# UZ-SLAMLab/DefSLAM

Hardware: AMD Instinct MI355X
Metric: SfT GN iters/sec (500-node mesh, 1k matches) (higher is better)
Workload: dtype f64

## Files before the change

### defslam_amd/_lib.py

```python
from __future__ import annotations

import ctypes as C
import os

_HERE = os.path.dirname(os.path.abspath(__file__))
LIB_PATH = os.path.join(_HERE, "lib", "libdefslam_hip.so")
LAB_LIB_PATH = os.path.join(_HERE, "lib", "libdefslam_hip_lab.so")

DSH_OK = 0
DSH_ERR_ARG = 1
DSH_ERR_STATE = 3
DSH_TRACE_STRIDE = 8
DSH_MAX_ITERS = 64

c_double_p = C.POINTER(C.c_double)
c_float_p = C.POINTER(C.c_float)
c_i32_p = C.POINTER(C.c_int32)
c_u8_p = C.POINTER(C.c_uint8)


class SftFrameC(C.Structure):
    _fields_ = [
        ("Tcw", c_float_p),
        ("K", C.c_double * 4),
# ... 37 lines not shown

class BbsC(C.Structure):
    _fields_ = [("umin", C.c_double), ("umax", C.c_double), ("nptsu", C.c_int32), ("vmin", C.c_double), ("vmax", C.c_double),
                ("nptsv", C.c_int32), ("valdim", C.c_int32)]


SchwarpProblemC._fields_ = [("bbs", BbsC), ("P", C.c_int32), ("kp1", C.c_void_p), ("kp2", C.c_void_p), ("invsig", C.c_void_p), ("fx_slot", C.c_double),
                            ("fy_slot", C.c_double), ("lam", C.c_double), ("fx", C.c_float), ("fy", C.c_float), ("max_iters", C.c_int32), ("x", C.c_void_p),
                            ("diff", C.c_void_p), ("drop", C.c_void_p), ("info", C.c_int32 * 2), ("costs", C.c_double * 2), ("init_lambda", C.c_double), ("init_ok", C.c_int32)]



class SchwarpStoreC(C.Structure):
    _fields_ = [("point_id", C.c_void_p), ("idx2", C.c_void_p), ("tag", C.c_int32)]


class TrackFrameC(C.Structure):
    _fields_ = [("Tcw", c_float_p), ("Ow", C.c_float * 3), ("K", C.c_float * 4), ("bounds", C.c_float * 4), ("grid_cols", C.c_int32),
                ("grid_rows", C.c_int32), ("levels", C.c_int32), ("scale_factors", c_float_p), ("log_scale_factor", C.c_float), ("N", C.c_int32),
                ("kp", c_float_p), ("octave", c_i32_p), ("desc", c_u8_p), ("state", c_u8_p)]


class TrackProblemC(C.Structure):
    _fields_ = [("frame", TrackFrameC), ("mode", C.c_int32), ("th", C.c_float), ("Q", C.c_int32), ("xyz", c_float_p), ("octave", c_i32_p),
                ("normal", c_float_p), ("max_distance", c_float_p), ("desc", c_u8_p), ("skip", c_u8_p), ("match", c_i32_p), ("in_view", c_u8_p),
                ("level", c_i32_p), ("uv", c_float_p), ("view_cos", c_float_p), ("nmatches", C.c_int32), ("rescans", C.c_int32)]


DSH_TRACK_FRAME = 0
DSH_TRACK_LOCAL = 1


class MpKeyFrameC(C.Structure):
    _fields_ = [("Ow", C.c_float * 3), ("N", C.c_int32), ("desc", c_u8_p), ("octave", c_i32_p), ("levels", C.c_int32),
                ("scale_factors", c_float_p), ("bad", C.c_int32)]


DSH_MP_DESCRIPTOR = 1
DSH_MP_NORMAL_DEPTH = 2
DSH_MP_NO_OBS = 1
DSH_MP_NO_GOOD_DESC = 2
DSH_MP_MAX_OBS = 65535


class MpdbDescC(C.Structure):
    _fields_ = [("ctx", C.c_void_p), ("point_capacity", C.c_int32), ("keyframe_capacity", C.c_int32), ("observation_capacity", C.c_int64)]


DSH_MPDB_POSITION = 1
DSH_MPDB_NORMAL_DEPTH = 2
DSH_MPDB_DESCRIPTOR = 4


class TrackCloseCountsC(C.Structure):
    _fields_ = [(n, C.c_int32) for n in ("matches_inliers", "matches_outliers", "to_match_local", "observed", "inliers", "outliers",
                                         "local_map_points", "n_moved")]


class TrackEndCountsC(C.Structure):
    _fields_ = [(n, C.c_int32) for n in ("cleaned", "dropped", "kept")]


class PoseOnlyProblemC(C.Structure):
    _fields_ = [("Tcw", c_float_p), ("K", C.c_float * 4), ("N", C.c_int32), ("kp", c_float_p), ("octave", c_i32_p), ("levels", C.c_int32),
                ("inv_level_sigma2", c_float_p), ("frame_points", c_i32_p), ("outlier", c_u8_p), ("Tcw_out", C.c_float * 16),
                ("pose", C.c_double * 7), ("n_initial", C.c_int32), ("n_bad", C.c_int32), ("n_good", C.c_int32), ("rounds", C.c_int32),
                ("iters", C.c_int32 * 4), ("trials", C.c_int32 * 4), ("bad", C.c_int32 * 4), ("chi2", C.c_double * 4)]


class KfKeypointsC(C.Structure):
    _fields_ = [("rows", C.c_int32), ("cols", C.c_int32), ("N", C.c_int32), ("kp", c_float_p)]


class SurfaceGridC(C.Structure):
    _fields_ = [("ctx", C.c_void_p), ("bbs", C.POINTER(BbsC)), ("depth_ctrl", c_double_p), ("Twc", c_float_p), ("xs", C.c_int32), ("ys", C.c_int32)]


class TemplateSwitchCountsC(C.Structure):
    _fields_ = [(n, C.c_int32) for n in ("n_new", "first_id", "n_moved", "n_masked", "n_embedded", "n_points")]


class TemplateSwitchInputC(C.Structure):
    _fields_ = [("kfdb", C.c_void_p), ("slot", C.c_int32), ("kf", C.POINTER(KfKeypointsC)), ("surface_pts", c_float_p), ("Twc", c_float_p)]


class AnchorListsC(C.Structure):
    _fields_ = ([(n, C.c_int32) for n in ("anchor_capacity", "pair_capacity", "query_capacity")] + [("max_matrix_bytes", C.c_int64)] +
                [(n, c_i32_p) for n in ("anchor_slot", "anchor_count", "anchor_pairs", "pair_ptr", "pair_idx1", "pair_idx2", "pair_point")] +
                [("pair_own", c_u8_p)] + [(n, c_i32_p) for n in ("query_ptr", "query_idx1", "query_point")] + [("has", c_u8_p)] +
                [(n, C.c_int32) for n in ("n_anchors", "n_pairs", "n_queries", "n_no_ref")])


DSH_MP_NO_REF = 4
DSH_MP_SKIPPED_BAD = 8
DSH_UPKEEP_IDS = 0
DSH_UPKEEP_EMBEDDED = 1


class KeyframeProcessInputC(C.Structure):
    _fields_ = [("kfdb", C.c_void_p), ("slot", C.c_int32)]


class KeyframeProcessCountsC(C.Structure):
    _fields_ = [(n, C.c_int32) for n in ("n_empty", "n_bad", "n_added", "n_recent", "n_no_good_desc", "n_no_ref")] + [("first_record", C.c_int64)]


class PointUpkeepInputC(C.Structure):
    _fields_ = [("kfdb", C.c_void_p), ("what", C.c_int32), ("select", C.c_int32), ("n", C.c_int32), ("ids", c_i32_p)]


class PointUpkeepCountsC(C.Structure):
    _fields_ = [(n, C.c_int32) for n in ("n_selected", "n_no_obs", "n_no_good_desc", "n_no_ref", "n_bad")]


class PointEraseCountsC(C.Structure):
    _fields_ = [(n, C.c_int32) for n in ("n_found", "n_ref_moved", "n_set_bad", "n_records", "n_entries")]


DIFFPROP_FIELDS = ["I1u", "I1v", "I2u", "I2v", "J12a", "J12b", "J12c", "J12d", "J21a", "J21b", "J21c", "J21d",
                   "H12uux", "H12uuy", "H12uvx", "H12uvy", "H12vvx", "H12vvy"]


EXPORTED_SYMBOLS = [
    "dsh_create", "dsh_destroy", "dsh_last_error", "dsh_stream", "dsh_synchronize",
    "dsh_template_build", "dsh_template_set", "dsh_template_dims", "dsh_template_get", "dsh_template_embed",
    "dsh_sft_solve", "dsh_sft_batch_upload", "dsh_sft_batch_run", "dsh_sft_batch_download",
    "dsh_sft_batch_counts", "dsh_sft_batch_problem_info",
    "dsh_bbs_eval", "dsh_bbs_coloc", "dsh_normals_estimate", "dsh_schwarp_eval", "dsh_schwarp_fit", "dsh_schwarp_fit_batch",
    "dsh_sfn_estimate", "dsh_bbs_bending", "dsh_warp_initialize", "dsh_search_by_schwarp",
    "dsh_template_embed_device", "dsh_scale_min_median", "dsh_optimize_horn", "dsh_surface_register",
    "dsh_comm_unique_id", "dsh_comm_create", "dsh_comm_destroy", "dsh_sft_shared_solve", "dsh_sft_shared_solve_group", "dsh_sft_connected_solve", "dsh_sft_connected_solve_group",
    "dsh_diffdb_create", "dsh_diffdb_destroy", "dsh_diffdb_clear", "dsh_diffdb_count", "dsh_diffdb_append", "dsh_schwarp_fit_batch_store",
    "dsh_normals_estimate_db", "dsh_sfn_estimate_db",
    "dsh_search_by_projection_batch", "dsh_search_by_projection_frame", "dsh_search_by_projection_local",
    "dsh_kfdb_create", "dsh_kfdb_destroy", "dsh_kfdb_clear", "dsh_kfdb_add", "dsh_kfdb_set_bad", "dsh_kfdb_count", "dsh_mappoint_update",
    "dsh_mpdb_create", "dsh_mpdb_destroy", "dsh_mpdb_clear", "dsh_mpdb_point_count", "dsh_mpdb_keyframe_count", "dsh_mpdb_add_points",
    "dsh_mpdb_update_points", "dsh_mpdb_set_points_bad", "dsh_mpdb_add_observations", "dsh_mpdb_erase_observations", "dsh_mpdb_add_keyframe",
    "dsh_mpdb_set_keyframe_point", "dsh_mpdb_set_keyframe_parent", "dsh_mpdb_set_keyframe_bad",
    "dsh_local_map_update", "dsh_local_map_points", "dsh_local_map_search",
    "dsh_trackstate_set_embedding", "dsh_trackstate_clear_embedding", "dsh_trackstate_set_counters", "dsh_trackstate_get",
    "dsh_trackstate_seed_local_points", "dsh_trackstate_repose", "dsh_trackstate_cull", "dsh_track_close_frame",
    "dsh_track_end_frame", "dsh_track_last_frame", "dsh_motion_model_search",
    "dsh_track_pose_only", "dsh_track_pose_only_batch",
    "dsh_surface_vertices", "dsh_need_new_template", "dsh_template_switch", "dsh_point_store_get_points", "dsh_point_store_get_embedding",
    "dsh_point_store_add_observations_indexed", "dsh_point_store_set_reference_keyframes", "dsh_point_store_get_reference_keyframes", "dsh_keyframe_anchors",
    "dsh_keyframe_process_new", "dsh_point_store_upkeep",
    "dsh_point_store_erase_observations", "dsh_point_store_set_bad", "dsh_point_store_cull", "dsh_point_store_get_observations",
    "dsh_point_store_get_keyframe_table",
]
DSH_COMM_ID_BYTES = 128

LAB_SYMBOLS = ["dsh_lab_set_option", "dsh_lab_sft_run_timed", "dsh_lab_sft_assemble_timed", "dsh_lab_sft_phase_ms", "dsh_lab_sft_step_trace",
               "dsh_lab_sft_system", "dsh_lab_sft_solver_info", "dsh_lab_sft_wave_check", "dsh_lab_sft_dump", "dsh_lab_sft_rounds_timed",
               "dsh_lab_sft_factor_check"]

_lib = None
_lab = None


def load() -> C.CDLL:
    global _lib
    if _lib is None:
        _lib = _bind(LIB_PATH, lab=False)
    return _lib


def load_lab() -> C.CDLL:
    global _lab
    if _lab is None:
        _lab = _bind(LAB_LIB_PATH, lab=True)
    return _lab


def _bind(path: str, lab: bool) -> C.CDLL:
    if not os.path.exists(path):
        raise OSError(f"{path} is missing: run `python -c 'import __graft_entry__ as g; g.build()'` "
                      f"(or `make -C defslam_amd/csrc`). There is no CPU fallback.")
    L = C.CDLL(path)
    vp = C.c_void_p
    L.dsh_create.argtypes = [C.POINTER(vp), C.c_int]
    L.dsh_destroy.argtypes = [vp]
    L.dsh_last_error.argtypes = [vp]
    L.dsh_last_error.restype = C.c_char_p
    L.dsh_stream.argtypes = [vp]
    L.dsh_stream.restype = vp
    L.dsh_synchronize.argtypes = [vp]
    L.dsh_template_build.argtypes = [vp, C.c_int, c_double_p, C.c_int, c_i32_p]
    L.dsh_template_set.argtypes = [vp, C.c_int, c_double_p, c_u8_p, c_i32_p, c_i32_p, c_double_p, c_double_p, C.c_int, c_i32_p,
                                   c_double_p, C.c_double]
    L.dsh_template_dims.argtypes = [vp, c_i32_p, c_i32_p, c_i32_p]
    L.dsh_template_get.argtypes = [vp, c_u8_p, c_i32_p, c_i32_p, c_double_p, c_double_p, c_i32_p, c_double_p, c_double_p]
    L.dsh_template_embed.argtypes = [vp, C.c_int, c_float_p, c_i32_p, c_i32_p, c_float_p]
    L.dsh_sft_solve.argtypes = [vp, C.POINTER(SftFrameC), C.POINTER(SftResultC)]
    L.dsh_sft_batch_upload.argtypes = [vp, C.c_int, C.POINTER(SftFrameC)]
    L.dsh_sft_batch_run.argtypes = [vp]
    L.dsh_sft_batch_download.argtypes = [vp, C.c_int, C.POINTER(SftResultC)]
    L.dsh_sft_batch_counts.argtypes = [vp, C.POINTER(C.c_int64), C.POINTER(C.c_int64)]
    L.dsh_sft_batch_problem_info.argtypes = [vp, C.c_int, C.POINTER(C.c_int64), c_i32_p]
    L.dsh_bbs_eval.argtypes = [vp, C.POINTER(BbsC), c_double_p, c_double_p, c_double_p, C.c_int, C.c_int, C.c_int, c_double_p, c_u8_p]
    L.dsh_bbs_coloc.argtypes = [vp, C.POINTER(BbsC), c_double_p, c_double_p, C.c_int, C.c_int, C.c_int, c_i32_p, c_double_p, c_i32_p]
    L.dsh_normals_estimate.argtypes = [vp, C.c_int, c_i32_p, c_float_p, c_u8_p, c_float_p, c_u8_p, c_float_p, c_u8_p, c_float_p,
                                       c_double_p, c_double_p, c_i32_p, c_float_p, c_float_p, c_u8_p, c_i32_p]
    L.dsh_schwarp_eval.argtypes = [vp, C.POINTER(BbsC), C.c_int, c_float_p, c_float_p, c_float_p, C.c_double, C.c_double, C.c_double, c_double_p,
                                   c_double_p, c_double_p]
    L.dsh_schwarp_fit.argtypes = [vp, C.POINTER(BbsC), C.c_int, c_float_p, c_float_p, c_float_p, C.c_double, C.c_double, C.c_double, C.c_float,
                                  C.c_float, C.c_int, c_double_p, c_float_p, c_u8_p, c_i32_p, c_double_p]
    L.dsh_schwarp_fit_batch.argtypes = [vp, C.c_int, C.POINTER(SchwarpProblemC)]
    L.dsh_diffdb_create.argtypes = [vp, C.c_int64, C.POINTER(vp)]
    L.dsh_diffdb_destroy.argtypes = [vp]
    L.dsh_diffdb_clear.argtypes = [vp]
    L.dsh_diffdb_count.argtypes = [vp]
    L.dsh_diffdb_count.restype = C.c_int64
    L.dsh_diffdb_append.argtypes = [vp, C.c_int, c_float_p, c_i32_p, c_i32_p, c_i32_p]
    L.dsh_schwarp_fit_batch_store.argtypes = [vp, C.c_int, C.POINTER(SchwarpProblemC), C.POINTER(SchwarpStoreC), vp]
    L.dsh_normals_estimate_db.argtypes = [vp, vp, C.c_int, c_i32_p, c_float_p, c_u8_p, c_float_p, c_double_p, c_double_p, c_i32_p, c_float_p, c_i32_p,
                                          C.c_int32, c_i32_p, c_i32_p, c_i32_p, c_i32_p, c_float_p, c_u8_p]
    L.dsh_sfn_estimate.argtypes = [vp, C.POINTER(BbsC), C.c_int, c_double_p, c_double_p, c_float_p, C.c_double, C.c_double, C.c_int, c_double_p, c_double_p,
                                   c_double_p, c_double_p, c_float_p, c_i32_p]
    L.dsh_sfn_estimate_db.argtypes = [vp, C.POINTER(BbsC), vp, C.c_int, c_i32_p, c_double_p, c_double_p, C.c_double, C.c_double, C.c_int, c_double_p, c_double_p,
                                      c_double_p, c_double_p, c_float_p, c_i32_p]
    L.dsh_bbs_bending.argtypes = [C.POINTER(BbsC), C.c_double, c_double_p]
    L.dsh_search_by_schwarp.argtypes = [vp, C.POINTER(BbsC), c_double_p, C.c_int, c_float_p, c_u8_p, c_float_p, c_float_p, C.c_int, C.c_int, C.c_int, c_float_p,
                                        c_u8_p, c_u8_p, C.c_float, C.c_int, c_i32_p, c_i32_p]
    L.dsh_warp_initialize.argtypes = [vp, C.POINTER(BbsC), C.c_int, c_float_p, c_float_p, C.c_double, c_double_p, c_i32_p]
    c_i64_p = C.POINTER(C.c_int64)
    L.dsh_template_embed_device.argtypes = [vp, C.c_int, c_float_p, c_i32_p, c_i32_p, c_float_p]
    L.dsh_scale_min_median.argtypes = [vp, C.c_int, c_float_p, c_float_p, c_double_p, C.c_int64, c_float_p, c_i64_p, c_i32_p]
    L.dsh_optimize_horn.argtypes = [vp, C.c_int, c_float_p, c_float_p, c_double_p, C.c_double, C.c_double, c_i32_p, c_double_p]
    L.dsh_surface_register.argtypes = [vp, C.c_int, c_float_p, c_float_p, c_double_p, C.c_int64, c_float_p, C.c_double, C.c_int, c_i32_p, c_double_p,
                                       c_double_p, c_float_p, c_double_p]
    L.dsh_comm_unique_id.argtypes = [vp]
    L.dsh_comm_create.argtypes = [vp, C.c_int, C.c_int, vp, C.POINTER(vp)]
    L.dsh_comm_destroy.argtypes = [vp]
    L.dsh_sft_shared_solve.argtypes = [vp, vp, C.POINTER(SftFrameC), C.POINTER(SftResultC)]
    L.dsh_sft_shared_solve_group.argtypes = [C.c_int, C.POINTER(vp), C.POINTER(SftFrameC), C.POINTER(SftResultC)]
    L.dsh_sft_connected_solve.argtypes = [vp, vp, C.POINTER(SftFrameC), C.POINTER(SftResultC)]
    L.dsh_sft_connected_solve_group.argtypes = [vp, vp, C.POINTER(SftFrameC), C.POINTER(SftResultC)]
    L.dsh_search_by_projection_batch.argtypes = [vp, C.c_int, C.POINTER(TrackProblemC)]
    L.dsh_search_by_projection_frame.argtypes = [vp, C.POINTER(TrackFrameC), C.c_int, c_float_p, c_i32_p, c_u8_p, C.c_float, c_i32_p, c_i32_p]
    L.dsh_search_by_projection_local.argtypes = [vp, C.POINTER(TrackFrameC), C.c_int, c_float_p, c_float_p, c_float_p, c_u8_p, c_u8_p, C.c_float,
                                                 c_i32_p, c_u8_p, c_i32_p, c_i32_p]
    L.dsh_kfdb_create.argtypes = [vp, C.c_int32, C.POINTER(vp)]
    L.dsh_kfdb_destroy.argtypes = [vp]
    L.dsh_kfdb_clear.argtypes = [vp]
    L.dsh_kfdb_add.argtypes = [vp, C.POINTER(MpKeyFrameC), c_i32_p]
    L.dsh_kfdb_set_bad.argtypes = [vp, C.c_int32, C.c_int32]
    L.dsh_kfdb_count.argtypes = [vp]
    L.dsh_mappoint_update.argtypes = [vp, vp, C.c_int, c_float_p, c_i32_p, c_i32_p, c_i32_p, c_i32_p, C.c_int32, c_u8_p, c_i32_p, c_float_p,
                                      c_float_p, c_float_p, c_i32_p]
    i32 = C.c_int32
    L.dsh_mpdb_create.argtypes = [C.POINTER(MpdbDescC), C.POINTER(vp)]
    L.dsh_mpdb_destroy.argtypes = [vp]
    L.dsh_mpdb_clear.argtypes = [vp]
    L.dsh_mpdb_point_count.argtypes = [vp]
    L.dsh_mpdb_keyframe_count.argtypes = [vp]
    L.dsh_mpdb_add_points.argtypes = [vp, C.c_int, c_float_p, c_float_p, c_float_p, c_u8_p, c_u8_p, c_i32_p]
    L.dsh_mpdb_update_points.argtypes = [vp, C.c_int, c_i32_p, i32, c_float_p, c_float_p, c_float_p, c_u8_p]
    L.dsh_mpdb_set_points_bad.argtypes = [vp, C.c_int, c_i32_p, c_u8_p]
    L.dsh_mpdb_add_observations.argtypes = [vp, C.c_int, c_i32_p, c_i32_p]
    L.dsh_mpdb_erase_observations.argtypes = [vp, C.c_int, c_i32_p, c_i32_p]
    L.dsh_mpdb_add_keyframe.argtypes = [vp, i32, c_i32_p, i32, i32, c_i32_p]
    L.dsh_mpdb_set_keyframe_point.argtypes = [vp, i32, i32, i32]
    L.dsh_mpdb_set_keyframe_parent.argtypes = [vp, i32, i32]
    L.dsh_mpdb_set_keyframe_bad.argtypes = [vp, i32, i32]
    L.dsh_local_map_update.argtypes = [vp, C.c_int, c_i32_p, c_u8_p, i32, c_i32_p, c_i32_p, c_i32_p, c_i32_p, c_i32_p, c_i32_p]
    L.dsh_local_map_points.argtypes = [vp, i32, c_i32_p, c_i32_p]
    L.dsh_local_map_search.argtypes = [vp, C.POINTER(TrackFrameC), C.c_float, i32, c_i32_p, c_i32_p, c_u8_p, c_i32_p, c_float_p, c_float_p, c_i32_p]
    L.dsh_trackstate_set_embedding.argtypes = [vp, C.c_int, c_i32_p, c_i32_p, c_double_p]
    L.dsh_trackstate_clear_embedding.argtypes = [vp]
    L.dsh_trackstate_set_counters.argtypes = [vp, C.c_int, c_i32_p, c_i32_p, c_i32_p]
    L.dsh_trackstate_get.argtypes = [vp, C.c_int, c_i32_p, c_i32_p, c_i32_p, c_i32_p, c_float_p]
    L.dsh_trackstate_seed_local_points.argtypes = [vp, C.c_int, c_i32_p]
    L.dsh_trackstate_repose.argtypes = [vp, C.c_int, c_double_p, c_i32_p]
    L.dsh_trackstate_cull.argtypes = [vp, C.c_int, c_i32_p, c_i32_p, i32, c_u8_p]
    L.dsh_track_close_frame.argtypes = [vp, C.POINTER(TrackFrameC), C.c_int, c_i32_p, c_u8_p, C.c_int, c_double_p, i32, C.POINTER(TrackCloseCountsC)]
    L.dsh_track_end_frame.argtypes = [vp, C.c_int, c_i32_p, c_u8_p, c_i32_p, c_i32_p, c_u8_p, C.POINTER(TrackEndCountsC)]
    L.dsh_track_last_frame.argtypes = [vp, i32, c_i32_p, c_i32_p, c_i32_p]
    L.dsh_motion_model_search.argtypes = [vp, C.POINTER(TrackFrameC), C.c_float, C.c_float, i32, c_i32_p, c_i32_p, c_i32_p, c_float_p]
    L.dsh_track_pose_only.argtypes = [vp, C.POINTER(PoseOnlyProblemC)]
    L.dsh_track_pose_only_batch.argtypes = [vp, C.c_int, C.POINTER(PoseOnlyProblemC)]
    L.dsh_surface_vertices.argtypes = [C.POINTER(SurfaceGridC), c_double_p]
    L.dsh_need_new_template.argtypes = [vp, i32, C.POINTER(KfKeypointsC), c_i32_p, c_u8_p]
    L.dsh_template_switch.argtypes = [vp, C.POINTER(TemplateSwitchInputC), c_i32_p, C.POINTER(TemplateSwitchCountsC)]
    L.dsh_point_store_get_points.argtypes = [vp, C.c_int, c_i32_p, c_float_p, c_float_p, c_float_p, c_u8_p, c_u8_p]
    L.dsh_point_store_get_embedding.argtypes = [vp, C.c_int, c_i32_p, c_i32_p, c_double_p]
    L.dsh_point_store_add_observations_indexed.argtypes = [vp, C.c_int, c_i32_p, c_i32_p, c_i32_p]
    L.dsh_point_store_set_reference_keyframes.argtypes = [vp, C.c_int, c_i32_p, c_i32_p]
    L.dsh_point_store_get_reference_keyframes.argtypes = [vp, C.c_int, c_i32_p, c_i32_p]
    L.dsh_keyframe_anchors.argtypes = [vp, i32, i32, C.POINTER(AnchorListsC)]
    L.dsh_keyframe_process_new.argtypes = [vp, C.POINTER(KeyframeProcessInputC), c_u8_p, c_i32_p, C.POINTER(KeyframeProcessCountsC)]
    L.dsh_point_store_upkeep.argtypes = [vp, C.POINTER(PointUpkeepInputC), c_i32_p, C.POINTER(PointUpkeepCountsC)]
    L.dsh_point_store_erase_observations.argtypes = [vp, C.c_int, c_i32_p, c_i32_p, i32, c_u8_p, C.POINTER(PointEraseCountsC)]
    L.dsh_point_store_set_bad.argtypes = [vp, C.c_int, c_i32_p, C.POINTER(PointEraseCountsC)]
    L.dsh_point_store_cull.argtypes = [vp, C.c_int, c_i32_p, c_i32_p, i32, c_u8_p, C.POINTER(PointEraseCountsC)]
    L.dsh_point_store_get_observations.argtypes = [vp, C.c_int, c_i32_p, c_i32_p, i32, c_i32_p, c_i32_p, c_i32_p]
    L.dsh_point_store_get_keyframe_table.argtypes = [vp, i32, i32, c_i32_p]
    for name in EXPORTED_SYMBOLS:
        fn = getattr(L, name)
        if name not in ("dsh_last_error", "dsh_stream"):
            fn.restype = C.c_int
    if lab:
        L.dsh_lab_set_option.argtypes = [vp, C.c_char_p, C.c_int]
        L.dsh_lab_sft_run_timed.argtypes = [vp, C.c_int, c_double_p]
        L.dsh_lab_sft_assemble_timed.argtypes = [vp, C.c_int, c_double_p]
        L.dsh_lab_sft_phase_ms.argtypes = [vp, C.c_int, c_double_p]
        L.dsh_lab_sft_step_trace.argtypes = [vp, C.c_int, c_double_p]
        L.dsh_lab_sft_system.argtypes = [vp, C.c_int, C.c_int32, c_double_p, c_double_p, c_double_p]
        L.dsh_lab_sft_solver_info.argtypes = [vp, C.c_int, c_i32_p]
        L.dsh_lab_sft_wave_check.argtypes = [vp, C.c_double, C.c_int, C.c_int, c_double_p, c_double_p, c_i32_p, c_double_p]
        L.dsh_lab_sft_dump.argtypes = [vp, C.c_int, C.c_int, C.c_int64, c_double_p]
        L.dsh_lab_sft_rounds_timed.argtypes = [vp, c_double_p, c_i32_p]
        L.dsh_lab_sft_factor_check.argtypes = [vp, c_double_p, c_u8_p, C.c_int, c_double_p, c_i32_p]
        for name in LAB_SYMBOLS:
            getattr(L, name).restype = C.c_int
    return L


class HipEvents:

    def __init__(self):
        self._hip = C.CDLL("libamdhip64.so")
        self._hip.hipEventCreate.argtypes = [C.POINTER(C.c_void_p)]
        self._hip.hipEventRecord.argtypes = [C.c_void_p, C.c_void_p]
        self._hip.hipEventSynchronize.argtypes = [C.c_void_p]
        self._hip.hipEventElapsedTime.argtypes = [C.POINTER(C.c_float), C.c_void_p, C.c_void_p]
        self._hip.hipEventDestroy.argtypes = [C.c_void_p]
        self.e0, self.e1 = C.c_void_p(), C.c_void_p()
        for e in (self.e0, self.e1):
            if self._hip.hipEventCreate(C.byref(e)) != 0:
                raise OSError("hipEventCreate failed")

    def start(self, stream: int):
        if self._hip.hipEventRecord(self.e0, C.c_void_p(stream)) != 0:
            raise OSError("hipEventRecord failed")

    def stop_ms(self, stream: int) -> float:
        ms = C.c_float()
        if (self._hip.hipEventRecord(self.e1, C.c_void_p(stream)) != 0 or self._hip.hipEventSynchronize(self.e1) != 0
                or self._hip.hipEventElapsedTime(C.byref(ms), self.e0, self.e1) != 0):
            raise OSError("HIP event timing failed")
        return float(ms.value)

    def close(self):
        for e in (self.e0, self.e1):
            if e:
                self._hip.hipEventDestroy(e)
        self.e0 = self.e1 = None


HIP_DEVICE_ATTRIBUTE_MULTIPROCESSOR_COUNT = 63


def device_cus(device: int = 0) -> int:
    hip = C.CDLL("libamdhip64.so")
    hip.hipDeviceGetAttribute.argtypes = [C.POINTER(C.c_int), C.c_int, C.c_int]
    n = C.c_int(0)
    if hip.hipDeviceGetAttribute(C.byref(n), HIP_DEVICE_ATTRIBUTE_MULTIPROCESSOR_COUNT, int(device)) != 0 or n.value <= 0:
        raise OSError("hipDeviceGetAttribute(hipDeviceAttributeMultiprocessorCount) failed")
    return int(n.value)
```

### defslam_amd/csrc/dsh_api.cpp

```cpp
#include <hip/hip_runtime.h>

#include <algorithm>
#include <cmath>
#include <cstdio>
#include <cstdlib>
#include <cstring>

#include <memory>
#include <mutex>
#include <string>
#include <vector>

#include "dsh_sft_ctx.h"

#include "mapping_launch.h"

#ifdef DSH_LAB
#include "../../include/defslam_hip_debug.h"
#endif

LdsMarks g_lds_marks[64];
std::mutex g_lds_mu;

using dsh::Tcw_from_pose7;

dsh_ctx_base* dsh_base(dsh_ctx* ctx) { return static_cast<dsh_ctx_base*>(ctx); }
const dsh::TemplateHost* dsh_facet_template(dsh_ctx_base* c) {
  const dsh_ctx* x = static_cast<const dsh_ctx*>(c);
  return x && x->tmpl.valid && x->tmpl.F > 0 ? &x->tmpl : nullptr;
}

namespace {

void drop_graphs(dsh_ctx* c) {
  if (!c->host_only && c->stream) (void)hipStreamSynchronize(c->stream);
  for (auto& g : c->graphs)
    if (g->d_base) (void)hipFree(g->d_base);
  c->graphs.clear();
  c->packed.clear();
}

int upload_template(dsh_ctx* c) {
  c->B = 0;
  c->ran = false;
  drop_graphs(c);
  if (c->host_only) return DSH_OK;
  const dsh::TemplateHost& t = c->tmpl;
  Arena a;
  const size_t o_xyz0 = a.take(sizeof(double) * 3 * t.n);
  const size_t o_ptr = a.take(sizeof(int32_t) * (t.n + 1));
  const size_t o_idx = a.take(sizeof(int32_t) * t.nbr_idx.size());
  const size_t o_w = a.take(sizeof(double) * t.nbr_w.size());
  const size_t o_sw = a.take(sizeof(double) * t.n);
  const size_t o_k0 = a.take(sizeof(double) * t.n);
  if (c->d_tmpl) { (void)hipFree(c->d_tmpl); c->d_tmpl = nullptr; }
  HIPCHK(c, hipMalloc((void**)&c->d_tmpl, a.size));
  c->d_tmpl_bytes = a.size;
  std::vector<char> st(a.size, 0);
  std::memcpy(&st[o_xyz0], t.xyz0.data(), sizeof(double) * 3 * t.n);
  std::memcpy(&st[o_ptr], t.nbr_ptr.data(), sizeof(int32_t) * (t.n + 1));
  std::memcpy(&st[o_idx], t.nbr_idx.data(), sizeof(int32_t) * t.nbr_idx.size());
  std::memcpy(&st[o_w], t.nbr_w.data(), sizeof(double) * t.nbr_w.size());
  std::memcpy(&st[o_sw], t.nbr_sumw.data(), sizeof(double) * t.n);
  std::memcpy(&st[o_k0], t.k0.data(), sizeof(double) * t.n);
  HIPCHK(c, hipMemcpy(c->d_tmpl, st.data(), a.size, hipMemcpyHostToDevice));
  c->dt.xyz0 = (const double*)(c->d_tmpl + o_xyz0);
  c->dt.nbr_ptr = (const int32_t*)(c->d_tmpl + o_ptr);
  c->dt.nbr_idx = (const int32_t*)(c->d_tmpl + o_idx);
  c->dt.nbr_w = (const double*)(c->d_tmpl + o_w);
  c->dt.nbr_sumw = (const double*)(c->d_tmpl + o_sw);
  c->dt.k0 = (const double*)(c->d_tmpl + o_k0);
  return DSH_OK;
}

template <class T>
size_t reserve(Arena& a, const std::vector<T>& v) { return a.take(sizeof(T) * v.size()); }
template <class T>
void put(char* st, size_t off, const std::vector<T>& v) {
  if (!v.empty()) std::memcpy(st + off, v.data(), sizeof(T) * v.size());
}

int graph_for(dsh_ctx* c, const std::vector<uint8_t>& opt, dsh::SftGraph** out, std::string& err) {
  uint64_t h = 1469598103934665603ull;
  for (uint8_t b : opt) { h ^= b; h *= 1099511628211ull; }
  for (auto& g : c->graphs)
    if (g->opt_hash == h && g->opt == opt) { g->last_use = c->upload_serial; *out = g.get(); return DSH_OK; }
  if (c->graphs.size() >= 64) {
    if (!c->host_only && c->stream) (void)hipStreamSynchronize(c->stream);
    auto& gs = c->graphs;
    for (size_t i = 0; i < gs.size();) {
      if (gs[i]->last_use != c->upload_serial) {
        if (gs[i]->d_base) (void)hipFree(gs[i]->d_base);
        gs.erase(gs.begin() + i);
      } else {
        i++;
      }
    }
  }
  std::unique_ptr<dsh::SftGraph> g(new dsh::SftGraph());
  const int rc = dsh::build_graph(c->tmpl, opt, *g, err);
  if (rc != DSH_OK) return rc;
  g->last_use = c->upload_serial;
  if (!c->host_only) {
    Arena a;
    auto& o = g->o;
    o.act = reserve(a, g->act); o.actnode = reserve(a, g->actnode); o.star_node = reserve(a, g->star_node); o.star_sL = reserve(a, g->star_sL);
    o.str_nodes = reserve(a, g->str_nodes); o.str_L0 = reserve(a, g->str_L0); o.off_ptr = reserve(a, g->off_ptr); o.off_rc = reserve(a, g->off_rc);
    o.sh_ptr = reserve(a, g->sh_ptr); o.sh_rec = reserve(a, g->sh_rec); o.sh_cf = reserve(a, g->sh_cf); o.tmask = reserve(a, g->tmask);
    o.hgather = reserve(a, g->hgather);
    o.hgatherT = reserve(a, g->hgatherT);
    std::vector<char> st(a.size, 0);
    put(st.data(), o.act, g->act); put(st.data(), o.actnode, g->actnode); put(st.data(), o.star_node, g->star_node); put(st.data(), o.star_sL, g->star_sL);
    put(st.data(), o.str_nodes, g->str_nodes); put(st.data(), o.str_L0, g->str_L0); put(st.data(), o.off_ptr, g->off_ptr); put(st.data(), o.off_rc, g->off_rc);
    put(st.data(), o.sh_ptr, g->sh_ptr); put(st.data(), o.sh_rec, g->sh_rec); put(st.data(), o.sh_cf, g->sh_cf); put(st.data(), o.tmask, g->tmask);
    put(st.data(), o.hgather, g->hgather);
    put(st.data(), o.hgatherT, g->hgatherT);
    if (hipMalloc((void**)&g->d_base, a.size) != hipSuccess) { err = "out of device memory (graph)"; return DSH_ERR_HIP; }
    g->d_bytes = a.size;
    if (hipMemcpy(g->d_base, st.data(), a.size, hipMemcpyHostToDevice) != hipSuccess) { (void)hipFree(g->d_base); err = "graph upload failed"; return DSH_ERR_HIP; }
  }
  *out = g.get();
  c->graphs.push_back(std::move(g));
  return DSH_OK;
}

int pack_problem(dsh_ctx* c, const dsh_sft_frame& f, Packed& P, std::string& err) {
  const dsh::TemplateHost& t = c->tmpl;
  std::vector<uint8_t> viewed, opt;
  int rc = dsh::frame_active_set(t, f, viewed, opt, err);
  if (rc != DSH_OK) return rc;
  rc = graph_for(c, opt, &P.g, err);
  if (rc != DSH_OK) return rc;
  const dsh::SftGraph& g = *P.g;
  rc = dsh::pack_frame(t, g, f, viewed, P.f, err);
  if (rc != DSH_OK) return rc;
  SftDev& h = P.h;
  h = SftDev{};
  h.n = t.n; h.nA = g.nA; h.Dn = 3 * g.nA; h.kd = g.kd; h.ldh = h.kd + 1;
  h.M = f.M; h.V = P.f.V; h.S = g.S; h.Es = g.Es; h.noff = g.noff; h.max_iters = f.max_iters; h.mode = 0;
  h.fx = f.K[0]; h.fy = f.K[1]; h.cx = f.K[2]; h.cy = f.K[3];
  h.w_ref = f.reg_temp / std::pow(t.median_L, 2);
  h.w_curv = f.reg_lap / (double)g.nA;
  h.w_str = g.Es > 0 ? f.reg_inex / (double)g.Es : 0.0;
  const float deltaMono = (float)std::sqrt(5.991);
  h.hub_delta = (double)deltaMono;
  h.hub_dsqr = h.hub_delta * h.hub_delta;
  return DSH_OK;
}

int run_rounds_enqueue(dsh_ctx* c);
int run_rounds(dsh_ctx* c) {
  const int rc = run_rounds_enqueue(c);
  if (rc != DSH_OK)
    for (int s = 0; s < c->plan.n_sub; s++) if (c->sub_stream[s]) (void)hipStreamSynchronize(c->sub_stream[s]);
  return rc;
}
int run_rounds_enqueue(dsh_ctx* c) {
  const int B = c->B, S = c->plan.n_sub;
  int b0[kSftMaxSub + 1];
  for (int s = 0; s <= S; s++) b0[s] = (int)((long long)B * s / S);
  int tail_below = -1;
  if (S == 1 && c->opt.tail != 0) {
    if (c->opt.tail > 0) tail_below = c->opt.tail * c->num_cus;
    else tail_below = std::min(4 * c->num_cus, std::max(2 * c->num_cus, (int)((long long)3 * B / 4)));
  }
  auto launch = [&](int s, int phase) {
    const bool ev = c->phase_events && S == 1;
    if (ev) { hipEvent_t e; if (hipEventCreate(&e) == hipSuccess) { (void)hipEventRecord(e, c->stream); c->phase_events->push_back(e); c->phase_ids.push_back(phase); } }
    hipError_t r;
    {
      LDS_LOCK();
      if (phase == SFTB_PH_TAIL) r = sftb_tail_launch(c->d_probs + b0[s], c->d_runs + b0[s], c->d_counters + 16 * s, b0[s + 1] - b0[s], c->plan.max_kd, c->plan.jl_doubles, &LDS_MARKS(c).tail, c->num_cus, tail_below, c->sub_stream[s]);
      else r = sftb_launch(c->d_probs + b0[s], c->d_runs + b0[s], c->d_counters + 16 * s, c->d_linlist + b0[s], b0[s + 1] - b0[s], phase, c->plan.jl_doubles, c->plan.xyz_doubles, LDS_MARKS(c).b,
                           c->num_cus, tail_below, c->sub_stream[s]);
    }
    if (ev) { hipEvent_t e; if (hipEventCreate(&e) == hipSuccess) { (void)hipEventRecord(e, c->stream); c->phase_events->push_back(e); } }
    return r;
  };
  if (S > 1) {
    HIPCHK(c, hipEventRecord(c->sub_event[0], c->stream));
    for (int s = 1; s < S; s++) HIPCHK(c, hipStreamWaitEvent(c->sub_stream[s], c->sub_event[0], 0));
  }
  for (int s = 0; s < S; s++) HIPCHK(c, launch(s, SFTB_PH_INIT));
  const int worst = std::max(1, c->plan.max_iters_batch) * 10 + 1;
  int rounds = 0, group = std::max(1, std::min(worst, c->rounds_hint));
  if (tail_below >= B) group = 0;
  HIPCHK(c, c->spec_done.ensure(64 * kSftMaxSub, true));
  int rc = DSH_OK;
  while (true) {
    for (int i = 0; i < group && rounds < worst; i++, rounds++)
      for (int s = 0; s < S; s++) {
        HIPCHK(c, launch(s, SFTB_PH_LIN));
        HIPCHK(c, launch(s, SFTB_PH_FACTOR));
        HIPCHK(c, launch(s, SFTB_PH_TRIAL));
      }
    if (tail_below >= 0) HIPCHK(c, launch(0, SFTB_PH_TAIL));
    for (int s = 0; s < S; s++) HIPCHK(c, hipMemcpyAsync(c->spec_done.p + 64 * s, c->d_counters + 16 * s, 8 * sizeof(int), hipMemcpyDeviceToHost, c->sub_stream[s]));
    for (int s = 0; s < S; s++) HIPCHK(c, hipStreamSynchronize(c->sub_stream[s]));
    int done = 0;
    for (int s = 0; s < S; s++) done += *reinterpret_cast<const int*>(c->spec_done.p + 64 * s);
    const int* c0 = reinterpret_cast<const int*>(c->spec_done.p);
    if (done >= B) { c->rounds_hint = (tail_below >= 0 && c0[6]) ? std::max(1, c0[7]) : rounds; break; }
    if (rounds >= worst) { rc = dsh_fail(c, DSH_ERR_STATE, "batched rounds: a problem did not terminate within its trial budget"); break; }
    group = 2;
  }
  return rc;
}

int run_once(dsh_ctx* c) {
  if (c->plan.rounds_mode) return run_rounds(c);
  if (c->plan.K <= 1) {
    LDS_LOCK();
    HIPCHK(c, sft_lm_launch(c->d_probs, c->B, c->plan.max_kd, c->plan.jl_doubles, c->plan.nw, LDS_MARKS(c).lm, c->stream));
    return DSH_OK;
  }
  const int K = c->plan.K, B = c->B;
  HIPCHK(c, hipMemsetAsync(c->d_spec, 0, sizeof(SftSpec) * (size_t)B * K, c->stream));
  const int rounds_per_iter = (10 + K - 1) / K;
  const int worst = c->plan.max_iters_batch * rounds_per_iter;
  auto launch = [&](int phase) { LDS_LOCK(); return sft_spec_launch(c->d_probs, c->d_spec, B, K, phase, c->plan.nh, c->opt.owner_waves, c->plan.max_kd, c->plan.jl_doubles, LDS_MARKS(c).spec, c->stream); };
  if (c->plan.nh > 0) HIPCHK(c, hipMemsetAsync(c->d_sync, 0, c->layout.sync_total, c->stream));
  HIPCHK(c, launch(SFT_SPEC_INIT));
  int rounds = 0, group = std::max(2, std::min(worst, c->spec_hint));
  HIPCHK(c, c->spec_done.ensure(sizeof(SftSpec) * (size_t)B, true));
  while (true) {
    for (int i = 0; i < group && rounds < worst; i++, rounds++) {
      HIPCHK(c, launch(SFT_SPEC_LIN));
      if (c->plan.any_split) {
        HIPCHK(c, launch(SFT_SPEC_FACTOR));
        HIPCHK(c, launch(SFT_SPEC_SOLVE));
      }
      HIPCHK(c, launch(SFT_SPEC_TRIAL));
    }
    HIPCHK(c, launch(SFT_SPEC_LIN));
    HIPCHK(c, hipMemcpyAsync(c->spec_done.p, c->d_spec, sizeof(SftSpec) * (size_t)B, hipMemcpyDeviceToHost, c->stream));
    HIPCHK(c, hipStreamSynchronize(c->stream));
    const SftSpec* sp = reinterpret_cast<const SftSpec*>(c->spec_done.p);
    bool all_done = true;
    int needed = 0;
    for (int b = 0; b < B; b++) { all_done = all_done && sp[b].done; needed = std::max(needed, sp[b].launches); }
    if (all_done) { c->spec_hint = needed; break; }
    if (rounds >= worst) return dsh_fail(c, DSH_ERR_STATE, "speculative trials: a problem did not terminate within its launch budget");
    group = 2;
  }
  return DSH_OK;
}


SftBatchLayout layout_batch(const SftBatchPlan& plan, const std::vector<Packed>& packed, int B) {
  const int K = plan.K, nh = plan.nh;
  SftBatchLayout L;
  Arena a;
  L.o_tab = a.take(sizeof(SftDev) * B * K);
  L.ro.resize(B);
  for (int b = 0; b < B; b++) {
    const dsh::SftFramePack& F = packed[b].f;
    SftBatchLayout::ReadOnly& o = L.ro[b];
    o.obs_nodes = reserve(a, F.obs_nodes); o.obs_bary = reserve(a, F.obs_bary); o.obs_uv = reserve(a, F.obs_uv); o.obs_w = reserve(a, F.obs_w);
    o.ob_ptr = reserve(a, F.ob_ptr); o.ob_m = reserve(a, F.ob_m); o.ob_c = reserve(a, F.ob_c); o.viewed = reserve(a, F.viewed);
    o.xyz_init = reserve(a, F.xyz_init);
    o.pose_init = a.take(8 * 8);
  }
  L.ro_bytes = a.size;
  L.res_off = a.size;
  (void)a.take(sizeof(SftResHdr) * (size_t)B);
  L.res_offs.resize(B);
  for (int b = 0; b < B; b++) {
    const SftDev& h = packed[b].h;
    SftBatchLayout::Result& r = L.res_offs[b];
    r.xyz = a.take(8 * 3 * (size_t)h.n) - L.res_off; r.chi2 = a.take(8 * (size_t)h.M) - L.res_off;
    r.trace = a.take(8 * DSH_TRACE_STRIDE * DSH_MAX_ITERS) - L.res_off;
    r.mp = a.take(4 * 3 * (size_t)h.M) - L.res_off; r.outl = a.take((size_t)h.M) - L.res_off;
  }
  L.res_bytes = a.size - L.res_off;
  L.ws.resize((size_t)B * K);
  L.ws_off = a.size;
  L.o_spec = a.take(sizeof(SftSpec) * (size_t)B * K);
  L.o_runs = a.take(plan.rounds_mode ? sizeof(SftRun) * (size_t)B + 64 * kSftMaxSub + sizeof(int) * (size_t)B : 0);
  if (nh > 0)
    for (int e = 0; e < B * K; e++) {
      const SftProblemPlan& p = plan.prob[e % B];
      if (p.split) for (int g = 0; g < 2; g++) L.sync_total += Arena::round((size_t)4 * (16 + p.part[g].nT));
    }
  L.o_sync = a.take(L.sync_total);
  size_t sync_used = 0;
  for (int e = 0; e < B * K; e++) {
    const int b = e % B, lane = e / B;
    const SftDev& h = packed[b].h;
    const SftProblemPlan& p = plan.prob[b];
    const size_t Dnp = (size_t)((h.Dn + kNB - 1) / kNB) * kNB;
    SftBatchLayout::Work& w = L.ws[e];
    w.sx0 = a.take(K > 1 ? 8 * 3 * (size_t)h.n : 0); w.sx1 = a.take(K > 1 ? 8 * 3 * (size_t)h.n : 0);
    w.shadow_xyz = a.take(lane ? 8 * 3 * (size_t)h.n : 0); w.shadow_chi2 = a.take(lane ? 8 * (size_t)h.M : 0); w.shadow_hdr = a.take(lane ? sizeof(SftResHdr) : 0);
    w.bak = a.take(8 * 3 * (size_t)h.n);
    w.camrec = a.take(8 * (size_t)h.M * SFT_CAM_STRIDE);
    w.wtv = a.take(p.lds_class >= 1 ? 0 : 8 * ((size_t)h.M + 1)); w.Jstar = a.take(p.lds_class >= 1 ? 0 : 8 * 4 * (size_t)h.S);
    w.Anode = a.take(p.lds_class >= 2 ? 0 : 8 * 6 * (size_t)h.nA); w.Jstr = a.take(p.lds_class >= 2 ? 0 : 8 * 4 * (size_t)h.Es);
    const size_t band_elems = p.tile_mode ? (Dnp / kTS + SFT_H_PAD_TILE_ROWS) * (size_t)p.tpr * kTS * kTS : Dnp * (size_t)h.ldh;
    const size_t bord_elems = (SFT_BORDER + 1) * Dnp + SFT_H_PAD_BORDER;
    w.Hc = a.take(p.tile_mode == 1 ? 8 * packed[b].g->hc_elems() : 0);
    w.Hb = a.take(p.tile_mode == 1 ? 0 : 8 * band_elems); w.Hbord = a.take(8 * bord_elems); w.Hcn = a.take(8 * 56);
    w.Lb = a.take(8 * band_elems); w.Lbord = a.take(8 * bord_elems); w.Lc = a.take(8 * 56);
    w.Linv = a.take(8 * (Dnp / kTS) * (size_t)kTS * kTS);
    w.Lt = a.take(p.tile_mode == 2 ? 8 * band_elems : 0); w.LbT = a.take(p.tile_mode == 2 ? 8 * (Dnp / kTS) * (size_t)kTS * kTS : 0);
    w.x = a.take(8 * (Dnp + 8)); w.dbg = a.take(1024);
    if (p.split)
      for (int g = 0; g < 4; g++) {
        const SftPart& q = p.part[g];
        const size_t tiles = 8 * (size_t)q.nT * q.tpr * kTS * kTS, col = 8 * (size_t)q.nT * kTS * kTS;
        SftBatchLayout::Part& po = w.part[g];
        po.Hb = a.take(g < 2 && lane == 0 ? tiles : 0);
        po.Lb = a.take(tiles); po.Lt = a.take(tiles); po.LbT = a.take(col); po.Linv = a.take(col);
        po.Lbord = a.take(8 * 8 * (size_t)kTS * q.nT); po.x = a.take(8 * ((size_t)kTS * q.nT + 8)); po.xchg = a.take(8 * (size_t)p.sp_xl);
        const bool helped = nh > 0 && g < 2;
        po.Pf = a.take(helped ? tiles : 0); po.PfB = a.take(helped ? col : 0);
        po.sync = L.o_sync + sync_used;
        if (helped) sync_used += Arena::round((size_t)4 * (16 + q.nT));
      }
  }
  L.size = a.size;
  return L;
}

void stage_read_only(char* st, const SftBatchLayout& L, const std::vector<Packed>& packed, int B) {
  for (int b = 0; b < B; b++) {
    const dsh::SftFramePack& F = packed[b].f;
    const SftBatchLayout::ReadOnly& o = L.ro[b];
    put(st, o.obs_nodes, F.obs_nodes); put(st, o.obs_bary, F.obs_bary); put(st, o.obs_uv, F.obs_uv); put(st, o.obs_w, F.obs_w);
    put(st, o.ob_ptr, F.ob_ptr); put(st, o.ob_m, F.ob_m); put(st, o.ob_c, F.ob_c); put(st, o.viewed, F.viewed); put(st, o.xyz_init, F.xyz_init);
    std::memcpy(st + o.pose_init, F.pose_init, 7 * sizeof(double));
  }
}

SftDev bind_entry(const std::vector<Packed>& packed, const dsh_ctx::TemplateDev& dt, char* base, const SftBatchLayout& L, const SftBatchPlan& plan, int B, int e) {
  const int b = e % B, lane = e / B;
  const dsh::SftGraph& g = *packed[b].g;
  const SftBatchLayout::ReadOnly& o = L.ro[b];
  const SftBatchLayout::Result& r = L.res_offs[b];
  const SftBatchLayout::Work& w = L.ws[e];
  SftDev h = packed[b].h;
  plan.prob[b].apply(h);
  char* rbase = base + L.res_off;
  SftResHdr* d_hdr = (SftResHdr*)rbase;
  const char* gb = g.d_base;
  h.xyz0 = dt.xyz0; h.nbr_ptr = dt.nbr_ptr; h.nbr_idx = dt.nbr_idx; h.nbr_w = dt.nbr_w; h.nbr_sumw = dt.nbr_sumw; h.k0 = dt.k0;
  h.act = (const int32_t*)(gb + g.o.act); h.actnode = (const int32_t*)(gb + g.o.actnode); h.star_node = (const int32_t*)(gb + g.o.star_node);
  h.star_sL = (const double*)(gb + g.o.star_sL); h.str_nodes = (const int32_t*)(gb + g.o.str_nodes); h.str_L0 = (const double*)(gb + g.o.str_L0);
  h.off_ptr = (const int32_t*)(gb + g.o.off_ptr); h.off_rc = (const int32_t*)(gb + g.o.off_rc); h.sh_ptr = (const int32_t*)(gb + g.o.sh_ptr);
  h.sh_rec = (const uint32_t*)(gb + g.o.sh_rec); h.sh_cf = (const double*)(gb + g.o.sh_cf); h.tmask = (const int32_t*)(gb + g.o.tmask);
  h.hgather = (const uint32_t*)(gb + g.o.hgather);
  h.hgatherT = (const uint32_t*)(gb + g.o.hgatherT);
  h.obs_nodes = (const int32_t*)(base + o.obs_nodes); h.obs_bary = (const double*)(base + o.obs_bary);
  h.obs_uv = (const double*)(base + o.obs_uv); h.obs_w = (const double*)(base + o.obs_w);
  h.ob_ptr = (const int32_t*)(base + o.ob_ptr); h.ob_m = (const int32_t*)(base + o.ob_m); h.ob_c = (const double*)(base + o.ob_c);
  h.viewed = (const uint8_t*)(base + o.viewed);
  h.xyz_init = (const double*)(base + o.xyz_init); h.pose_init = (const double*)(base + o.pose_init);
  h.res = d_hdr + b; h.pose = d_hdr[b].pose;
  h.xyz = (double*)(rbase + r.xyz); h.chi2_obs = (double*)(rbase + r.chi2); h.trace = (double*)(rbase + r.trace);
  h.mappoint = (float*)(rbase + r.mp); h.outlier = (uint8_t*)(rbase + r.outl);
  h.xyz_bak = (double*)(base + w.bak);
  h.camrec = (double*)(base + w.camrec); h.wtv = (double*)(base + w.wtv); h.Anode = (double*)(base + w.Anode);
  h.Jstar = (double*)(base + w.Jstar); h.Jstr = (double*)(base + w.Jstr);
  h.Hc = (double*)(base + w.Hc); h.Hb = (double*)(base + w.Hb); h.Hbord = (double*)(base + w.Hbord); h.Hcorner = (double*)(base + w.Hcn);
  h.Lb = (double*)(base + w.Lb); h.Lbord = (double*)(base + w.Lbord); h.Lcorner = (double*)(base + w.Lc); h.Linv = (double*)(base + w.Linv);
  h.Lt = (double*)(base + w.Lt); h.LbT = (double*)(base + w.LbT);
  h.x = (double*)(base + w.x); h.dbg = (double*)(base + w.dbg);
  h.spec_xyz[0] = (double*)(base + w.sx0); h.spec_xyz[1] = (double*)(base + w.sx1);
  if (h.split)
    for (int g = 0; g < 4; g++) {
      const SftBatchLayout::Part& po = w.part[g];
      SftPart& q = h.part[g];
      q.Hb = g < 2 ? (double*)(base + L.ws[b].part[g].Hb) : (double*)(base + po.xchg);
      q.Lb = (double*)(base + po.Lb); q.Lt = (double*)(base + po.Lt); q.LbT = (double*)(base + po.LbT); q.Linv = (double*)(base + po.Linv);
      q.Lbord = (double*)(base + po.Lbord); q.x = (double*)(base + po.x); q.xchg = (double*)(base + po.xchg);
      const bool helped = plan.nh > 0 && g < 2;
      q.Pf = helped ? (double*)(base + po.Pf) : nullptr; q.PfB = helped ? (double*)(base + po.PfB) : nullptr;
      q.sync = helped ? (int32_t*)(base + po.sync) : nullptr;
    }
  if (lane) {
    h.xyz = (double*)(base + w.shadow_xyz); h.chi2_obs = (double*)(base + w.shadow_chi2);
    h.res = (SftResHdr*)(base + w.shadow_hdr); h.pose = ((SftResHdr*)(base + w.shadow_hdr))->pose;
    h.trace = nullptr; h.mappoint = nullptr; h.outlier = nullptr;
    if (h.tile_mode == 1 || h.split) {
      const SftBatchLayout::Work& w0 = L.ws[b];
      h.Hc = (double*)(base + w0.Hc); h.Hbord = (double*)(base + w0.Hbord); h.Hcorner = (double*)(base + w0.Hcn);
    }
  }
  return h;
}

int sub_streams(dsh_ctx* c, int want) {
  for (int i = 1; i < want; i++)
    if (!c->sub_stream[i] && hipStreamCreateWithFlags(&c->sub_stream[i], hipStreamNonBlocking) != hipSuccess) c->sub_stream[i] = nullptr;
  for (int i = 0; i < want; i++) if (!c->sub_stream[i] || !c->sub_event[0]) return 1;
  return want;
}

}

int dsh_sft_upload(dsh_ctx* c, int B, const dsh_sft_frame* frames, SftUploadMode mode) {
  if (!c || B <= 0 || !frames) return dsh_fail(c, DSH_ERR_ARG, "dsh_sft_batch_upload: bad argument");
  if (!c->tmpl.valid) return dsh_fail(c, DSH_ERR_STATE, "dsh_sft_batch_upload: no template");
  if (!c->host_only) (void)hipSetDevice(c->device);
  c->B = 0;
  c->ran = false;
  c->upload_serial++;
  if ((int)c->packed.size() != B) c->packed.resize(B);
  std::vector<SftSizes> sizes(B);
  for (int b = 0; b < B; b++) {
    std::string e;
    const int rc = pack_problem(c, frames[b], c->packed[b], e);
    if (rc != DSH_OK) return dsh_fail(c, rc, "problem " + std::to_string(b) + ": " + e);
    const SftDev& h = c->packed[b].h;
    sizes[b] = SftSizes{h.n, h.nA, h.Dn, h.kd, h.M, h.S, h.Es, h.max_iters};
  }
  SftBatchPlan plan = sft_plan_batch(sizes.data(), B, c->num_cus, c->opt, c->host_only, mode);
  if (c->host_only) {
    c->h_probs.resize(B);
    for (int b = 0; b < B; b++) { c->h_probs[b] = c->packed[b].h; plan.prob[b].apply(c->h_probs[b]); }
    c->plan = std::move(plan);
    c->B = B;
    return DSH_OK;
  }
  if (sft_lm_kernel_lds_bytes(plan.max_kd, plan.jl_doubles) > 160 * 1024 || plan.max_kd + kNB + SFT_BORDER > SFT_NT)
    return dsh_fail(c, DSH_ERR_ARG, "half-bandwidth too large for the LDS panel / workgroup");
  if (plan.n_sub > 1) plan.n_sub = sub_streams(c, plan.n_sub);
  SftBatchLayout L = layout_batch(plan, c->packed, B);
  bool fresh_arena = false;
  if (L.size > c->d_batch_cap) {
    HIPCHK(c, hipStreamSynchronize(c->stream));
    if (c->d_batch) { (void)hipFree(c->d_batch); c->d_batch = nullptr; c->d_batch_cap = 0; }
    HIPCHK(c, hipMalloc((void**)&c->d_batch, L.size));
    c->d_batch_cap = L.size;
    fresh_arena = true;
  }
  if (c->stage_busy) { HIPCHK(c, hipEventSynchronize(c->stage_free)); c->stage_busy = false; }
  HIPCHK(c, c->stage.ensure(L.ro_bytes, true));
  char* st = c->stage.p;
  char* base = c->d_batch;
  const size_t entries = (size_t)B * plan.K;
  c->h_probs.resize(entries);
  for (size_t e = 0; e < entries; e++) c->h_probs[e] = bind_entry(c->packed, c->dt, base, L, plan, B, (int)e);
  std::memcpy(st + L.o_tab, c->h_probs.data(), sizeof(SftDev) * entries);
  stage_read_only(st, L, c->packed, B);
  HIPCHK(c, hipMemcpyAsync(base, st, L.ro_bytes, hipMemcpyHostToDevice, c->stream));
  HIPCHK(c, hipEventRecord(c->stage_free, c->stream));
  c->stage_busy = true;
  if (fresh_arena) HIPCHK(c, hipMemsetAsync(base + L.ws_off, 0, L.size - L.ws_off, c->stream));
  HIPCHK(c, hipMemsetAsync(base + L.res_off, 0, L.res_bytes, c->stream));
  c->d_probs = (SftDev*)(base + L.o_tab);
  c->d_spec = (SftSpec*)(base + L.o_spec);
  c->d_runs = (SftRun*)(base + L.o_runs);
  c->d_counters = (int*)(base + L.o_runs + sizeof(SftRun) * (size_t)B);
  c->d_linlist = c->d_counters + 16 * kSftMaxSub;
  c->d_sync = base + L.o_sync;
  c->plan = std::move(plan);
  c->layout = std::move(L);
  c->B = B;
  return DSH_OK;
}

extern "C" {

int dsh_create(dsh_ctx** out, int device) {
  if (!out) return DSH_ERR_ARG;
  *out = nullptr;
  if (device == -1) {
    dsh_ctx* hc = new dsh_ctx();
    hc->device = -1;
    hc->host_only = true;
    *out = hc;
    return DSH_OK;
  }
  int count = 0;
  if (hipGetDeviceCount(&count) != hipSuccess || count <= 0) return DSH_ERR_NO_DEVICE;
  if (device < 0 || device >= count) return DSH_ERR_ARG;
  dsh_ctx* c = new dsh_ctx();
  c->device = device;
  if (hipSetDevice(device) != hipSuccess || hipStreamCreateWithFlags(&c->stream, hipStreamNonBlocking) != hipSuccess) {
    delete c;
    return DSH_ERR_HIP;
  }
  if (hipEventCreateWithFlags(&c->stage_free, hipEventDisableTiming) != hipSuccess) {
    (void)hipStreamDestroy(c->stream);
    delete c;
    return DSH_ERR_HIP;
  }
  int cus = 0;
  if (hipDeviceGetAttribute(&cus, hipDeviceAttributeMultiprocessorCount, device) == hipSuccess && cus > 0) c->num_cus = cus;
  c->sub_stream[0] = c->stream;
  if (hipEventCreateWithFlags(&c->sub_event[0], hipEventDisableTiming) != hipSuccess) c->sub_event[0] = nullptr;
  *out = c;
  return DSH_OK;
}

int dsh_destroy(dsh_ctx* c) {
  if (!c) return DSH_ERR_ARG;
  dsh_detach_stores(c);
  if (c->host_only) { c->stage.release(); c->results.release(); delete c; return DSH_OK; }
  (void)hipSetDevice(c->device);
  drop_graphs(c);
  for (int i = 1; i < kSftMaxSub; i++) if (c->sub_stream[i]) { (void)hipStreamSynchronize(c->sub_stream[i]); (void)hipStreamDestroy(c->sub_stream[i]); }
  for (int i = 0; i < kSftMaxSub; i++) if (c->sub_event[i]) (void)hipEventDestroy(c->sub_event[i]);
  if (c->stream) { (void)hipStreamSynchronize(c->stream); (void)hipStreamDestroy(c->stream); }
  if (c->stage_free) (void)hipEventDestroy(c->stage_free);
  c->stage.release();
  c->results.release();
  c->spec_done.release();
  if (c->d_tmpl) (void)hipFree(c->d_tmpl);
  c->scratch.release();
  c->pin_in.release();
  c->pin_out.release();
  if (c->d_batch) (void)hipFree(c->d_batch);
  if (c->d_sc) (void)hipFree(c->d_sc);
  delete c;
  return DSH_OK;
}

const char* dsh_last_error(const dsh_ctx* c) { return c ? c->err.c_str() : "null context"; }
void* dsh_stream(dsh_ctx* c) { return c ? (void*)c->stream : nullptr; }
int dsh_synchronize(dsh_ctx* c) {
  if (const int rc = dsh_enter(c, "dsh_synchronize")) return rc;
  HIPCHK(c, hipStreamSynchronize(c->stream));
  return DSH_OK;
}

int dsh_template_build(dsh_ctx* c, int n, const double* xyz0, int F, const int32_t* facets) {
  if (!c || n <= 0 || F <= 0 || !xyz0 || !facets) return dsh_fail(c, DSH_ERR_ARG, "dsh_template_build: bad argument");
  for (int i = 0; i < 3 * F; i++)
    if (facets[i] < 0 || facets[i] >= n) return dsh_fail(c, DSH_ERR_ARG, "dsh_template_build: facet index out of range");
  if (!c->host_only) (void)hipSetDevice(c->device);
  c->tmpl.build(n, xyz0, F, facets);
  return upload_template(c);
}

int dsh_template_set(dsh_ctx* c, int n, const double* xyz0, const uint8_t* boundary, const int32_t* rp, const int32_t* col, const double* w,
                     const double* k0, int E, const int32_t* en, const double* eL, double median_L) {
  if (!c || n <= 0 || E < 0 || !xyz0 || !boundary || !rp || !col || !w || !k0 || !en || !eL) return dsh_fail(c, DSH_ERR_ARG, "dsh_template_set: bad argument");
  if (rp[0] != 0) return dsh_fail(c, DSH_ERR_ARG, "dsh_template_set: nbr_rowptr[0] != 0");
  for (int i = 0; i < n; i++)
    if (rp[i + 1] < rp[i]) return dsh_fail(c, DSH_ERR_ARG, "dsh_template_set: nbr_rowptr is not non-decreasing");
  for (int p = 0; p < rp[n]; p++)
    if (col[p] < 0 || col[p] >= n) return dsh_fail(c, DSH_ERR_ARG, "dsh_template_set: neighbour index out of range");
  for (int e = 0; e < E; e++) {
    if (en[2 * e] < 0 || en[2 * e] >= n || en[2 * e + 1] < 0 || en[2 * e + 1] >= n) return dsh_fail(c, DSH_ERR_ARG, "dsh_template_set: edge node out of range");
    if (!(eL[e] > 0.0)) return dsh_fail(c, DSH_ERR_ARG, "dsh_template_set: edge rest length must be positive");
  }
  if (!(median_L > 0.0)) return dsh_fail(c, DSH_ERR_ARG, "dsh_template_set: median edge length must be positive");
  if (!c->host_only) (void)hipSetDevice(c->device);
  c->tmpl.set(n, xyz0, boundary, rp, col, w, k0, E, en, eL, median_L);
  return upload_template(c);
}

int dsh_template_dims(const dsh_ctx* c, int32_t* n, int32_t* E, int32_t* nnz) {
  if (!c || !c->tmpl.valid) return DSH_ERR_STATE;
  if (n) *n = c->tmpl.n;
  if (E) *E = c->tmpl.E;
  if (nnz) *nnz = (int32_t)c->tmpl.nbr_idx.size();
  return DSH_OK;
}

int dsh_template_get(const dsh_ctx* c, uint8_t* boundary, int32_t* rp, int32_t* col, double* w, double* k0, int32_t* en, double* eL, double* med) {
  if (!c || !c->tmpl.valid) return DSH_ERR_STATE;
  const dsh::TemplateHost& t = c->tmpl;
  if (boundary) std::memcpy(boundary, t.boundary.data(), t.n);
  if (rp) std::memcpy(rp, t.nbr_ptr.data(), sizeof(int32_t) * (t.n + 1));
  if (col) std::memcpy(col, t.nbr_idx.data(), sizeof(int32_t) * t.nbr_idx.size());
  if (w) std::memcpy(w, t.nbr_w.data(), sizeof(double) * t.nbr_w.size());
  if (k0) std::memcpy(k0, t.k0.data(), sizeof(double) * t.n);
  if (en) std::memcpy(en, t.edge_nodes.data(), sizeof(int32_t) * 2 * t.E);
  if (eL) std::memcpy(eL, t.edge_L0.data(), sizeof(double) * t.E);
  if (med) *med = t.median_L;
  return DSH_OK;
}

int dsh_template_embed(const dsh_ctx* c, int P, const float* pts, int32_t* facet_id, int32_t* nodes, float* bary) {
  if (!c || !c->tmpl.valid || c->tmpl.F <= 0) return DSH_ERR_STATE;
  if (P < 0 || !pts || !facet_id || !nodes || !bary) return DSH_ERR_ARG;
  c->tmpl.embed(P, pts, facet_id, nodes, bary);
  return DSH_OK;
}

int dsh_template_embed_device(dsh_ctx* c, int P, const float* pts, int32_t* facet_id, int32_t* nodes, float* bary) {
  if (!c) return DSH_ERR_ARG;
  if (!c->tmpl.valid || c->tmpl.F <= 0) return dsh_fail(c, DSH_ERR_STATE, "dsh_template_embed_device: needs a template built from facets");
  if (P < 0 || (P > 0 && (!pts || !facet_id || !nodes || !bary))) return dsh_fail(c, DSH_ERR_ARG, "dsh_template_embed_device: bad argument");
  if (c->host_only) return dsh_fail(c, DSH_ERR_NO_DEVICE, "dsh_template_embed_device: host-only context, no GPU (dsh_template_embed is the host routine)");
  if (P == 0) return DSH_OK;
  if (const int rc = dsh_enter(c, "dsh_template_embed_device")) return rc;
  const dsh::TemplateHost& t = c->tmpl;
  const size_t Pz = (size_t)P;
  UpBlock up;
  const size_t o_pts = up.copy_of(pts, 12 * Pz), o_xyz = up.copy_of(t.xyz0.data(), 24 * (size_t)t.n), o_fac = up.copy_of(t.facets.data(), 12 * (size_t)t.F),
               o_ptr = up.copy_of(t.nf_ptr.data(), 4 * (size_t)(t.n + 1)), o_idx = up.copy_of(t.nf_idx.data(), 4 * t.nf_idx.size());
  DownBlock down;
  const size_t d_fid = down.copy_to(facet_id, 4 * Pz), d_nodes = down.copy_to(nodes, 12 * Pz), d_bary = down.copy_to(bary, 12 * Pz);
  if (const int rc = up.copy(c)) return rc;
  if (const int rc = down.alloc(c)) return rc;
  HIPCHK(c, reg_embed(P, up.dev<float>(o_pts), t.n, up.dev<double>(o_xyz), up.dev<int32_t>(o_fac), up.dev<int32_t>(o_ptr), up.dev<int32_t>(o_idx),
                      down.dev<int32_t>(d_fid), down.dev<int32_t>(d_nodes), down.dev<float>(d_bary), c->stream));
  return down.receive(c);
}

int dsh_sft_batch_upload(dsh_ctx* c, int B, const dsh_sft_frame* frames) { return dsh_sft_upload(c, B, frames, SftUploadMode::batch); }

int dsh_sft_batch_run(dsh_ctx* c) {
  if (!c) return DSH_ERR_ARG;
  if (const int rc = dsh_enter(c, "dsh_sft_batch_run")) return rc;
  if (c->B <= 0) return dsh_fail(c, DSH_ERR_STATE, "dsh_sft_batch_run: nothing uploaded");
  const int rc = run_once(c);
  if (rc != DSH_OK) return rc;
  c->ran = true;
  return DSH_OK;
}

int dsh_sft_batch_counts(dsh_ctx* c, int64_t* iters, int64_t* trials) {
  if (!c || c->B <= 0 || !c->ran) return DSH_ERR_STATE;
  if (const int rc = dsh_enter(c, "dsh_sft_batch_counts")) return rc;
  const size_t bytes = sizeof(SftResHdr) * (size_t)c->B;
  HIPCHK(c, c->results.ensure(std::max(bytes, c->results.cap), true));
  HIPCHK(c, hipMemcpyAsync(c->results.p, c->d_batch + c->layout.res_off, bytes, hipMemcpyDeviceToHost, c->stream));
  HIPCHK(c, hipStreamSynchronize(c->stream));
  const SftResHdr* hd = reinterpret_cast<const SftResHdr*>(c->results.p);
  int64_t it = 0, tr = 0;
  for (int b = 0; b < c->B; b++) { it += hd[b].iters; tr += hd[b].trials; }
  if (iters) *iters = it;
  if (trials) *trials = tr;
  return DSH_OK;
}

int dsh_sft_batch_problem_info(dsh_ctx* c, int b, int64_t* bytes, int32_t* counts) {
  if (!c || b < 0 || b >= c->B) return DSH_ERR_ARG;
  const Packed& P = c->packed[b];
  const SftDev& h = P.h;
  const int64_t M = h.M, n = h.n, C = P.g->n_curv_ref, E = h.Es, V = h.V;
  const int64_t reads = 60 * M + 24 * n + 88 + 92 * C + 16 * E + 28 * V;
  const int64_t writes = 8 * (30 * M + 21 * C + 6 * E + 9 * V) + 8 * (2 * M + C + E + 3 * V) + 8 * M;
  if (bytes) *bytes = reads + writes;
  if (counts) { counts[0] = h.M; counts[1] = h.nA; counts[2] = P.g->n_curv_ref; counts[3] = h.Es; counts[4] = h.V; counts[5] = 6 + h.Dn; counts[6] = h.kd; counts[7] = c->plan.rounds_mode ? 1 : c->plan.nw; counts[8] = P.g->noff; }
  return DSH_OK;
}

int dsh_sft_batch_download(dsh_ctx* c, int B, dsh_sft_result* res) {
  if (!c || !res || B != c->B) return dsh_fail(c, DSH_ERR_ARG, "dsh_sft_batch_download: bad argument");
  if (const int rc = dsh_enter(c, "dsh_sft_batch_download")) return rc;
  if (!c->ran) return dsh_fail(c, DSH_ERR_STATE, "dsh_sft_batch_download: no run");
  HIPCHK(c, c->results.ensure(c->layout.res_bytes, true));
  HIPCHK(c, hipMemcpyAsync(c->results.p, c->d_batch + c->layout.res_off, c->layout.res_bytes, hipMemcpyDeviceToHost, c->stream));
  HIPCHK(c, hipStreamSynchronize(c->stream));
  const char* rb = c->results.p;
  const SftResHdr* hd = reinterpret_cast<const SftResHdr*>(rb);
  for (int b = 0; b < B; b++) {
    const SftDev& h = c->h_probs[b];
    const Packed& P = c->packed[b];
    const SftBatchLayout::Result& o = c->layout.res_offs[b];
    dsh_sft_result& r = res[b];
    r.rep_error = hd[b].rep_error;
    r.inliers = hd[b].inliers;
    r.iters = hd[b].iters;
    r.trials = hd[b].trials;
    r.status = hd[b].status;
    r.dim = 6 + h.Dn;
    r.half_bandwidth = h.kd;
    if (r.chi2_obs) std::memcpy(r.chi2_obs, rb + o.chi2, 8 * (size_t)h.M);
    if (r.outlier) std::memcpy(r.outlier, rb + o.outl, (size_t)h.M);
    if (r.xyz) std::memcpy(r.xyz, rb + o.xyz, 8 * 3 * (size_t)h.n);
    if (r.pose7) std::memcpy(r.pose7, hd[b].pose, 8 * 7);
    if (r.Tcw) Tcw_from_pose7(hd[b].pose, r.Tcw);
    if (r.mappoint_xyz) std::memcpy(r.mappoint_xyz, rb + o.mp, 4 * 3 * (size_t)h.M);
    if (r.trace) {
      const size_t rows = (size_t)std::max(P.f.max_iters, 0), done = std::min(rows, (size_t)std::max(hd[b].iters, 0));
      std::memcpy(r.trace, rb + o.trace, 8 * DSH_TRACE_STRIDE * done);
      std::memset(r.trace + DSH_TRACE_STRIDE * done, 0, 8 * DSH_TRACE_STRIDE * (rows - done));
    }
  }
  return DSH_OK;
}

int dsh_sft_solve(dsh_ctx* c, const dsh_sft_frame* frame, dsh_sft_result* result) {
  if (!c || !frame || !result) return dsh_fail(c, DSH_ERR_ARG, "dsh_sft_solve: bad argument");
  int rc = dsh_sft_batch_upload(c, 1, frame);
  if (rc != DSH_OK) return rc;
  rc = dsh_sft_batch_run(c);
  if (rc != DSH_OK) return rc;
  return dsh_sft_batch_download(c, 1, result);
}

#ifdef DSH_LAB
namespace {
struct EventPair {
  hipEvent_t e0 = nullptr, e1 = nullptr;
  hipError_t create() { hipError_t e = hipEventCreate(&e0); return e != hipSuccess ? e : hipEventCreate(&e1); }
  ~EventPair() { if (e0) (void)hipEventDestroy(e0); if (e1) (void)hipEventDestroy(e1); }
};
}

int dsh_lab_set_option(dsh_ctx* c, const char* name, int value) {
  if (!c || !name) return DSH_ERR_ARG;
  const std::string k(name);
  if (k == "waves") { if (value != 0 && value != 4 && value != 8) return dsh_fail(c, DSH_ERR_ARG, "dsh_lab_set_option: waves is 0 (automatic), 4 or 8"); c->opt.waves = value; }
  else if (k == "dataflow") c->opt.dataflow = value != 0;
  else if (k == "wide_off") c->opt.wide_off = value != 0;
  else if (k == "rounds") c->opt.rounds = value != 0;
  else if (k == "streams") { if (value < 0 || value > kSftMaxSub) return dsh_fail(c, DSH_ERR_ARG, "dsh_lab_set_option: streams is 0 (automatic) or 1..4 sub-batches"); c->opt.streams = value; }
  else if (k == "split") { if (value < 0 || value > 2) return dsh_fail(c, DSH_ERR_ARG, "dsh_lab_set_option: split is 0 (off), 1 (wide bands only) or 2 (every band long enough)"); c->opt.split = value; }
  else if (k == "helpers_wbt") { if (value < 1 || value > 16) return dsh_fail(c, DSH_ERR_ARG, "dsh_lab_set_option: helpers_wbt is 1..16 (tiles of half-bandwidth from which parts get helper workgroups)"); c->opt.helpers_wbt = value; }
  else if (k == "owner_waves") { if (value != 8 && value != 16) return dsh_fail(c, DSH_ERR_ARG, "dsh_lab_set_option: owner_waves is 8 or 16 (wavefronts of a FACTOR workgroup with helpers)"); c->opt.owner_waves = value; }
  else if (k == "helpers") { if (value < -1 || value > 3) return dsh_fail(c, DSH_ERR_ARG, "dsh_lab_set_option: helpers is -1 (automatic) or 0..3 workgroups per part"); c->opt.helpers = value; }
  else if (k == "tail") { if (value < -1 || value > 8) return dsh_fail(c, DSH_ERR_ARG, "dsh_lab_set_option: tail is -1 (automatic), 0 (rounds to the end) or the number of problems per CU from which downwards the last problems go to the tail kernel"); c->opt.tail = value; }
  else if (k == "speculate") { if (value < 0 || value > SFT_SPEC_MAXK) return dsh_fail(c, DSH_ERR_ARG, "dsh_lab_set_option: speculate is 0 (automatic) or 1..4 lanes"); c->opt.speculate = value; }
  else return dsh_fail(c, DSH_ERR_ARG, "dsh_lab_set_option: unknown option " + k);
  return DSH_OK;
}

int dsh_lab_sft_solver_info(dsh_ctx* c, int b, int32_t* out8) {
  if (!c || !out8 || b < 0 || b >= c->B) return dsh_fail(c, DSH_ERR_ARG, "dsh_lab_sft_solver_info: bad argument");
  const SftDev& h = c->h_probs[b];
  out8[0] = h.split; out8[1] = h.sp_c0; out8[2] = h.sp_s; out8[3] = h.sp_n1p; out8[4] = h.sp_pad; out8[5] = c->plan.K; out8[6] = h.tile_mode; out8[7] = c->plan.nw;
  return DSH_OK;
}

int dsh_lab_sft_run_timed(dsh_ctx* c, int launches, double* total_ms) {
  if (!c || launches <= 0 || !total_ms) return dsh_fail(c, DSH_ERR_ARG, "dsh_lab_sft_run_timed: bad argument");
  if (const int rc = dsh_enter(c, "dsh_lab_sft_run_timed")) return rc;
  if (c->B <= 0) return dsh_fail(c, DSH_ERR_STATE, "dsh_lab_sft_run_timed: nothing uploaded");
  EventPair ev;
  HIPCHK(c, ev.create());
  HIPCHK(c, hipEventRecord(ev.e0, c->stream));
  for (int i = 0; i < launches; i++) { const int rc = run_once(c); if (rc != DSH_OK) return rc; }
  HIPCHK(c, hipEventRecord(ev.e1, c->stream));
  HIPCHK(c, hipEventSynchronize(ev.e1));
  float ms = 0.f;
  HIPCHK(c, hipEventElapsedTime(&ms, ev.e0, ev.e1));
  *total_ms = (double)ms;
  c->ran = true;
  return DSH_OK;
}

int dsh_lab_sft_assemble_timed(dsh_ctx* c, int launches, double* total_ms) {
  if (!c || launches <= 0 || !total_ms) return dsh_fail(c, DSH_ERR_ARG, "dsh_lab_sft_assemble_timed: bad argument");
  if (const int rc = dsh_enter(c, "dsh_lab_sft_assemble_timed")) return rc;
  if (c->B <= 0 || !c->ran) return dsh_fail(c, DSH_ERR_STATE, "dsh_lab_sft_assemble_timed: needs an uploaded batch that has run once");
  EventPair ev;
  HIPCHK(c, ev.create());
  HIPCHK(c, hipEventRecord(ev.e0, c->stream));
  for (int i = 0; i < launches; i++) HIPCHK(c, sft_assembly_launch(c->d_probs, c->B, c->plan.max_kd, c->plan.jl_doubles, c->plan.rounds_mode ? 8 : c->plan.nw, c->stream));
  HIPCHK(c, hipEventRecord(ev.e1, c->stream));
  HIPCHK(c, hipEventSynchronize(ev.e1));
  float ms = 0.f;
  HIPCHK(c, hipEventElapsedTime(&ms, ev.e0, ev.e1));
  *total_ms = ms;
  c->ran = false;
  return DSH_OK;
}

int dsh_lab_sft_wave_check(dsh_ctx* c, double rel, int launches, int only, double* x_ref, double* x_new, int32_t* ok2, double* ms2) {
  if (!c || launches <= 0 || !ms2) return dsh_fail(c, DSH_ERR_ARG, "dsh_lab_sft_wave_check: bad argument");
  if (const int rc = dsh_enter(c, "dsh_lab_sft_wave_check")) return rc;
  if (c->B <= 0 || !c->ran) return dsh_fail(c, DSH_ERR_STATE, "dsh_lab_sft_wave_check: needs an uploaded batch that has run once");
  for (int b = 0; b < c->B; b++)
    if (c->h_probs[b].tile_mode != 1) return dsh_fail(c, DSH_ERR_STATE, "dsh_lab_sft_wave_check: register-window problems (half-bandwidth <= 128) only");
  HIPCHK(c, sft_assembly_launch(c->d_probs, c->B, c->plan.max_kd, c->plan.jl_doubles, c->plan.rounds_mode ? 8 : c->plan.nw, c->stream));
  EventPair ev;
  HIPCHK(c, ev.create());
  for (int which = 0; which < 2; which++) {
    if (only == 2 - which) continue;
    HIPCHK(c, sft_wave_lab_launch(c->d_probs, c->B, which, rel, c->plan.max_kd, c->plan.jl_doubles, c->stream));
    HIPCHK(c, hipEventRecord(ev.e0, c->stream));
    for (int i = 0; i < launches; i++) HIPCHK(c, sft_wave_lab_launch(c->d_probs, c->B, which, rel, c->plan.max_kd, c->plan.jl_doubles, c->stream));
    HIPCHK(c, hipEventRecord(ev.e1, c->stream));
    HIPCHK(c, hipEventSynchronize(ev.e1));
    float ms = 0.f;
    HIPCHK(c, hipEventElapsedTime(&ms, ev.e0, ev.e1));
    ms2[which] = (double)ms / launches;
    double* dst = which == 0 ? x_ref : x_new;
    size_t off = 0;
    for (int b = 0; b < c->B; b++) {
      const SftDev& h = c->h_probs[b];
      const size_t Dnp = (size_t)((h.Dn + kNB - 1) / kNB) * kNB;
      if (dst) HIPCHK(c, hipMemcpy(dst + off, h.x, 8 * (Dnp + 6), hipMemcpyDeviceToHost));
      off += Dnp + 6;
      double flag = 0.0;
      if (ok2) { HIPCHK(c, hipMemcpy(&flag, h.dbg + 2, 8, hipMemcpyDeviceToHost)); ok2[2 * b + which] = (int32_t)flag; }
    }
  }
  return DSH_OK;
}

int dsh_lab_sft_factor_check(dsh_ctx* c, const double* lambda, const uint8_t* factor, int grid, double* x, int32_t* ok) {
  if (!c || !lambda || grid < 0) return dsh_fail(c, DSH_ERR_ARG, "dsh_lab_sft_factor_check: bad argument");
  if (const int rc = dsh_enter(c, "dsh_lab_sft_factor_check")) return rc;
  if (c->B <= 0 || !c->ran) return dsh_fail(c, DSH_ERR_STATE, "dsh_lab_sft_factor_check: needs an uploaded batch that has run once");
  for (int b = 0; b < c->B; b++)
    if (c->h_probs[b].tile_mode != 1) return dsh_fail(c, DSH_ERR_STATE, "dsh_lab_sft_factor_check: register-window problems (half-bandwidth <= 128) only");
  const int B = c->B;
  struct OwnedDevBuf { void* p = nullptr; ~OwnedDevBuf() { if (p) (void)hipFree(p); } } runs, counters;
  HIPCHK(c, hipMalloc(&runs.p, sizeof(SftRun) * (size_t)B));
  HIPCHK(c, hipMalloc(&counters.p, 16 * sizeof(int)));
  std::vector<SftRun> h_runs(B);
  for (int b = 0; b < B; b++) {
    SftRun& R = h_runs[b];
    std::memset(&R, 0, sizeof(R));
    R.lambda = lambda[b];
    R.state = (!factor || factor[b]) ? SFTB_TRIAL : SFTB_DONE;
    R.fact_ok = -1;
  }
  HIPCHK(c, sft_assembly_launch(c->d_probs, B, c->plan.max_kd, c->plan.jl_doubles, c->plan.rounds_mode ? 8 : c->plan.nw, c->stream));
  for (int b = 0; b < B; b++) HIPCHK(c, hipMemcpyAsync(c->h_probs[b].dbg + 1, &lambda[b], sizeof(double), hipMemcpyHostToDevice, c->stream));
  HIPCHK(c, hipMemcpyAsync(runs.p, h_runs.data(), sizeof(SftRun) * (size_t)B, hipMemcpyHostToDevice, c->stream));
  HIPCHK(c, hipMemsetAsync(counters.p, 0, 16 * sizeof(int), c->stream));
  HIPCHK(c, sftb_factor_lab_launch(c->d_probs, (SftRun*)runs.p, (int*)counters.p, B, grid ? grid : std::min(B, 4 * c->num_cus), c->stream));
  HIPCHK(c, hipStreamSynchronize(c->stream));
  HIPCHK(c, hipMemcpy(h_runs.data(), runs.p, sizeof(SftRun) * (size_t)B, hipMemcpyDeviceToHost));
  size_t off = 0;
  for (int b = 0; b < B; b++) {
    const SftDev& h = c->h_probs[b];
    const size_t Dnp = (size_t)((h.Dn + kNB - 1) / kNB) * kNB;
    if (x) HIPCHK(c, hipMemcpy(x + off, h.x, 8 * (Dnp + 6), hipMemcpyDeviceToHost));
    off += Dnp + 6;
    if (ok) ok[b] = h_runs[b].fact_ok;
  }
  return DSH_OK;
}

int dsh_lab_sft_rounds_timed(dsh_ctx* c, double* ms4, int32_t* rounds) {
  if (!c || !ms4) return dsh_fail(c, DSH_ERR_ARG, "dsh_lab_sft_rounds_timed: bad argument");
  if (const int rc = dsh_enter(c, "dsh_lab_sft_rounds_timed")) return rc;
  if (c->B <= 0 || !c->plan.rounds_mode) return dsh_fail(c, DSH_ERR_STATE, "dsh_lab_sft_rounds_timed: needs an uploaded batch that runs as rounds of phase kernels");
  std::vector<hipEvent_t> ev;
  c->phase_events = &ev;
  c->phase_ids.clear();
  const int rc = run_rounds(c);
  c->phase_events = nullptr;
  (void)hipStreamSynchronize(c->stream);
  for (int i = 0; i < 7; i++) ms4[i] = 0.0;
  { int32_t cnt[16] = {0}; if (hipMemcpy(cnt, c->d_counters, sizeof(cnt), hipMemcpyDeviceToHost) == hipSuccess) { ms4[5] = (double)cnt[8]; ms4[6] = (double)cnt[9]; } }
  int n_trial = 0;
  for (size_t i = 0; i + 1 < ev.size(); i += 2) {
    float ms = 0.f;
    (void)hipEventElapsedTime(&ms, ev[i], ev[i + 1]);
    const int ph = c->phase_ids[i / 2];
    ms4[ph == SFTB_PH_INIT ? 0 : ph == SFTB_PH_LIN ? 1 : ph == SFTB_PH_FACTOR ? 2 : ph == SFTB_PH_TRIAL ? 3 : 4] += ms;
    n_trial += ph == SFTB_PH_TRIAL;
  }
  if (rounds) *rounds = n_trial;
  for (hipEvent_t e : ev) (void)hipEventDestroy(e);
  if (rc == DSH_OK) c->ran = true;
  return rc;
}

int dsh_lab_sft_dump(dsh_ctx* c, int b, int what, int64_t n, double* out) {
  if (!c || !out || b < 0 || b >= c->B || n <= 0) return dsh_fail(c, DSH_ERR_ARG, "dsh_lab_sft_dump: bad argument");
  if (const int rc = dsh_enter(c, "dsh_lab_sft_dump")) return rc;
  const SftDev& h = c->h_probs[b];
  const double* src = what == 0 ? h.Lb : what == 1 ? h.Linv : what == 2 ? h.Lbord : what == 3 ? h.Hc : what == 4 ? h.Hbord : what == 5 ? h.x : what == 6 ? h.Hcorner :
                      (what == 8 || what == 9) ? (const double*)h.part[what - 8].sync : h.dbg;
  if (!src) return dsh_fail(c, DSH_ERR_STATE, "dsh_lab_sft_dump: the problem has no such buffer");
  HIPCHK(c, hipStreamSynchronize(c->stream));
  HIPCHK(c, hipMemcpy(out, src, 8 * (size_t)n, hipMemcpyDeviceToHost));
  return DSH_OK;
}

int dsh_lab_sft_phase_ms(dsh_ctx* c, int b, double* out8) {
  if (!c || !out8 || b < 0 || b >= c->B) return dsh_fail(c, DSH_ERR_ARG, "dsh_lab_sft_phase_ms: bad argument");
  if (const int rc = dsh_enter(c, "dsh_lab_sft_phase_ms")) return rc;
  if (!c->ran) return dsh_fail(c, DSH_ERR_STATE, "dsh_lab_sft_phase_ms: no run");
#ifndef SFT_PHASE_TIMERS
  return dsh_fail(c, DSH_ERR_STATE, "dsh_lab_sft_phase_ms: this build has no phase timers (make lab EXTRA=-DSFT_PHASE_TIMERS)");
#else
  HIPCHK(c, hipStreamSynchronize(c->stream));
  HIPCHK(c, hipMemcpy(out8, c->h_probs[b].dbg, 8 * sizeof(double), hipMemcpyDeviceToHost));
  for (int i = 0; i < 8; i++) out8[i] *= 1e-5;
  {
    double as[6];
    HIPCHK(c, hipMemcpy(as, c->h_probs[b].dbg + 32, sizeof(as), hipMemcpyDeviceToHost));
    std::fprintf(stderr, "[lab] assembly sections of problem %d, kcycles of wave 0: corner %.0f, diagonal gather %.0f, butterfly+finish %.0f, off-diagonal %.0f, round overhead %.0f; rounds %.0f\n",
                 b, as[0] * 1e-3, as[1] * 1e-3, as[2] * 1e-3, as[3] * 1e-3, as[4] * 1e-3, as[5]);
  }
  return DSH_OK;
#endif
}

int dsh_lab_sft_step_trace(dsh_ctx* c, int b, double* out64) {
  if (!c || !out64 || b < 0 || b >= c->B) return dsh_fail(c, DSH_ERR_ARG, "dsh_lab_sft_step_trace: bad argument");
  if (const int rc = dsh_enter(c, "dsh_lab_sft_step_trace")) return rc;
  if (!c->ran) return dsh_fail(c, DSH_ERR_STATE, "dsh_lab_sft_step_trace: no run");
#ifndef SFT_STEP_TRACE
  return dsh_fail(c, DSH_ERR_STATE, "dsh_lab_sft_step_trace: this build has no step trace (make lab EXTRA=-DSFT_STEP_TRACE)");
#else
  HIPCHK(c, hipStreamSynchronize(c->stream));
  HIPCHK(c, hipMemcpy(out64, c->h_probs[b].dbg + 16, 64 * sizeof(double), hipMemcpyDeviceToHost));
  return DSH_OK;
#endif
}

int dsh_lab_sft_system(dsh_ctx* c, int b, int32_t D, double* H, double* bvec, double* chi2) {
  if (!c || b < 0 || b >= c->B) return dsh_fail(c, DSH_ERR_ARG, "dsh_lab_sft_system: bad argument");
  if (const int rc = dsh_enter(c, "dsh_lab_sft_system")) return rc;
  HIPCHK(c, hipStreamSynchronize(c->stream));
  SftDev h = c->h_probs[b];
  if (D != 6 + h.Dn) return dsh_fail(c, DSH_ERR_ARG, "dsh_lab_sft_system: D mismatch");
  const int32_t mode_saved = h.mode, split_saved = h.split;
  h.mode = 1;
  h.split = 0;
  HIPCHK(c, hipMemcpy(c->d_probs + b, &h, sizeof(SftDev), hipMemcpyHostToDevice));
  { LDS_LOCK(); HIPCHK(c, sft_lm_launch(c->d_probs + b, 1, c->plan.max_kd, c->plan.jl_doubles, c->plan.nw, LDS_MARKS(c).lm, c->stream)); }
  HIPCHK(c, hipStreamSynchronize(c->stream));
  c->ran = false;
  h.mode = mode_saved;
  h.split = split_saved;
  HIPCHK(c, hipMemcpy(c->d_probs + b, &h, sizeof(SftDev), hipMemcpyHostToDevice));
  const size_t Dnp = (size_t)((h.Dn + kNB - 1) / kNB) * kNB;
  const size_t band_elems = h.tile_mode ? (Dnp / kTS) * (size_t)h.tpr * kTS * kTS : Dnp * (size_t)h.ldh;
  std::vector<double> Hb(h.tile_mode == 1 ? 0 : band_elems), Hbord(SFT_BORDER * Dnp), Hc(56);
  auto hidx = [&](int r, int cc) -> size_t {
    const size_t tb = ((size_t)(r >> 4) * h.tpr + ((r >> 4) - (cc >> 4))) * (kTS * kTS);
    if (h.tile_mode == 1) return tb + ((((r & 15) & 3) << 4) + (cc & 15)) * 4 + ((r & 15) >> 2);
    if (h.tile_mode == 2) return tb + ((((cc & 15) & 3) << 4) + (r & 15)) * 4 + ((cc & 15) >> 2);
    return (size_t)r * h.ldh + (cc - r + h.kd);
  };
  const dsh::SftGraph& g = *c->packed[b].g;
  std::vector<double> Hcomp;
  if (h.tile_mode == 1) {
    Hcomp.resize(g.hc_elems());
    HIPCHK(c, hipMemcpy(Hcomp.data(), h.Hc, 8 * Hcomp.size(), hipMemcpyDeviceToHost));
  } else {
    HIPCHK(c, hipMemcpy(Hb.data(), h.Hb, 8 * Hb.size(), hipMemcpyDeviceToHost));
  }
  auto hval = [&](int r, int cc) -> double {
    if (h.tile_mode != 1) return Hb[hidx(r, cc)];
    const int I = r >> 4, d = I - (cc >> 4);
    if (d > kBT) return 0.0;
    const int lane = (((r & 15) & 3) << 4) + (cc & 15), q = (r & 15) >> 2;
    return Hcomp[g.hgather[(((size_t)I * (kBT + 1) + d) * 64 + lane) * 4 + q] / 8];
  };
  HIPCHK(c, hipMemcpy(Hbord.data(), h.Hbord, 8 * Hbord.size(), hipMemcpyDeviceToHost));
  HIPCHK(c, hipMemcpy(Hc.data(), h.Hcorner, 8 * 49, hipMemcpyDeviceToHost));
  if (chi2) HIPCHK(c, hipMemcpy(chi2, h.dbg, 8, hipMemcpyDeviceToHost));
  if (H) {
    std::fill(H, H + (size_t)D * D, 0.0);
    for (int r = 0; r < h.Dn; r++)
      for (int k = 0; k <= h.kd; k++) {
        const int cidx = r - h.kd + k;
        if (cidx < 0) continue;
        const double v = hval(r, cidx);
        H[(size_t)(6 + r) + (size_t)(6 + cidx) * D] = v;
        H[(size_t)(6 + cidx) + (size_t)(6 + r) * D] = v;
      }
    for (int k = 0; k < 6; k++)
      for (int r = 0; r < h.Dn; r++) {
        const double v = Hbord[(size_t)k * Dnp + r];
        H[(size_t)k + (size_t)(6 + r) * D] = v;
        H[(size_t)(6 + r) + (size_t)k * D] = v;
      }
    for (int r = 0; r < 6; r++)
      for (int k = 0; k <= r; k++) {
        H[(size_t)r + (size_t)k * D] = Hc[r * 7 + k];
        H[(size_t)k + (size_t)r * D] = Hc[r * 7 + k];
      }
  }
  if (bvec) {
    for (int r = 0; r < 6; r++) bvec[r] = Hc[42 + r];
    for (int r = 0; r < h.Dn; r++) bvec[6 + r] = Hbord[(size_t)6 * Dnp + r];
  }
  return DSH_OK;
}
#endif

}
```

### defslam_amd/csrc/dsh_sft_ctx.h

```cpp
#pragma once
#include <hip/hip_runtime.h>

#include <memory>
#include <mutex>
#include <string>
#include <vector>

#include "../../include/defslam_hip.h"
#include "dsh_ctx.h"
#include "dsh_template.h"
#include "sft_pack.h"
#include "sft_plan.h"
#include "sft_problem.h"

struct LdsMarks { size_t lm[2] = {0, 0}, sc = 0, spec[2] = {0, 0}, cn = 0, b[2] = {0, 0}, tail = 0; };
extern LdsMarks g_lds_marks[64];
extern std::mutex g_lds_mu;
#define LDS_MARKS(c) (g_lds_marks[(c)->device & 63])
#define LDS_LOCK() std::lock_guard<std::mutex> lds_lock__(g_lds_mu)

struct Packed {
  SftDev h{};
  dsh::SftGraph* g = nullptr;
  dsh::SftFramePack f;
};

struct dsh_ctx : dsh_ctx_base {
  dsh::TemplateHost tmpl;
  char* d_tmpl = nullptr;
  size_t d_tmpl_bytes = 0;
  struct TemplateDev {
    const double *xyz0, *nbr_w, *nbr_sumw, *k0;
    const int32_t *nbr_ptr, *nbr_idx;
  } dt{};
  std::vector<std::unique_ptr<dsh::SftGraph>> graphs;
  uint64_t upload_serial = 0;
  int B = 0;
  std::vector<Packed> packed;
  SftBatchPlan plan;
  SftBatchLayout layout;
  char* d_batch = nullptr;
  size_t d_batch_cap = 0;
  SftDev* d_probs = nullptr;
  std::vector<SftDev> h_probs;
  HostBuf stage;
  hipEvent_t stage_free = nullptr;
  bool stage_busy = false;
  HostBuf results;
  char* d_sync = nullptr;
  int spec_hint = 12;
  SftSpec* d_spec = nullptr;
  HostBuf spec_done;
  SftSc* d_sc = nullptr;
  SftRun* d_runs = nullptr;
  int* d_counters = nullptr;
  int* d_linlist = nullptr;
  int rounds_hint = 24;
  hipStream_t sub_stream[kSftMaxSub] = {nullptr, nullptr, nullptr, nullptr};
  hipEvent_t sub_event[kSftMaxSub] = {nullptr, nullptr, nullptr, nullptr};
  std::vector<hipEvent_t>* phase_events = nullptr;
  std::vector<int> phase_ids;
  int num_cus = 256;
  bool ran = false;
  SftOptions opt;
};

int dsh_sft_upload(dsh_ctx* c, int B, const dsh_sft_frame* frames, SftUploadMode mode);
```

### defslam_amd/csrc/sft_batch.h

```cpp
#pragma once

#define SFTB_NW 8
#ifndef SFTB_LIN_NW
#define SFTB_LIN_NW 8
#endif
#ifndef SFTB_LIN_WAVES
#define SFTB_LIN_WAVES 2
#endif
#ifndef SFTB_TRIAL_WAVES
#define SFTB_TRIAL_WAVES 2
#endif

__device__ __forceinline__ void sftb_ctl_lds(char* smem, Ctl*& ctl, double*& red, double*& out, double*& panel) {
  ctl = reinterpret_cast<Ctl*>(smem);
  red = reinterpret_cast<double*>(smem + 512);
  out = red + 16 * 27 + 5;
  panel = out + 32;
}

__global__ __launch_bounds__(64 * SFTB_NW, 2) void sftb_init_kernel(const SftDev* __restrict__ probs, SftRun* __restrict__ runs, int* __restrict__ counters, int* __restrict__ lin_list, int tail_below) {
  const SftDev& P = probs[blockIdx.x];
  if (blockIdx.x == 0 && threadIdx.x == 0 && (int)gridDim.x <= tail_below) counters[6] = 1;
  init_state<64 * SFTB_NW>(P);
  if (threadIdx.x == 0) {
    SftRun& R = runs[blockIdx.x];
    R.lambda = -1.0; R.ni = 2.0; R.chi_cur = 0.0; R.chi_ini = 0.0; R.rho = 0.0; R.lambda_start = 0.0;
    R.it = 0; R.qmax = 0; R.nbad = 0; R.accepted = 0; R.all_ok = 1; R.iters = 0; R.trials = 0; R.fact_ok = 1;
    R.state = P.max_iters > 0 ? SFTB_LIN : SFTB_FINISH;
    if (P.max_iters > 0) lin_list[atomicAdd(&counters[2], 1)] = blockIdx.x;
  }
}

template <int NW>
__device__ __forceinline__ void sftb_lin_problem(const SftDev& P, SftRun& R, Ctl* ctl, double* red, double* out, double* panel) {
  constexpr int NT = 64 * NW;
  const int tid = threadIdx.x;
  auto nothing = [] {};
  const double chi0 = linearise<NW, decltype(nothing), true>(P, ctl, red, out, panel, nothing);
  double lambda = R.lambda;
  if (R.it == 0) {
    double mx = 0.0;
    for (int r = tid; r < P.Dn; r += NT) mx = fmax(mx, fabs(h_diag(P, r)));
    if (tid < 6) mx = fmax(mx, fabs(P.Hcorner[tid * 8]));
    mx = block_max(mx, red);
    lambda = 1e-5 * mx;
  }
  if (tid == 0) {
    if (R.it == 0) { R.lambda = lambda; R.ni = 2.0; R.nbad = 0; }
    R.chi_cur = chi0; R.chi_ini = chi0; R.qmax = 0; R.rho = 0.0; R.accepted = 0; R.all_ok = 1; R.lambda_start = lambda;
    R.state = SFTB_TRIAL;
  }
}

__global__ __launch_bounds__(64 * SFTB_LIN_NW, SFTB_LIN_WAVES) void sftb_lin_kernel(const SftDev* __restrict__ probs, SftRun* __restrict__ runs, int* __restrict__ counters,
                                                                                  const int* __restrict__ lin_list, int B, int tail_below) {
  constexpr int NW = SFTB_LIN_NW, NT = 64 * NW;
  extern __shared__ __attribute__((aligned(16))) char smem[];
  __shared__ int next_b;
  Ctl* ctl; double *red, *out, *panel;
  sftb_ctl_lds(smem, ctl, red, out, panel);
  const int tid = threadIdx.x;
  if (counters[6] || B - counters[0] <= tail_below) {
    if (blockIdx.x == 0 && tid == 0) counters[6] = 1;
    return;
  }
  if (blockIdx.x == 0 && tid == 0) counters[7]++;
  auto fetch = [&]() { const int i = atomicAdd(&counters[3], 1); return i < counters[2] ? lin_list[i] : -1; };
  int nxt = -1;
  if (tid == 0) nxt = fetch();
  while (true) {
    if (tid == 0) next_b = nxt;
    __syncthreads();
    const int b = __builtin_amdgcn_readfirstlane(next_b);
    if (b < 0) break;
    if (tid == 0) { nxt = fetch(); atomicAdd(&counters[9], 1); }
    sftb_lin_problem<NW>(probs[b], runs[b], ctl, red, out, panel);
  }
}

__global__ __launch_bounds__(64, 1) void sftb_factor_kernel(const SftDev* __restrict__ probs, SftRun* __restrict__ runs, int* __restrict__ counters, int B) {
  extern __shared__ __attribute__((aligned(16))) char smem[];
  lds_double* lds = to_lds(reinterpret_cast<double*>(smem));
  const int lane = threadIdx.x;
  if (counters[6]) return;
  for (int i = lane; i < WV_LDS_DOUBLES; i += 64) lds[i] = 0.0;
  if (blockIdx.x == 0 && lane == 0) { counters[2] = 0; counters[3] = 0; }
  WvPrev Q;
  Q.Lg = nullptr; Q.Linv = nullptr; Q.x = nullptr; Q.nT = 0; Q.active = 0; Q.xb = 0.0;
  int n_done = 0;
  while (true) {
    int b = 0;
    if (lane == 0) b = atomicAdd(&counters[1], 1);
    b = __builtin_amdgcn_readfirstlane(b);
    if (b >= B) break;
    if (runs[b].state != SFTB_TRIAL) continue;
    const SftDev& P = probs[b];
    const double lambda = runs[b].lambda;
    double xcam;
    const int ok = wv_factor(P, lambda, lambda, lds, Q, xcam);
    if (lane == 0) runs[b].fact_ok = ok;
    Q = wv_prev_of(P, ok, xcam, lane);
    n_done++;
  }
  int lane_now;
  asm volatile("v_mbcnt_lo_u32_b32 %0, -1, 0\n\tv_mbcnt_hi_u32_b32 %0, -1, %0" : "=v"(lane_now));
  if (Q.active) wv_backsub_now(Q, lane_now);
  if (lane_now == 0 && n_done) atomicAdd(&counters[8], n_done);
}

template <int NW>
__device__ __forceinline__ int sftb_trial_problem(const SftDev& P, SftRun& R, Ctl* ctl, double* red, double* out, double* panel, int* counters, int* lin_list, int b) {
  constexpr int NT = 64 * NW;
  const int tid = threadIdx.x;
  const int Dn = P.Dn;
  const int Dnp = ((Dn + NB - 1) / NB) * NB;
  const int ok = R.fact_ok;
  const double lam = R.lambda;
  const bool in_lds = P.lds_class >= 1;
  if (!in_lds)
    for (int i = tid; i < 3 * P.n; i += NT) {
      const double v = P.xyz[i];
      P.xyz_bak[i] = v;
      const int a = P.act[i / 3];
      if (a >= 0) P.xyz[i] = v + P.x[3 * a + (i % 3)];
    }
  if (tid < 7) R.pose_bak[tid] = P.pose[tid];
  __syncthreads();
  if (tid == 0) pose_oplus(P.pose, P.x + Dnp);
  double sc = 0.0;
  for (int r = tid; r < Dn; r += NT) { const double xv = P.x[r]; sc += xv * (lam * xv + P.Hbord[(size_t)6 * Dnp + r]); }
  if (tid < 6) { const double xv = P.x[Dnp + tid]; sc += xv * (lam * xv + P.Hcorner[42 + tid]); }
  __syncthreads();
  block_sum<1>(&sc, red, out);
  const double scale = out[0];
  __syncthreads();
  const auto staged = asm_records<NW, 1>(P, panel);
  const double chi_new = in_lds ? eval_edges<false, 1>(P, ctl, red, out, staged, P.x)
                                : eval_edges<false, 0>(P, ctl, red, out, asm_records<NW, 0>(P, panel));
  if (tid == 0) {
    const double tempChi = ok ? chi_new : DBL_MAX;
    double rho = (R.chi_cur - tempChi);
    rho /= (scale + 1e-3);
    R.rho = rho;
    if (rho > 0 && isfinite(tempChi)) {
      double alpha = 1. - pow((2 * rho - 1), 3);
      alpha = fmin(alpha, 2. / 3.);
      const double sf = fmax(1. / 3., alpha);
      R.lambda = lam * sf; R.ni = 2.0; R.chi_cur = tempChi; R.accepted = 1;
      ctl->stop = 0;
    } else {
      R.lambda = lam * R.ni; R.ni *= 2.0;
      ctl->stop = 1;
    }
    R.qmax++;
    R.all_ok &= ok;
    ctl->qmax = R.qmax;
    ctl->rho = rho;
  }
  __syncthreads();
  if (ctl->stop) {
    if (!in_lds)
      for (int i = tid; i < 3 * P.n; i += NT) P.xyz[i] = P.xyz_bak[i];
    if (tid < 7) P.pose[tid] = R.pose_bak[tid];
  } else if (in_lds) {
    for (int i = tid; i < 3 * P.n; i += NT) P.xyz[i] = staged.xyz_l[i];
  }
  const bool again = (ctl->rho < 0) && (ctl->qmax < 10);
  if (again) return 0;
  __syncthreads();
  if (tid == 0) {
    const int qmax = R.qmax;
    R.trials += qmax;
    R.iters++;
    if (P.trace) {
      double* t = P.trace + R.it * 8;
      t[0] = R.chi_ini; t[1] = R.lambda_start; t[2] = qmax; t[3] = R.chi_cur; t[4] = R.lambda; t[5] = R.rho; t[6] = R.accepted; t[7] = R.all_ok;
    }
    if (!R.all_ok) P.res->status |= 1;
    bool term = (qmax == 10) || (R.rho == 0);
    if (!term) {
      if ((R.chi_ini - R.chi_cur) * 1e3 < R.chi_ini) R.nbad++; else R.nbad = 0;
      term = R.nbad >= 3;
    }
    R.it++;
    if (R.it >= P.max_iters) term = true;
    ctl->nbad = term ? 1 : 0;
    ctl->it = R.iters;
    ctl->accepted = R.trials;
    R.state = term ? SFTB_DONE : SFTB_LIN;
    if (!term && lin_list) lin_list[atomicAdd(&counters[2], 1)] = b;
  }
  __syncthreads();
  if (ctl->nbad) {
    const int iters = ctl->it, trials = ctl->accepted;
    __syncthreads();
    classify<NT>(P, ctl, panel, iters, trials);
    if (tid == 0) atomicAdd(&counters[0], 1);
    return 2;
  }
  return 1;
}

__global__ __launch_bounds__(64 * SFTB_NW, SFTB_TRIAL_WAVES) void sftb_trial_kernel(const SftDev* __restrict__ probs, SftRun* __restrict__ runs, int* __restrict__ counters, int* __restrict__ lin_list) {
  constexpr int NW = SFTB_NW, NT = 64 * NW;
  SftRun& R = runs[blockIdx.x];
  const int st = R.state;
  if (counters[6]) return;
  if (blockIdx.x == 0 && threadIdx.x == 0) counters[1] = 0;
  if (st != SFTB_TRIAL && st != SFTB_FINISH) return;
  extern __shared__ __attribute__((aligned(16))) char smem[];
  const SftDev& P = probs[blockIdx.x];
  Ctl* ctl; double *red, *out, *panel;
  sftb_ctl_lds(smem, ctl, red, out, panel);
  const int tid = threadIdx.x;
  if (st == SFTB_FINISH) {
    classify<NT>(P, ctl, panel, 0, 0);
    if (tid == 0) { R.state = SFTB_DONE; atomicAdd(&counters[0], 1); }
    return;
  }
  (void)sftb_trial_problem<NW>(P, R, ctl, red, out, panel, counters, lin_list, blockIdx.x);
}

__device__ __noinline__ void sftb_solve8(const SftDev& P, unsigned ctl_off, unsigned ws_off, double lambda) {
  typedef __attribute__((address_space(3))) char lds_char;
  Ctl* ctl = reinterpret_cast<Ctl*>((char*)(lds_char*)(size_t)__builtin_amdgcn_readfirstlane(ctl_off));
  double* ws = reinterpret_cast<double*>((char*)(lds_char*)(size_t)__builtin_amdgcn_readfirstlane(ws_off));
  factor_tiles_df8<1>(P, ctl, ws, lambda, true);
  backsub_tiles<8>(P, ctl, ws);
}

__global__ __launch_bounds__(64 * SFTB_NW, SFT_WAVES_PER_EU) void sftb_tail_kernel(const SftDev* __restrict__ probs, SftRun* __restrict__ runs, int* __restrict__ counters, int B, int tail_below) {
  constexpr int NW = SFTB_NW, NT = 64 * NW;
  extern __shared__ __attribute__((aligned(16))) char smem[];
  Ctl* ctl; double *red, *out, *panel;
  sftb_ctl_lds(smem, ctl, red, out, panel);
  const int tid = threadIdx.x;
  if (!counters[6]) {
    if (B - counters[0] > tail_below) return;
    if (blockIdx.x == 0 && tid == 0) counters[6] = 1;
  }
  while (true) {
    __syncthreads();
    if (tid == 0) ctl->it = atomicAdd(&counters[5], 1);
    __syncthreads();
    const int b = __builtin_amdgcn_readfirstlane(ctl->it);
    __syncthreads();
    if (b >= B) break;
    SftRun& R = runs[b];
    const SftDev& P = probs[b];
    int st = R.state;
    if (st == SFTB_FINISH) {
      classify<NT>(P, ctl, panel, 0, 0);
      if (tid == 0) { R.state = SFTB_DONE; atomicAdd(&counters[0], 1); }
      continue;
    }
    while (st == SFTB_LIN || st == SFTB_TRIAL) {
      if (st == SFTB_LIN) {
        sftb_lin_problem<NW>(P, R, ctl, red, out, panel);
        __syncthreads();
      }
      if (tid == 0) ctl->lambda = R.lambda;
      __syncthreads();
      sftb_solve8(P, (unsigned)(size_t)(__attribute__((address_space(3))) char*)(char*)ctl, (unsigned)(size_t)(__attribute__((address_space(3))) char*)(char*)panel, R.lambda);
      if (tid == 0) R.fact_ok = ctl->fact_ok;
      __syncthreads();
      const int r = sftb_trial_problem<NW>(P, R, ctl, red, out, panel, counters, nullptr, b);
      __syncthreads();
      st = r == 0 ? SFTB_TRIAL : (r == 1 ? SFTB_LIN : SFTB_DONE);
    }
  }
}
```

### defslam_amd/csrc/sft_kernels.hip

```cpp
#include <hip/hip_runtime.h>
#include <type_traits>
#include <utility>
#include <algorithm>
#include <cstdio>
#include <cstdlib>
#include <math.h>
#include <float.h>
#define SFT_KERNEL_SOURCE
#include "sft_problem.h"
#include "tile_chol.h"

#define NB 32

#if defined(SFT_PHASE_TIMERS) && defined(DSH_LAB)
#define PH_T0() long long ph_t0__ = wall_clock64()
#define PH_ADD(slot)                                                          \
  do {                                                                        \
    const long long t1__ = wall_clock64();                                    \
    if (threadIdx.x == 0) P.dbg[slot] += (double)(t1__ - ph_t0__);            \
    ph_t0__ = t1__;                                                           \
  } while (0)
#define PH_RESET() ph_t0__ = wall_clock64()
#define AS_T0() long long as_t0__ = clock64()
#define AS_ADD(slot) do { const long long t1__ = clock64(); if (threadIdx.x == 0) P.dbg[slot] += (double)(t1__ - as_t0__); as_t0__ = t1__; } while (0)
#else
#define AS_T0() do {} while (0)
#define AS_ADD(slot) do {} while (0)
#define PH_T0() do {} while (0)
#define PH_ADD(slot) do {} while (0)
#define PH_RESET() do {} while (0)
#endif

#if defined(SFT_STEP_TRACE) && defined(DSH_LAB)
#define ST_MARK(ev) do { if (st_on && k == 40 && (threadIdx.x & 63) == 0) st_buf[(threadIdx.x >> 6) * 8 + (ev)] = (double)clock64(); } while (0)
#define ST_DONE() do {} while (0)
#define ST_BEGIN() lds_double* st_buf = to_lds(ws) + 5376; const bool st_on = P.dbg[8] < 0.5
#define ST_END() do { __syncthreads(); if (st_on && threadIdx.x < 64) P.dbg[16 + threadIdx.x] = st_buf[threadIdx.x]; if (threadIdx.x == 0) P.dbg[8] = 1.0; } while (0)
#else
#define ST_MARK(ev) do {} while (0)
#define ST_DONE() do {} while (0)
#define ST_BEGIN() do {} while (0)
#define ST_END() do {} while (0)
#endif

#define TS 16
#define TP 17
#define BT 8
#define TILE_LDS (TS * TP)


namespace {

__device__ __forceinline__ size_t tile_off(int I, int d) { return ((size_t)I * (BT + 1) + d) * (TS * TS); }

__device__ __forceinline__ int tile_elem(int row, int col) { return (((row & 3) << 4) + col) * 4 + (row >> 2); }

template <class PT>
__device__ __forceinline__ size_t h_index(const PT& P, int r, int c) {
  if (P.tile_mode == 1) return tile_off(r >> 4, (r >> 4) - (c >> 4)) + tile_elem(r & 15, c & 15);
  if (P.tile_mode == 2) return ((size_t)(r >> 4) * P.tpr + ((r >> 4) - (c >> 4))) * (TS * TS) + tile_elem(c & 15, r & 15);
  return (size_t)r * P.ldh + (c - r + P.kd);
}
struct SplitMap {
  int on, c0, s, n1p, pad, Dn, tpr0, tpr1;
  SFT_G double *H0, *H1;
};
template <class PT>
__device__ __forceinline__ SplitMap split_map(const PT& P) {
  return SplitMap{P.split, P.sp_c0, P.sp_s, P.sp_n1p, P.sp_pad, P.Dn, P.part[0].tpr, P.part[1].tpr, P.part[0].Hb, P.part[1].Hb};
}
__device__ __forceinline__ void split_target(const SplitMap& S, int r, int c, SFT_G double*& H, int& tpr, int& rr, int& cc) {
  if (r < S.c0 + S.s) { H = S.H0; tpr = S.tpr0; rr = r; cc = c; return; }
  const int rp = S.pad + (S.Dn - 1 - r);
  H = S.H1; tpr = S.tpr1; cc = rp;
  rr = (c >= S.c0 + S.s) ? S.pad + (S.Dn - 1 - c) : S.n1p + (S.s - 1 - (c - S.c0));
}
__device__ __forceinline__ size_t wide_elem(int tpr, int rr, int cc) {
  return ((size_t)(rr >> 4) * tpr + ((rr >> 4) - (cc >> 4))) * (TS * TS) + tile_elem(cc & 15, rr & 15);
}

template <class PT>
__device__ __forceinline__ double h_diag(const PT& P, int r) {
  if (P.tile_mode == 1) { const int a = r / 3, e = r - 3 * a; return P.Hc[9 * (size_t)(a + P.off_ptr[a]) + 4 * e]; }
  if (P.tile_mode == 2 && P.split) {
    SFT_G double* H; int tpr, rr, cc;
    split_target(split_map(P), r, r, H, tpr, rr, cc);
    return H[wide_elem(tpr, rr, cc)];
  }
  return P.Hb[h_index(P, r, r)];
}

struct Ctl {
  double R[9], t[3];
  double lambda, ni, chi_cur, chi_tmp, chi_ini, rho, scale;
  int fact_ok, qmax, nbad, stop, accepted, it;
};

__device__ __forceinline__ void quat_to_R(const double* q, double* R) {
  const double tx = 2 * q[0], ty = 2 * q[1], tz = 2 * q[2];
  const double twx = tx * q[3], twy = ty * q[3], twz = tz * q[3];
  const double txx = tx * q[0], txy = ty * q[0], txz = tz * q[0];
  const double tyy = ty * q[1], tyz = tz * q[1], tzz = tz * q[2];
  R[0] = 1 - (tyy + tzz); R[1] = txy - twz;       R[2] = txz + twy;
  R[3] = txy + twz;       R[4] = 1 - (txx + tzz); R[5] = tyz - twx;
  R[6] = txz - twy;       R[7] = tyz + twx;       R[8] = 1 - (txx + tyy);
}

__device__ void quat_from_R(const double* R, double* q) {
  double t = R[0] + R[4] + R[8];
  if (t > 0.0) {
    t = sqrt(t + 1.0);
    q[3] = 0.5 * t;
    t = 0.5 / t;
    q[0] = (R[7] - R[5]) * t;
    q[1] = (R[2] - R[6]) * t;
    q[2] = (R[3] - R[1]) * t;
  } else {
    int i = 0;
    if (R[4] > R[0]) i = 1;
    if (R[8] > R[i * 4]) i = 2;
    const int j = (i + 1) % 3, k = (j + 1) % 3;
    t = sqrt(R[i * 4] - R[j * 4] - R[k * 4] + 1.0);
    q[i] = 0.5 * t;
    t = 0.5 / t;
    q[3] = (R[k * 3 + j] - R[j * 3 + k]) * t;
    q[j] = (R[j * 3 + i] + R[i * 3 + j]) * t;
    q[k] = (R[k * 3 + i] + R[i * 3 + k]) * t;
  }
}

__device__ __forceinline__ void quat_unit_pos(double* q) {
  if (q[3] < 0) { q[0] = -q[0]; q[1] = -q[1]; q[2] = -q[2]; q[3] = -q[3]; }
  const double nrm = sqrt(q[0] * q[0] + q[1] * q[1] + q[2] * q[2] + q[3] * q[3]);
  q[0] /= nrm; q[1] /= nrm; q[2] /= nrm; q[3] /= nrm;
}

__device__ void pose_oplus(double* pose, const double* d) {
  const double om0 = d[0], om1 = d[1], om2 = d[2];
  const double theta = sqrt(om0 * om0 + om1 * om1 + om2 * om2);
  const double Om[9] = {0, -om2, om1, om2, 0, -om0, -om1, om0, 0};
  double Om2[9];
  for (int i = 0; i < 3; i++)
    for (int j = 0; j < 3; j++) {
      double s = 0;
      for (int k = 0; k < 3; k++) s += Om[i * 3 + k] * Om[k * 3 + j];
      Om2[i * 3 + j] = s;
    }
  double Rd[9], V[9];
  if (theta < 0.00001) {
    for (int i = 0; i < 9; i++) { Rd[i] = ((i % 4 == 0 ? 1.0 : 0.0) + Om[i]) + Om2[i]; V[i] = Rd[i]; }
  } else {
    const double a = sin(theta) / theta;
    const double b = (1 - cos(theta)) / (theta * theta);
    const double c = (theta - sin(theta)) / (theta * theta * theta);
    for (int i = 0; i < 9; i++) {
      const double id = (i % 4 == 0) ? 1.0 : 0.0;
      Rd[i] = (id + a * Om[i]) + b * Om2[i];
      V[i] = (id + b * Om[i]) + c * Om2[i];
    }
  }
  double qd[4], td[3];
  quat_from_R(Rd, qd);
// ... 2785 lines not shown
  if (e != hipSuccess) return e;
  if (nw == 4) hipLaunchKernelGGL(sft_assembly_kernel<4>, dim3(B), dim3(256), lds, stream, d_probs);
  else hipLaunchKernelGGL(sft_assembly_kernel<8>, dim3(B), dim3(512), lds, stream, d_probs);
  return hipGetLastError();
}
#endif

extern "C" hipError_t sft_sc_launch(const SftDev* d_probs, SftSc* d_sc, int B, int phase, int max_kd, size_t jl_doubles, size_t* configured, hipStream_t stream) {
  const size_t lds = sft_lm_kernel_lds_bytes(max_kd, jl_doubles);
  if (lds > *configured) {
    hipError_t e = hipFuncSetAttribute(reinterpret_cast<const void*>(sft_sc_kernel<8>), hipFuncAttributeMaxDynamicSharedMemorySize, (int)lds);
    if (e != hipSuccess) return e;
    *configured = lds;
  }
  hipLaunchKernelGGL(sft_sc_kernel<8>, dim3(B), dim3(512), lds, stream, d_probs, d_sc, phase);
  return hipGetLastError();
}

extern "C" hipError_t sft_cn_launch(const SftDev* d_probs, SftSc* d_sc, int phase, int max_kd, size_t jl_doubles, size_t* configured, hipStream_t stream) {
  const size_t lds = sft_lm_kernel_lds_bytes(max_kd, jl_doubles);
  if (lds > *configured) {
    hipError_t e = hipFuncSetAttribute(reinterpret_cast<const void*>(sft_cn_kernel<8>), hipFuncAttributeMaxDynamicSharedMemorySize, (int)lds);
    if (e != hipSuccess) return e;
    *configured = lds;
  }
  hipLaunchKernelGGL(sft_cn_kernel<8>, dim3(1), dim3(512), lds, stream, d_probs, d_sc, phase);
  return hipGetLastError();
}

extern "C" hipError_t sftb_tail_launch(const SftDev* d_probs, SftRun* d_runs, int* d_counters, int B, int max_kd, size_t jl_doubles, size_t* configured, int num_cus, int tail_below, hipStream_t stream) {
  const size_t lds = sft_lm_kernel_lds_bytes(max_kd, jl_doubles);
  if (lds > *configured) {
    hipError_t e = hipFuncSetAttribute(reinterpret_cast<const void*>(sftb_tail_kernel), hipFuncAttributeMaxDynamicSharedMemorySize, (int)lds);
    if (e != hipSuccess) return e;
    *configured = lds;
  }
  hipLaunchKernelGGL(sftb_tail_kernel, dim3(std::min(B, num_cus)), dim3(64 * SFTB_NW), lds, stream, d_probs, d_runs, d_counters, B, tail_below);
  return hipGetLastError();
}

#ifdef DSH_LAB
__global__ __launch_bounds__(1024) void sft_part_factor_kernel(const SftDev* __restrict__ probs, SftSpec* __restrict__ specs, int K, int nh) {
  constexpr int NT = 1024;
  extern __shared__ __attribute__((aligned(16))) char smem[];
  const int roles = 1 + nh, per_role = gridDim.x / roles;
  const int role = blockIdx.x / per_role, bid = blockIdx.x % per_role;
  const int fpart = bid % 2, bx = bid / 2;
  const int B = per_role / (K * 2), b = bx / K, j = bx % K;
  const SftDev& P = probs[(size_t)j * B + b];
  const SftSpec& S = specs[(size_t)j * B + b];
  Ctl* ctl = reinterpret_cast<Ctl*>(smem);
  double* red = reinterpret_cast<double*>(smem + 512);
  double* panel = red + 16 * 27 + 5 + 32;
  const int tid = threadIdx.x;
  if (S.done) return;
  if (!(P.tile_mode == 2 && P.split) || S.need_lin == 1) return;
  if (S.qbase + j >= 10) return;
  const int epoch = S.launches + 1;
  if (role > 0) {
    factor_wide_helper<16>(P, fpart, role - 1, nh, epoch, ctl, panel);
    return;
  }
  double lam = S.lambda, ni = S.ni;
  if (S.need_lin == 2 && S.it == 0) {
    double mx = 0.0;
    for (int r = tid; r < P.Dn; r += NT) mx = fmax(mx, fabs(h_diag(P, r)));
    if (tid < 6) mx = fmax(mx, fabs(P.Hcorner[tid * 8]));
    mx = block_max(mx, red);
    lam = 1e-5 * mx; ni = 2.0;
  }
  for (int t = 0; t < j; t++) { lam *= ni; ni *= 2.0; }
  if (tid == 0) ctl->lambda = lam;
  __syncthreads();
  factor_part<SFT_WIDE_NEAR, 16>(P, fpart, ctl, panel, epoch, nh);
}
#endif

__global__ void sft_vec_sum2_kernel(const double* a, const double* b, double* out_a, double* out_b, int n) {
  for (int i = blockIdx.x * blockDim.x + threadIdx.x; i < n; i += gridDim.x * blockDim.x) {
    const double v = a[i] + b[i];
    out_a[i] = v;
    out_b[i] = v;
  }
}
extern "C" hipError_t sft_vec_sum2(const double* a, const double* b, double* out_a, double* out_b, int n, hipStream_t stream) {
  hipLaunchKernelGGL(sft_vec_sum2_kernel, dim3(64), dim3(256), 0, stream, a, b, out_a, out_b, n);
  return hipGetLastError();
}

extern "C" hipError_t sft_spec_launch(const SftDev* d_probs, SftSpec* d_spec, int B, int K, int phase, int nh, int owner_waves, int max_kd, size_t jl_doubles, size_t* configured, hipStream_t stream) {
  const size_t lds = sft_lm_kernel_lds_bytes(max_kd, jl_doubles);
#ifdef DSH_LAB
  if (phase == SFT_SPEC_FACTOR && nh > 0 && owner_waves == 16) {
    if (lds > configured[1]) {
      hipError_t e = hipFuncSetAttribute(reinterpret_cast<const void*>(sft_part_factor_kernel), hipFuncAttributeMaxDynamicSharedMemorySize, (int)lds);
      if (e != hipSuccess) return e;
      configured[1] = lds;
    }
    hipLaunchKernelGGL(sft_part_factor_kernel, dim3(B * K * 2 * (1 + nh)), dim3(1024), lds, stream, d_probs, d_spec, K, nh);
    return hipGetLastError();
  }
#endif
  if (lds > *configured) {
    hipError_t e = hipFuncSetAttribute(reinterpret_cast<const void*>(sft_spec_kernel<8>), hipFuncAttributeMaxDynamicSharedMemorySize, (int)lds);
    if (e != hipSuccess) return e;
    *configured = lds;
  }
  const int wgs = (phase == SFT_SPEC_FACTOR || phase == SFT_SPEC_SOLVE) ? 2 : 1, roles = phase == SFT_SPEC_FACTOR ? 1 + nh : 1;
  hipLaunchKernelGGL(sft_spec_kernel<8>, dim3(B * K * wgs * roles), dim3(512), lds, stream, d_probs, d_spec, K, phase, nh);
  return hipGetLastError();
}

__global__ void sft_sc_local_reduce_kernel(SftSc* const* scs, int G) {
  const int i = threadIdx.x;
  if (i >= SFT_SC_XCHG) return;
  double s = 0.0;
  for (int g = 0; g < G; g++) s += scs[g]->send[i];
  for (int g = 0; g < G; g++) scs[g]->recv[i] = s;
}
extern "C" hipError_t sft_sc_local_reduce(SftSc* const* d_ptrs, int G, hipStream_t stream) {
  hipLaunchKernelGGL(sft_sc_local_reduce_kernel, dim3(1), dim3(64), 0, stream, d_ptrs, G);
  return hipGetLastError();
}

extern "C" hipError_t sft_lm_launch(const SftDev* d_probs, int B, int max_kd, size_t jl_doubles, int nw, size_t* configured, hipStream_t stream) {
  const size_t lds = sft_lm_kernel_lds_bytes(max_kd, jl_doubles);
  const int slot = nw == 4 ? 0 : 1;
  if (lds > configured[slot]) {
    const void* fn = nw == 4 ? reinterpret_cast<const void*>(sft_lm_kernel<4>) : reinterpret_cast<const void*>(sft_lm_kernel<8>);
    hipError_t e = hipFuncSetAttribute(fn, hipFuncAttributeMaxDynamicSharedMemorySize, (int)lds);
    if (e != hipSuccess) return e;
    configured[slot] = lds;
  }
  if (nw == 4) hipLaunchKernelGGL(sft_lm_kernel<4>, dim3(B), dim3(256), lds, stream, d_probs);
  else hipLaunchKernelGGL(sft_lm_kernel<8>, dim3(B), dim3(512), lds, stream, d_probs);
  return hipGetLastError();
}

#ifdef DSH_LAB
extern "C" hipError_t sft_wave_lab_launch(const SftDev* d_probs, int B, int which, double rel, int max_kd, size_t jl_doubles, hipStream_t stream) {
  if (which == 0) {
    (void)jl_doubles;
    const size_t lds = sft_lm_kernel_lds_bytes(max_kd, 0);
    hipError_t e = hipFuncSetAttribute(reinterpret_cast<const void*>(sft_ref_solve_kernel<4>), hipFuncAttributeMaxDynamicSharedMemorySize, (int)lds);
    if (e != hipSuccess) return e;
    hipLaunchKernelGGL(sft_ref_solve_kernel<4>, dim3(B), dim3(256), lds, stream, d_probs, rel);
  } else {
    hipLaunchKernelGGL(sft_wave_solve_kernel, dim3(B), dim3(64), WV_LDS_DOUBLES * sizeof(double), stream, d_probs);
  }
  return hipGetLastError();
}
#endif

extern "C" hipError_t sftb_launch(const SftDev* d_probs, SftRun* d_runs, int* d_counters, int* d_list, int B, int phase, size_t jl_doubles, size_t xyz_doubles, size_t* configured, int num_cus, int tail_below, hipStream_t stream) {
  const size_t head = 512 + (16 * 27 + 5 + 32) * sizeof(double) + 64;
  if (phase == SFTB_PH_INIT) {
    hipError_t e = hipMemsetAsync(d_counters, 0, 16 * sizeof(int), stream);
    if (e != hipSuccess) return e;
    hipLaunchKernelGGL(sftb_init_kernel, dim3(B), dim3(64 * SFTB_NW), 0, stream, d_probs, d_runs, d_counters, d_list, tail_below);
  } else if (phase == SFTB_PH_LIN) {
    const size_t lds = head + jl_doubles * sizeof(double);
    if (lds > configured[0]) {
      hipError_t e = hipFuncSetAttribute(reinterpret_cast<const void*>(sftb_lin_kernel), hipFuncAttributeMaxDynamicSharedMemorySize, (int)lds);
      if (e != hipSuccess) return e;
      configured[0] = lds;
    }
    const int per_cu = lds > 80 * 1024 ? 1 : 2;
    hipLaunchKernelGGL(sftb_lin_kernel, dim3(std::min(B, per_cu * num_cus)), dim3(64 * SFTB_LIN_NW), lds, stream, d_probs, d_runs, d_counters, d_list, B, tail_below);
  } else if (phase == SFTB_PH_FACTOR) {
    hipLaunchKernelGGL(sftb_factor_kernel, dim3(std::min(B, 4 * num_cus)), dim3(64), WV_LDS_DOUBLES * sizeof(double), stream, d_probs, d_runs, d_counters, B);
  } else {
    const size_t lds = head + std::max<size_t>(2048, xyz_doubles) * sizeof(double);
    if (lds > configured[1]) {
      hipError_t e = hipFuncSetAttribute(reinterpret_cast<const void*>(sftb_trial_kernel), hipFuncAttributeMaxDynamicSharedMemorySize, (int)lds);
      if (e != hipSuccess) return e;
      configured[1] = lds;
    }
    hipLaunchKernelGGL(sftb_trial_kernel, dim3(B), dim3(64 * SFTB_NW), lds, stream, d_probs, d_runs, d_counters, d_list);
  }
  return hipGetLastError();
}

#ifdef DSH_LAB
extern "C" hipError_t sftb_factor_lab_launch(const SftDev* d_probs, SftRun* d_runs, int* d_counters, int B, int grid, hipStream_t stream) {
  hipLaunchKernelGGL(sftb_factor_kernel, dim3(grid), dim3(64), WV_LDS_DOUBLES * sizeof(double), stream, d_probs, d_runs, d_counters, B);
  return hipGetLastError();
}
#endif
```

### defslam_amd/csrc/sft_plan.cpp

```cpp
#include "sft_plan.h"

#include <algorithm>

namespace {

void set_tile_mode(SftProblemPlan& p, int kd, int tile_mode) {
  p.tile_mode = tile_mode;
  p.wbt = tile_mode == 1 ? kBT : (tile_mode == 2 ? (kd + kTS - 1) / kTS : 0);
  p.tpr = tile_mode ? p.wbt + 1 : 0;
}

void set_cut(SftProblemPlan& p, const SftSizes& z, const SftCut& cut) {
  const int sT = cut.sT, n1p = ((cut.n1 + kTS - 1) / kTS) * kTS;
  p.split = 1; p.sp_c0 = cut.c0; p.sp_s = cut.sp; p.sp_n1p = n1p; p.sp_pad = n1p - cut.n1;
  SftPart& p0 = p.part[0]; SftPart& p1 = p.part[1]; SftPart& p2 = p.part[2];
  p0 = SftPart{}; p1 = SftPart{}; p2 = SftPart{};
  p0.nS = cut.c0 / kTS; p0.nT = p0.nS + sT; p0.tpr = p.tpr; p0.wbt = p.wbt; p0.b_base = 0; p0.b_sign = 1; p0.b_lo = 0; p0.b_hi = cut.c0 + cut.sp;
  p1.nS = n1p / kTS; p1.nT = p1.nS + sT; p1.tpr = p.tpr; p1.wbt = p.wbt; p1.b_base = z.Dn - 1 + p.sp_pad; p1.b_sign = -1; p1.b_lo = p.sp_pad; p1.b_hi = n1p;
  p2.nS = sT; p2.nT = sT; p2.wbt = sT - 1; p2.tpr = sT;
  p.sp_xl = sT * p2.tpr * kTS * kTS + 8 * kTS * sT + 64;
  p.part[3] = p2;
}

}

SftBatchPlan sft_plan_batch(const SftSizes* sizes, int B, int num_cus, const SftOptions& opt, bool host_only, SftUploadMode mode) {
  const bool one_lane = mode != SftUploadMode::batch;
  const bool force_split = mode == SftUploadMode::connected;
  SftBatchPlan plan;
  plan.prob.resize(B);
  bool all_tiles = true;
  for (int b = 0; b < B; b++) {
    const int kd = sizes[b].kd;
    set_tile_mode(plan.prob[b], kd, (kd <= kTS * kBT) ? 1 : ((kd <= kTS * kWB && !opt.wide_off) ? 2 : 0));
    all_tiles = all_tiles && plan.prob[b].tile_mode == 1;
    plan.max_iters_batch = std::max(plan.max_iters_batch, (int)sizes[b].max_iters);
  }
  if (all_tiles && 2 * B > num_cus) plan.nw = 4;
  if ((opt.waves == 4 && all_tiles) || opt.waves == 8) plan.nw = opt.waves;
  if (one_lane) plan.nw = 8;
  plan.rounds_mode = all_tiles && plan.nw == 4 && opt.waves == 0 && opt.rounds != 0 && !host_only;
  if (plan.rounds_mode) {
    const int want = opt.streams > 0 ? opt.streams : 1;
    while (plan.n_sub < want && plan.n_sub < kSftMaxSub && B / (plan.n_sub + 1) >= 16 * num_cus) plan.n_sub++;
    if (opt.streams > 0) plan.n_sub = std::min(std::min(opt.streams, kSftMaxSub), std::max(1, B / 64));
  }
  int K = 1;
  if (plan.nw == 8 && !one_lane && !host_only) {
    K = (4 * B <= num_cus) ? 4 : ((3 * B <= num_cus) ? 3 : ((2 * B <= num_cus) ? 2 : 1));
    bool wide = opt.split != 0 && opt.helpers != 0;
    for (int b = 0; b < B; b++) {
      const SftCut cut = sft_cut(sizes[b].Dn, sizes[b].kd);
      const int packed_tile_mode = plan.prob[b].tile_mode;
      wide = wide && packed_tile_mode == 2 && cut.sT >= opt.helpers_wbt && cut.room;
    }
    if (wide && K == 4 && (long long)B * 4 * 2 * 3 > num_cus && (long long)B * 2 * 2 * 3 <= num_cus) K = 2;
    if (opt.speculate >= 1 && opt.speculate <= SFT_SPEC_MAXK) K = opt.speculate;
    for (int b = 0; b < B; b++) if (sizes[b].max_iters < 1) K = 1;
  }
  plan.K = K;
  const size_t lds_budget = ((((plan.nw == 4 && !plan.rounds_mode) || SFT_WAVES_PER_EU >= 4) ? 75 : 155) * 1024) / 8;
  for (int b = 0; b < B; b++) {
    const SftSizes& z = sizes[b];
    SftProblemPlan& p = plan.prob[b];
    if ((force_split && p.tile_mode == 1) ||
        (K > 1 && p.tile_mode == 1 && opt.split >= 2 && 20 * B <= num_cus && z.kd > kTS && z.Dn >= 8 * kTS * ((z.kd + kTS - 1) / kTS))) {
      set_tile_mode(p, z.kd, 2);
    }
    p.dataflow = p.tile_mode == 1 && opt.dataflow;
    if ((force_split || (K > 1 && opt.split)) && p.tile_mode == 2) {
      const SftCut cut = sft_cut(z.Dn, z.kd);
      if (cut.room) set_cut(p, z, cut);
    }
    size_t used = 0;
    const size_t need1 = ((3 * (size_t)z.n + 1) & ~(size_t)1) + (((size_t)z.M + 1) & ~(size_t)1) + 4 * (size_t)z.S, need2 = need1 + 6 * (size_t)z.nA + 4 * (size_t)z.Es;
    const size_t need3 = need2 + 5 * (size_t)z.M;
    p.lds_class = (plan.rounds_mode && used + need3 <= lds_budget) ? 3 : (used + need2 <= lds_budget) ? 2 : ((used + need1 <= lds_budget) ? 1 : 0);
    used += p.lds_class == 3 ? need3 : p.lds_class == 2 ? need2 : (p.lds_class == 1 ? need1 : 0);
    plan.jl_doubles = std::max(plan.jl_doubles, used);
    if (p.lds_class >= 1) plan.xyz_doubles = std::max(plan.xyz_doubles, ((3 * (size_t)z.n + 1) & ~(size_t)1));
    plan.max_kd = std::max(plan.max_kd, p.tile_mode == 2 ? std::max((int)z.kd, kTS * kBT + 1) : (int)z.kd);
    plan.any_split = plan.any_split || p.split != 0;
  }
  bool any = false;
  for (int b = 0; b < B; b++) any = any || (plan.prob[b].split != 0 && plan.prob[b].wbt >= opt.helpers_wbt);
  for (int b = 0; b < B; b++)
    if (plan.prob[b].split && std::max(plan.prob[b].part[0].nT, plan.prob[b].part[1].nT) >= 60000) any = false;
  if (any && K > 1 && !force_split) {
    while (plan.nh < 3 && (long long)B * K * 2 * (2 + plan.nh) <= num_cus) plan.nh++;
    if (plan.nh == 1) plan.nh = 0;
    if (opt.helpers >= 0) plan.nh = opt.helpers;
  }
  return plan;
}
```

### defslam_amd/csrc/sft_plan.h

```cpp
#pragma once
#include <stddef.h>
#include <stdint.h>

#include <vector>

#include "sft_problem.h"

constexpr int kNB = 32;
constexpr int kTS = 16, kBT = 8, kWB = 16;
constexpr int kSftMaxSub = 4;

struct SftOptions { int waves = 0; int dataflow = 1; int wide_off = 0; int speculate = 0; int split = 2; int rounds = 1; int streams = 0; int helpers = -1; int tail = -1; int owner_waves = 8; int helpers_wbt = 12; };

enum class SftUploadMode { batch, shared_camera, connected };

struct SftSizes { int32_t n, nA, Dn, kd, M, S, Es, max_iters; };

struct SftCut {
  int sT, sp, c0, n1;
  bool room;
};
inline SftCut sft_cut(int Dn, int kd) {
  SftCut c;
  c.sT = (kd + kTS - 1) / kTS;
  c.sp = kTS * c.sT;
  c.c0 = ((Dn - c.sp) / 2 / kTS) * kTS;
  c.n1 = Dn - c.sp - c.c0;
  c.room = c.sT >= 2 && c.c0 >= 4 * kTS && c.n1 >= 4 * kTS;
  return c;
}

struct SftProblemPlan {
  int32_t tile_mode = 0, wbt = 0, tpr = 0;
  bool dataflow = false;
  int32_t lds_class = 0;
  int32_t split = 0, sp_c0 = 0, sp_s = 0, sp_n1p = 0, sp_pad = 0, sp_xl = 0;
  SftPart part[4] = {};
  void apply(SftDev& h) const {
    h.tile_mode = tile_mode; h.wbt = wbt; h.tpr = tpr;
    h.mode = (h.mode & ~2) | (dataflow ? 2 : 0);
    h.lds_class = lds_class;
    h.split = split; h.sp_c0 = sp_c0; h.sp_s = sp_s; h.sp_n1p = sp_n1p; h.sp_pad = sp_pad; h.sp_xl = sp_xl;
    for (int g = 0; g < 4; g++) h.part[g] = part[g];
  }
};

struct SftBatchPlan {
  int nw = 8;
  bool rounds_mode = false;
  int n_sub = 1;
  int K = 1;
  int nh = 0;
  bool any_split = false;
  int max_kd = 0;
  size_t jl_doubles = 0;
  size_t xyz_doubles = 0;
  int max_iters_batch = 0;
  std::vector<SftProblemPlan> prob;
};

SftBatchPlan sft_plan_batch(const SftSizes* sizes, int B, int num_cus, const SftOptions& opt, bool host_only, SftUploadMode mode);

struct SftBatchLayout {
  struct ReadOnly { size_t obs_nodes, obs_bary, obs_uv, obs_w, ob_ptr, ob_m, ob_c, viewed, xyz_init, pose_init; };
  struct Result { size_t xyz, chi2, trace, mp, outl; };
  struct Part { size_t Hb, Lb, Lt, LbT, Lbord, Linv, x, xchg, Pf, PfB, sync; };
  struct Work { size_t bak, camrec, wtv, Anode, Jstar, Jstr, Hc, Hb, Hbord, Hcn, Lb, Lbord, Lc, Linv, Lt, LbT, x, dbg, sx0, sx1, shadow_xyz, shadow_chi2, shadow_hdr; Part part[4]; };
  size_t o_tab = 0;
  std::vector<ReadOnly> ro;
  size_t ro_bytes = 0;
  size_t res_off = 0, res_bytes = 0;
  std::vector<Result> res_offs;
  size_t ws_off = 0;
  size_t o_spec = 0;
  size_t o_runs = 0;
  size_t o_sync = 0, sync_total = 0;
  std::vector<Work> ws;
  size_t size = 0;
};
```

### defslam_amd/csrc/sft_problem.h

```cpp
#pragma once
#include <stdint.h>

#define SFT_NT 512
#define SFT_CAM_STRIDE 16
#define SFT_BORDER 7
#define SFT_H_PAD_TILE_ROWS 9
#define SFT_H_PAD_BORDER 160

#define SFT_KIND_OBS 0u
#define SFT_KIND_REF 1u
#define SFT_KIND_STAR 2u
#define SFT_KIND_STR 3u
#define SFT_REC(kind, s, t, e) (((uint32_t)(kind) << 30) | ((uint32_t)(s) << 26) | ((uint32_t)(t) << 22) | (uint32_t)(e))

#if defined(__HIP_DEVICE_COMPILE__) && defined(SFT_KERNEL_SOURCE)
#define SFT_G __attribute__((address_space(1)))
#else
#define SFT_G
#endif

struct SftResHdr {
  int32_t iters, trials, status, inliers;
  double rep_error;
  double pose[8];
  double pad[5];
};

#define SFT_SC_XCHG 32
#define SFT_SC_LIN 0
#define SFT_SC_FAC 1
#define SFT_SC_SOL 2
#define SFT_SC_CTL 3
#define SFT_CN_LIN 0
#define SFT_CN_FAC 1
#define SFT_CN_SOL 2
#define SFT_CN_CTL 3
struct SftSc {
  double send[SFT_SC_XCHG], recv[SFT_SC_XCHG];
  double lambda, ni, chi_cur, chi_ini, rho, lambda_start;
  double bc[6];
  double pose_bak[8];
  int32_t it, qmax, nbad, accepted, again, done, all_ok, fact_ok, iters, trials, rank, nranks;
};

#define SFT_SPEC_MAXK 4
#define SFT_SPEC_INIT 0
#define SFT_SPEC_LIN 1
#define SFT_SPEC_TRIAL 2
#ifndef SFT_WAVES_PER_EU
#define SFT_WAVES_PER_EU 2
#endif
#define SFT_SPEC_FACTOR 3
#define SFT_SPEC_SOLVE 4
struct SftSpecRes { double chi_new, scale, lambda, ni, pose[8]; int32_t ok, valid; };
struct SftSpec {
  double lambda, ni, chi_cur, chi_ini, lambda_start, rho;
  double pose_bak[8];
  int32_t it, qbase, nbad, accepted, all_ok, iters, trials, done, launches, need_lin, last_lane, pad;
  SftSpecRes res[2];
};

#define SFTB_LIN 0
#define SFTB_TRIAL 1
#define SFTB_DONE 2
#define SFTB_FINISH 3
#define SFTB_PH_INIT 0
#define SFTB_PH_LIN 1
#define SFTB_PH_FACTOR 2
#define SFTB_PH_TRIAL 3
#define SFTB_PH_TAIL 4
struct SftRun {
  double lambda, ni, chi_cur, chi_ini, rho, lambda_start;
  double pose_bak[8];
  int32_t it, qmax, nbad, accepted, all_ok, iters, trials, state, fact_ok, pad[3];
};

struct SftPart {
  int32_t nT, nS, tpr, wbt;
  int32_t b_base, b_sign, b_lo, b_hi;
  SFT_G double* Hb;
  SFT_G double *Lb, *Lt, *LbT, *Lbord, *Linv, *x;
  SFT_G double* xchg;
  SFT_G double *Pf, *PfB;
  SFT_G int32_t* sync;
};

struct SftDev {
  int32_t n, nA, Dn, kd, ldh, M, V, S, Es, noff, max_iters, mode;
  int32_t tile_mode;
  int32_t pad1;
  int32_t lds_class;
  int32_t tpr, wbt;
  int32_t pad0;
  double fx, fy, cx, cy;
  double w_ref, w_curv, w_str, hub_delta, hub_dsqr;
  const SFT_G double* xyz0;
  const SFT_G int32_t* nbr_ptr;
  const SFT_G int32_t* nbr_idx;
  const SFT_G double* nbr_w;
  const SFT_G double* nbr_sumw;
  const SFT_G double* k0;
  const SFT_G int32_t* act;
  const SFT_G int32_t* actnode;
  const SFT_G int32_t* star_node;
  const SFT_G double* star_sL;
  const SFT_G int32_t* str_nodes;
  const SFT_G double* str_L0;
  const SFT_G int32_t* off_ptr;
  const SFT_G int32_t* off_rc;
  const SFT_G int32_t* sh_ptr;
  const SFT_G uint32_t* sh_rec;
  const SFT_G double* sh_cf;
  const SFT_G int32_t* tmask;
  const SFT_G uint32_t* hgatherT;
  const SFT_G uint32_t* hgather;
  const SFT_G int32_t* obs_nodes;
  const SFT_G double* obs_bary;
  const SFT_G double* obs_uv;
  const SFT_G double* obs_w;
  const SFT_G int32_t* ob_ptr;
  const SFT_G int32_t* ob_m;
  const SFT_G double* ob_c;
  const SFT_G uint8_t* viewed;
  const SFT_G double* xyz_init;
  const SFT_G double* pose_init;
  SFT_G double* xyz;
  SFT_G double* xyz_bak;
  SFT_G double* pose;
  SFT_G double* camrec;
  SFT_G double* wtv;
  SFT_G double* Anode;
  SFT_G double* Jstar;
  SFT_G double* Jstr;
  SFT_G double* Hc;
  SFT_G double* Hb;
  SFT_G double* Hbord;
  SFT_G double* Hcorner;
  SFT_G double* Lb;
  SFT_G double* Lbord;
  SFT_G double* Lcorner;
  SFT_G double* Linv;
  SFT_G double* Lt;
  SFT_G double* LbT;
  SFT_G double* x;
  SFT_G double* chi2_obs;
  SFT_G double* trace;
  SFT_G SftResHdr* res;
  SFT_G uint8_t* outlier;
  SFT_G float* mappoint;
  SFT_G double* dbg;
  SFT_G double* spec_xyz[2];
  int32_t split;
  int32_t sp_c0, sp_s, sp_n1p, sp_pad;
  int32_t sp_xl;
  int32_t pad2[2];
  SftPart part[4];
};

#include <hip/hip_runtime.h>
#include <stddef.h>
extern "C" size_t sft_lm_kernel_lds_bytes(int kd, size_t jl_doubles);
extern "C" hipError_t sft_lm_launch(const SftDev* d_probs, int B, int max_kd, size_t jl_doubles, int nw, size_t* configured, hipStream_t stream);
extern "C" hipError_t sftb_launch(const SftDev* d_probs, SftRun* d_runs, int* d_counters, int* d_list, int B, int phase, size_t jl_doubles, size_t xyz_doubles,
                                  size_t* configured, int num_cus, int tail_below, hipStream_t stream);
extern "C" hipError_t sftb_tail_launch(const SftDev* d_probs, SftRun* d_runs, int* d_counters, int B, int max_kd, size_t jl_doubles, size_t* configured, int num_cus,
                                       int tail_below, hipStream_t stream);
extern "C" hipError_t sft_spec_launch(const SftDev* d_probs, SftSpec* d_spec, int B, int K, int phase, int nh, int owner_waves, int max_kd, size_t jl_doubles,
                                      size_t* configured, hipStream_t stream);
extern "C" hipError_t sft_sc_launch(const SftDev* d_probs, SftSc* d_sc, int B, int phase, int max_kd, size_t jl_doubles, size_t* configured, hipStream_t stream);
extern "C" hipError_t sft_sc_local_reduce(SftSc* const* d_ptrs, int G, hipStream_t stream);
extern "C" hipError_t sft_cn_launch(const SftDev* d_probs, SftSc* d_sc, int phase, int max_kd, size_t jl_doubles, size_t* configured, hipStream_t stream);
extern "C" hipError_t sft_vec_sum2(const double* a, const double* b, double* out_a, double* out_b, int n, hipStream_t stream);
#ifdef DSH_LAB
extern "C" hipError_t sft_wave_lab_launch(const SftDev* d_probs, int B, int which, double rel, int max_kd, size_t jl_doubles, hipStream_t stream);
extern "C" hipError_t sft_assembly_launch(const SftDev* d_probs, int B, int max_kd, size_t jl_doubles, int nw, hipStream_t stream);
extern "C" hipError_t sftb_factor_lab_launch(const SftDev* d_probs, SftRun* d_runs, int* d_counters, int B, int grid, hipStream_t stream);
#endif
```

### defslam_amd/sft.py

```python
from __future__ import annotations

import ctypes as C
from dataclasses import dataclass, field
from typing import List, Optional, Sequence

import numpy as np

from . import _lib


class DshError(RuntimeError):
    pass


def _ptr(a: Optional[np.ndarray], ctype):
    if a is None:
        return None
    return a.ctypes.data_as(C.POINTER(ctype))


@dataclass
class Frame:
    Tcw: np.ndarray
    K: np.ndarray
    N: int
    obs_nodes: np.ndarray
    obs_bary: np.ndarray
    obs_uv: np.ndarray
    obs_invsig2: np.ndarray
    nodes_xyz: np.ndarray
    mvbOutlier: np.ndarray = field(default=None)
    repError: float = 0.0
    mappoints: np.ndarray = field(default=None)
    pose7: np.ndarray = field(default=None)
    chi2_obs: np.ndarray = field(default=None)
    iters: int = 0
    trials: int = 0
    dim: int = 0
    half_bandwidth: int = 0
    status: int = 0
    trace: np.ndarray = field(default=None)
    regs: Optional[tuple] = None


class Context:

    def __init__(self, device: int = 0, lab: bool = False):
        self.lab = bool(lab)
        self._L = _lib.load_lab() if lab else _lib.load()
        h = C.c_void_p()
        rc = self._L.dsh_create(C.byref(h), device)
        if rc != _lib.DSH_OK:
            raise DshError(f"dsh_create failed with status {rc} (no gfx950 device visible?)")
        self._h = h
        self.n = 0
        self._keep = None

    def close(self):
        if getattr(self, "_events", None) is not None:
            self._events.close()
            self._events = None
        if getattr(self, "_h", None):
            self._L.dsh_destroy(self._h)
            self._h = None

    def __del__(self):
        try:
            self.close()
        except Exception:
            pass

    def _check(self, rc: int, what: str):
        if rc != _lib.DSH_OK:
            raise DshError(f"{what}: status {rc}: {self._L.dsh_last_error(self._h).decode()}")

    def template_build(self, xyz0: np.ndarray, facets: np.ndarray):
        xyz0 = np.ascontiguousarray(xyz0, np.float64)
        facets = np.ascontiguousarray(facets, np.int32)
        self._check(self._L.dsh_template_build(self._h, xyz0.shape[0], _ptr(xyz0, C.c_double), facets.shape[0], _ptr(facets, C.c_int32)),
                    "dsh_template_build")
        self.n = xyz0.shape[0]

    def template_set(self, xyz0, boundary, nbr_ptr, nbr_idx, nbr_w, k0, edge_nodes, edge_L0, median_L):
        xyz0 = np.ascontiguousarray(xyz0, np.float64)
        boundary = np.ascontiguousarray(boundary, np.uint8)
        nbr_ptr = np.ascontiguousarray(nbr_ptr, np.int32)
        nbr_idx = np.ascontiguousarray(nbr_idx, np.int32)
        nbr_w = np.ascontiguousarray(nbr_w, np.float64)
        k0 = np.ascontiguousarray(k0, np.float64)
        edge_nodes = np.ascontiguousarray(edge_nodes, np.int32)
        edge_L0 = np.ascontiguousarray(edge_L0, np.float64)
        self._check(self._L.dsh_template_set(self._h, xyz0.shape[0], _ptr(xyz0, C.c_double), _ptr(boundary, C.c_uint8), _ptr(nbr_ptr, C.c_int32),
                                             _ptr(nbr_idx, C.c_int32), _ptr(nbr_w, C.c_double), _ptr(k0, C.c_double), edge_L0.shape[0],
                                             _ptr(edge_nodes, C.c_int32), _ptr(edge_L0, C.c_double), float(median_L)), "dsh_template_set")
        self.n = xyz0.shape[0]

    def template_get(self) -> dict:
        n, E, nnz = C.c_int32(), C.c_int32(), C.c_int32()
        self._check(self._L.dsh_template_dims(self._h, C.byref(n), C.byref(E), C.byref(nnz)), "dsh_template_dims")
        out = dict(boundary=np.zeros(n.value, np.uint8), nbr_ptr=np.zeros(n.value + 1, np.int32), nbr_idx=np.zeros(nnz.value, np.int32),
                   nbr_w=np.zeros(nnz.value), k0=np.zeros(n.value), edge_nodes=np.zeros((E.value, 2), np.int32), edge_L0=np.zeros(E.value))
        med = C.c_double()
        self._check(self._L.dsh_template_get(self._h, _ptr(out["boundary"], C.c_uint8), _ptr(out["nbr_ptr"], C.c_int32), _ptr(out["nbr_idx"], C.c_int32),
                                             _ptr(out["nbr_w"], C.c_double), _ptr(out["k0"], C.c_double), _ptr(out["edge_nodes"], C.c_int32),
                                             _ptr(out["edge_L0"], C.c_double), C.byref(med)), "dsh_template_get")
        out["median_L"] = med.value
        return out

    def template_embed(self, pts: np.ndarray):
        pts = np.ascontiguousarray(pts, np.float32)
        P = pts.shape[0]
        fid = np.zeros(P, np.int32)
        nodes = np.zeros((P, 3), np.int32)
        bary = np.zeros((P, 3), np.float32)
        self._check(self._L.dsh_template_embed(self._h, P, _ptr(pts, C.c_float), _ptr(fid, C.c_int32), _ptr(nodes, C.c_int32), _ptr(bary, C.c_float)),
                    "dsh_template_embed")
        return fid, nodes, bary

    def template_embed_device(self, pts: np.ndarray):
        pts = np.ascontiguousarray(pts, np.float32)
        P = pts.shape[0]
        fid = np.zeros(P, np.int32)
        nodes = np.zeros((P, 3), np.int32)
        bary = np.zeros((P, 3), np.float32)
        self._check(self._L.dsh_template_embed_device(self._h, P, _ptr(pts, C.c_float), _ptr(fid, C.c_int32), _ptr(nodes, C.c_int32), _ptr(bary, C.c_float)),
                    "dsh_template_embed_device")
        return fid, nodes, bary

    def _frame_c(self, f: Frame, reg_lap, reg_inex, reg_temp, layers, max_iters, keep: list) -> _lib.SftFrameC:
        Tcw = np.ascontiguousarray(f.Tcw, np.float32)
        nodes = np.ascontiguousarray(f.obs_nodes, np.int32)
        bary = np.ascontiguousarray(f.obs_bary, np.float64)
        uv = np.ascontiguousarray(f.obs_uv, np.float64)
        isg = np.ascontiguousarray(f.obs_invsig2, np.float64)
        xyz = np.ascontiguousarray(f.nodes_xyz, np.float64)
        keep += [Tcw, nodes, bary, uv, isg, xyz]
        fc = _lib.SftFrameC()
        fc.Tcw = _ptr(Tcw, C.c_float)
        for i in range(4):
            fc.K[i] = float(f.K[i])
        fc.n_frame = int(f.N)
        fc.M = int(nodes.shape[0])
        fc.obs_nodes = _ptr(nodes, C.c_int32)
        fc.obs_bary = _ptr(bary, C.c_double)
        fc.obs_uv = _ptr(uv, C.c_double)
        fc.obs_invsig2 = _ptr(isg, C.c_double)
        fc.xyz = _ptr(xyz, C.c_double)
        if f.regs is not None:
            reg_lap, reg_inex, reg_temp = f.regs
        fc.reg_lap, fc.reg_inex, fc.reg_temp = float(reg_lap), float(reg_inex), float(reg_temp)
        fc.neighbour_layers = int(layers)
        fc.max_iters = int(max_iters)
        return fc

    def batch_upload(self, frames: Sequence[Frame], RegLap=5000.0, RegInex=5000.0, RegTemp=0.0, NeighboursLayers=1, max_iters=50):
        keep: list = []
        arr = (_lib.SftFrameC * len(frames))()
        for i, f in enumerate(frames):
            arr[i] = self._frame_c(f, RegLap, RegInex, RegTemp, NeighboursLayers, max_iters, keep)
        self._check(self._L.dsh_sft_batch_upload(self._h, len(frames), arr), "dsh_sft_batch_upload")
        self._frames = list(frames)
        self._max_iters = max_iters

    def batch_run(self):
        self._check(self._L.dsh_sft_batch_run(self._h), "dsh_sft_batch_run")

    def batch_run_timed(self, launches: int = 1) -> float:
        if getattr(self, "_events", None) is None:
            self._events = _lib.HipEvents()
        st = self.stream()
        self._events.start(st)
        for _ in range(int(launches)):
            self.batch_run()
        return self._events.stop_ms(st)

    def _need_lab(self, what: str):
        if not self.lab:
            raise DshError(f"{what} is a lab entry point (include/defslam_hip_debug.h): create the context with Context(device, lab=True)")

    def set_option(self, name: str, value: int):
        self._need_lab("dsh_lab_set_option")
        self._check(self._L.dsh_lab_set_option(self._h, name.encode(), int(value)), "dsh_lab_set_option")

    def solver_info(self, b: int = 0) -> dict:
        self._need_lab("dsh_lab_sft_solver_info")
        o = (C.c_int32 * 8)()
        self._check(self._L.dsh_lab_sft_solver_info(self._h, int(b), o), "dsh_lab_sft_solver_info")
        return dict(split=int(o[0]), c0=int(o[1]), s=int(o[2]), n1p=int(o[3]), pad=int(o[4]), lanes=int(o[5]), tile_mode=int(o[6]), waves=int(o[7]))

    def lab_run_timed(self, launches: int = 1) -> float:
        self._need_lab("dsh_lab_sft_run_timed")
        ms = C.c_double()
        self._check(self._L.dsh_lab_sft_run_timed(self._h, int(launches), C.byref(ms)), "dsh_lab_sft_run_timed")
        return ms.value

    def batch_assemble_timed(self, launches: int = 1) -> float:
        self._need_lab("dsh_lab_sft_assemble_timed")
        ms = C.c_double()
        self._check(self._L.dsh_lab_sft_assemble_timed(self._h, int(launches), C.byref(ms)), "dsh_lab_sft_assemble_timed")
        return ms.value

    def wave_check(self, rel: float = 1.0, launches: int = 1, only: int = 0):
        self._need_lab("dsh_lab_sft_wave_check")
        B = len(self._frames)
        dims = []
        for b in range(B):
            _, counts = self.problem_info(b)
            Dn = int(counts[5]) - 6
            dims.append(((Dn + 31) // 32) * 32 + 6)
        tot = int(sum(dims))
        xr, xn = np.zeros(tot), np.zeros(tot)
        ok = np.zeros((B, 2), np.int32)
        ms = np.zeros(2)
        self._check(self._L.dsh_lab_sft_wave_check(self._h, C.c_double(rel), int(launches), int(only), _ptr(xr, C.c_double), _ptr(xn, C.c_double), _ptr(ok, C.c_int32),
                                                   _ptr(ms, C.c_double)), "dsh_lab_sft_wave_check")
        offs = np.concatenate([[0], np.cumsum(dims)])
        return [xr[offs[b]:offs[b + 1]] for b in range(B)], [xn[offs[b]:offs[b + 1]] for b in range(B)], ok, ms

    def factor_check(self, lam, factor=None, grid: int = 0):
        self._need_lab("dsh_lab_sft_factor_check")
        B = len(self._frames)
        lam = np.ascontiguousarray(lam, np.float64)
        if lam.shape != (B,):
            raise ValueError(f"factor_check: lam must have one damping per problem ({B})")
        fac = None if factor is None else np.ascontiguousarray(np.asarray(factor, bool).astype(np.uint8))
        if fac is not None and fac.shape != (B,):
            raise ValueError(f"factor_check: factor must have one flag per problem ({B})")
        dims = []
        for b in range(B):
            Dn = int(self.problem_info(b)[1][5]) - 6
            dims.append(((Dn + 31) // 32) * 32 + 6)
        x = np.zeros(int(sum(dims)))
        ok = np.zeros(B, np.int32)
        self._check(self._L.dsh_lab_sft_factor_check(self._h, _ptr(lam, C.c_double), _ptr(fac, C.c_uint8), int(grid), _ptr(x, C.c_double),
                                                     _ptr(ok, C.c_int32)), "dsh_lab_sft_factor_check")
        offs = np.concatenate([[0], np.cumsum(dims)])
        return [x[offs[b]:offs[b + 1]] for b in range(B)], ok

    def rounds_timed(self):
        self._need_lab("dsh_lab_sft_rounds_timed")
        ms = np.zeros(7)
        r = np.zeros(1, np.int32)
        self._check(self._L.dsh_lab_sft_rounds_timed(self._h, _ptr(ms, C.c_double), _ptr(r, C.c_int32)), "dsh_lab_sft_rounds_timed")
        return dict(init=float(ms[0]), lin=float(ms[1]), factor=float(ms[2]), trial=float(ms[3]), tail=float(ms[4]), factorisations_in_rounds=int(ms[5]), linearisations_in_rounds=int(ms[6])), int(r[0])

    def dump(self, b: int, what: int, n: int):
        self._need_lab("dsh_lab_sft_dump")
        out = np.zeros(int(n))
        self._check(self._L.dsh_lab_sft_dump(self._h, int(b), int(what), int(n), _ptr(out, C.c_double)), "dsh_lab_sft_dump")
        return out

    def phase_ms(self, b: int = 0):
        self._need_lab("dsh_lab_sft_phase_ms")
        out = np.zeros(8)
        self._check(self._L.dsh_lab_sft_phase_ms(self._h, b, _ptr(out, C.c_double)), "dsh_lab_sft_phase_ms")
        return dict(trsm=out[0], residuals=out[1], assembly=out[2], copy=out[3], panel=out[4], update=out[5], backsub=out[6], control=out[7])

    def step_trace(self, b: int = 0):
        self._need_lab("dsh_lab_sft_step_trace")
        out = np.zeros(64)
        self._check(self._L.dsh_lab_sft_step_trace(self._h, b, _ptr(out, C.c_double)), "dsh_lab_sft_step_trace")
        return out.reshape(8, 8)

    def synchronize(self):
        self._check(self._L.dsh_synchronize(self._h), "dsh_synchronize")

    def stream(self) -> int:
        return int(self._L.dsh_stream(self._h) or 0)

    def batch_counts(self):
        it, tr = C.c_int64(), C.c_int64()
        self._check(self._L.dsh_sft_batch_counts(self._h, C.byref(it), C.byref(tr)), "dsh_sft_batch_counts")
        return it.value, tr.value

    def problem_info(self, b: int):
        nbytes = C.c_int64()
        counts = np.zeros(9, np.int32)
        self._check(self._L.dsh_sft_batch_problem_info(self._h, b, C.byref(nbytes), _ptr(counts, C.c_int32)), "dsh_sft_batch_problem_info")
        return nbytes.value, counts

    def batch_download(self, only=None) -> List[int]:
        frames = self._frames
        res = (_lib.SftResultC * len(frames))()
        keep = []
        want = None if only is None else set(int(i) for i in only)
        for i, f in enumerate(frames):
            if want is not None and i not in want:
                keep.append(None)
                continue
            M, n = f.obs_nodes.shape[0], f.nodes_xyz.shape[0]
            bufs = dict(Tcw=np.zeros((4, 4), np.float32), pose7=np.zeros(7), xyz=np.zeros((n, 3)), chi2=np.zeros(M), outl=np.zeros(M, np.uint8),
                        mp=np.zeros((M, 3), np.float32), trace=np.zeros((max(self._max_iters, 1), _lib.DSH_TRACE_STRIDE)))
            keep.append(bufs)
            r = res[i]
            r.Tcw = _ptr(bufs["Tcw"], C.c_float)
            r.pose7 = _ptr(bufs["pose7"], C.c_double)
            r.xyz = _ptr(bufs["xyz"], C.c_double)
            r.chi2_obs = _ptr(bufs["chi2"], C.c_double)
            r.outlier = _ptr(bufs["outl"], C.c_uint8)
            r.mappoint_xyz = _ptr(bufs["mp"], C.c_float)
            r.trace = _ptr(bufs["trace"], C.c_double)
        self._check(self._L.dsh_sft_batch_download(self._h, len(frames), res), "dsh_sft_batch_download")
        out = []
        for i, f in enumerate(frames):
            b, r = keep[i], res[i]
            if b is None:
                f.iters, f.trials, f.dim, f.half_bandwidth, f.status = r.iters, r.trials, r.dim, r.half_bandwidth, r.status
                out.append(int(r.inliers))
                continue
            f.Tcw = b["Tcw"]
            f.pose7 = b["pose7"]
            f.nodes_xyz = b["xyz"]
            f.chi2_obs = b["chi2"]
            f.mvbOutlier = b["outl"].astype(bool)
            f.mappoints = b["mp"]
            f.repError = float(np.float32(r.rep_error))
            f.rep_error_f64 = r.rep_error
            f.iters, f.trials, f.dim, f.half_bandwidth, f.status = r.iters, r.trials, r.dim, r.half_bandwidth, r.status
            f.trace = b["trace"][:r.iters].copy()
            out.append(int(r.inliers))
        return out

    def prepare_solve(self, f: Frame, RegLap=5000.0, RegInex=5000.0, RegTemp=0.0, NeighboursLayers=1, max_iters=50):
        keep: list = []
        fc = self._frame_c(f, RegLap, RegInex, RegTemp, NeighboursLayers, max_iters, keep)
        M, n = f.obs_nodes.shape[0], f.nodes_xyz.shape[0]
        b = dict(Tcw=np.zeros((4, 4), np.float32), pose7=np.zeros(7), xyz=np.zeros((n, 3)), chi2=np.zeros(M), outl=np.zeros(M, np.uint8),
                 mp=np.zeros((M, 3), np.float32), trace=np.zeros((max(max_iters, 1), _lib.DSH_TRACE_STRIDE)))
        r = _lib.SftResultC()
        r.Tcw = _ptr(b["Tcw"], C.c_float)
        r.pose7 = _ptr(b["pose7"], C.c_double)
        r.xyz = _ptr(b["xyz"], C.c_double)
        r.chi2_obs = _ptr(b["chi2"], C.c_double)
        r.outlier = _ptr(b["outl"], C.c_uint8)
        r.mappoint_xyz = _ptr(b["mp"], C.c_float)
        r.trace = _ptr(b["trace"], C.c_double)
        ctx = self

        class _Call:
            frame = f

            def __call__(self_inner) -> int:
                rc = ctx._L.dsh_sft_solve(ctx._h, C.byref(fc), C.byref(r))
                if rc != _lib.DSH_OK:
                    ctx._check(rc, "dsh_sft_solve")
                f.Tcw, f.pose7, f.nodes_xyz, f.chi2_obs, f.mappoints = b["Tcw"], b["pose7"], b["xyz"], b["chi2"], b["mp"]
                f.mvbOutlier = b["outl"].view(np.bool_)
                f.repError = float(np.float32(r.rep_error))
                f.rep_error_f64 = r.rep_error
                f.iters, f.trials, f.dim, f.half_bandwidth, f.status = r.iters, r.trials, r.dim, r.half_bandwidth, r.status
                f.trace = b["trace"][:r.iters]
                return int(r.inliers)

        call = _Call()
        call._keep = (keep, b, fc, r)
        return call

    def debug_system(self, b: int, D: int):
        self._need_lab("dsh_lab_sft_system")
        H = np.zeros((D, D), order="F")
        bv = np.zeros(D)
        chi = C.c_double()
        self._check(self._L.dsh_lab_sft_system(self._h, b, D, _ptr(H, C.c_double), _ptr(bv, C.c_double), C.byref(chi)), "dsh_lab_sft_system")
        return H, bv, chi.value


def DefPoseOptimization(ctx: Context, pFrame: Frame, RegLap: float = 5000, RegInex: float = 5000, RegTemp: float = 0,
                        NeighboursLayers: int = 1, max_iters: int = 50) -> int:
    ctx.batch_upload([pFrame], RegLap, RegInex, RegTemp, NeighboursLayers, max_iters)
    ctx.batch_run()
    return ctx.batch_download()[0]


def DefPoseOptimizationBatch(ctx: Context, frames: Sequence[Frame], RegLap: float = 5000, RegInex: float = 5000, RegTemp: float = 0,
                             NeighboursLayers: int = 1, max_iters: int = 50) -> List[int]:
    ctx.batch_upload(frames, RegLap, RegInex, RegTemp, NeighboursLayers, max_iters)
    ctx.batch_run()
    return ctx.batch_download()


def _result_buffers(f: Frame, max_iters: int):
    M, n = f.obs_nodes.shape[0], f.nodes_xyz.shape[0]
    b = dict(Tcw=np.zeros((4, 4), np.float32), pose7=np.zeros(7), xyz=np.zeros((n, 3)), chi2=np.zeros(M), outl=np.zeros(M, np.uint8),
             mp=np.zeros((M, 3), np.float32), trace=np.zeros((max(max_iters, 1), _lib.DSH_TRACE_STRIDE)))
    r = _lib.SftResultC()
    r.Tcw = _ptr(b["Tcw"], C.c_float)
    r.pose7 = _ptr(b["pose7"], C.c_double)
    r.xyz = _ptr(b["xyz"], C.c_double)
    r.chi2_obs = _ptr(b["chi2"], C.c_double)
    r.outlier = _ptr(b["outl"], C.c_uint8)
    r.mappoint_xyz = _ptr(b["mp"], C.c_float)
    r.trace = _ptr(b["trace"], C.c_double)
    return b, r


def _write_back(f: Frame, b: dict, r) -> int:
    f.Tcw, f.pose7, f.nodes_xyz, f.chi2_obs, f.mappoints = b["Tcw"], b["pose7"], b["xyz"], b["chi2"], b["mp"]
    f.mvbOutlier = b["outl"].astype(bool)
    f.repError = float(np.float32(r.rep_error))
    f.rep_error_f64 = r.rep_error
    f.iters, f.trials, f.dim, f.half_bandwidth, f.status = r.iters, r.trials, r.dim, r.half_bandwidth, r.status
    f.trace = b["trace"][:r.iters].copy()
    return int(r.inliers)


def comm_unique_id() -> bytes:
    buf = C.create_string_buffer(_lib.DSH_COMM_ID_BYTES)
    if _lib.load().dsh_comm_unique_id(buf) != _lib.DSH_OK:
        raise DshError("dsh_comm_unique_id failed (RCCL not available?)")
    return buf.raw


class Comm:

    def __init__(self, ctx: Context, nranks: int, rank: int, unique_id: bytes):
        self._ctx = ctx
        h = C.c_void_p()
        buf = C.create_string_buffer(bytes(unique_id), _lib.DSH_COMM_ID_BYTES)
        ctx._check(ctx._L.dsh_comm_create(ctx._h, int(nranks), int(rank), buf, C.byref(h)), "dsh_comm_create")
        self._h = h
        self.nranks, self.rank = int(nranks), int(rank)

    def close(self):
        if getattr(self, "_h", None):
            self._ctx._L.dsh_comm_destroy(self._h)
            self._h = None


def SharedCameraPoseOptimization(ctx: Context, comm: Comm, pFrame: Frame, RegLap: float = 5000, RegInex: float = 5000, RegTemp: float = 0,
                                 NeighboursLayers: int = 1, max_iters: int = 50) -> int:
    keep: list = []
    fc = ctx._frame_c(pFrame, RegLap, RegInex, RegTemp, NeighboursLayers, max_iters, keep)
    b, r = _result_buffers(pFrame, max_iters)
    ctx._check(ctx._L.dsh_sft_shared_solve(ctx._h, comm._h, C.byref(fc), C.byref(r)), "dsh_sft_shared_solve")
    return _write_back(pFrame, b, r)


def SharedCameraPoseOptimizationGroup(ctxs: Sequence[Context], frames: Sequence[Frame], RegLap: float = 5000, RegInex: float = 5000, RegTemp: float = 0,
                                      NeighboursLayers: int = 1, max_iters: int = 50) -> List[int]:
    G = len(ctxs)
    keep: list = []
    fcs = (_lib.SftFrameC * G)()
    res = (_lib.SftResultC * G)()
    bufs = []
    for g in range(G):
        fcs[g] = ctxs[g]._frame_c(frames[g], RegLap, RegInex, RegTemp, NeighboursLayers, max_iters, keep)
        b, r = _result_buffers(frames[g], max_iters)
        bufs.append(b)
        res[g] = r
    hs = (C.c_void_p * G)(*[c._h for c in ctxs])
    ctxs[0]._check(ctxs[0]._L.dsh_sft_shared_solve_group(G, hs, fcs, res), "dsh_sft_shared_solve_group")
    return [_write_back(frames[g], bufs[g], res[g]) for g in range(G)]


def ConnectedPoseOptimization(ctx: Context, comm: Comm, pFrame: Frame, RegLap: float = 5000, RegInex: float = 5000, RegTemp: float = 0,
                              NeighboursLayers: int = 1, max_iters: int = 50) -> int:
    keep: list = []
    fc = ctx._frame_c(pFrame, RegLap, RegInex, RegTemp, NeighboursLayers, max_iters, keep)
    b, r = _result_buffers(pFrame, max_iters)
    ctx._check(ctx._L.dsh_sft_connected_solve(ctx._h, comm._h, C.byref(fc), C.byref(r)), "dsh_sft_connected_solve")
    return _write_back(pFrame, b, r)


def ConnectedPoseOptimizationGroup(ctx0: Context, ctx1: Context, frames: Sequence[Frame], RegLap: float = 5000, RegInex: float = 5000, RegTemp: float = 0,
                                   NeighboursLayers: int = 1, max_iters: int = 50) -> List[int]:
    keep: list = []
    fc = ctx0._frame_c(frames[0], RegLap, RegInex, RegTemp, NeighboursLayers, max_iters, keep)
    res = (_lib.SftResultC * 2)()
    bufs = []
    for g in range(2):
        b, r = _result_buffers(frames[g], max_iters)
        bufs.append(b)
        res[g] = r
    ctx0._check(ctx0._L.dsh_sft_connected_solve_group(ctx0._h, ctx1._h, C.byref(fc), res), "dsh_sft_connected_solve_group")
    return [_write_back(frames[g], bufs[g], res[g]) for g in range(2)]


def two_sided_cut(Dn: int, kd: int):
    sT = -(-kd // 16)
    s = 16 * sT
    c0 = ((Dn - s) // 2 // 16) * 16
    n1 = Dn - s - c0
    if sT < 2 or c0 < 64 or n1 < 64:
        return None
    n1p = -(-n1 // 16) * 16
    return c0, s, n1p, n1p - n1


def frame_from_synth(fr) -> Frame:
    return Frame(Tcw=fr.Tcw.copy(), K=fr.K.copy(), N=fr.n_frame, obs_nodes=fr.obs_nodes, obs_bary=fr.obs_bary, obs_uv=fr.obs_uv,
                 obs_invsig2=fr.obs_invsig2, nodes_xyz=fr.xyz.copy())
```

### include/defslam_hip_debug.h

```cpp
#ifndef DEFSLAM_HIP_DEBUG_H
#define DEFSLAM_HIP_DEBUG_H

#include "defslam_hip.h"

#ifdef __cplusplus
extern "C" {
#endif
#if defined(__GNUC__)
#pragma GCC visibility push(default)
#endif

int dsh_lab_set_option(dsh_ctx* ctx, const char* name, int value);
int dsh_lab_sft_solver_info(dsh_ctx* ctx, int b, int32_t* out8);

int dsh_lab_sft_run_timed(dsh_ctx* ctx, int launches, double* total_ms);
int dsh_lab_sft_assemble_timed(dsh_ctx* ctx, int launches, double* total_ms);
int dsh_lab_sft_wave_check(dsh_ctx* ctx, double rel, int launches, int only, double* x_ref, double* x_new, int32_t* ok2, double* ms2);
int dsh_lab_sft_factor_check(dsh_ctx* ctx, const double* lambda, const uint8_t* factor, int grid, double* x, int32_t* ok);
int dsh_lab_sft_rounds_timed(dsh_ctx* ctx, double* ms7, int32_t* rounds);
int dsh_lab_sft_dump(dsh_ctx* ctx, int b, int what, int64_t n, double* out);
int dsh_lab_sft_phase_ms(dsh_ctx* ctx, int b, double* out8);
int dsh_lab_sft_step_trace(dsh_ctx* ctx, int b, double* out64);
int dsh_lab_sft_system(dsh_ctx* ctx, int b, int32_t D, double* H, double* bvec, double* chi2);

#if defined(__GNUC__)
#pragma GCC visibility pop
#endif
#ifdef __cplusplus
}
#endif
#endif
```

Before: 422,100.

## Plan factor rounds to full wave sets, carrying small remainders to next round

Adds a PLAN kernel to each round. It compacts the problems that are still running into a rotating factor list and takes only whole multiples of the factor wave count when the remainder is small (up to tau). The rest wait for the next round. The intent is to avoid a FACTOR launch whose last wave set is mostly idle, which wastes a full factorisation latency on a few problems. In exchange each round gets an extra kernel launch and some problems converge later, so the worst-case round count is doubled.

```diff
diff --git a/defslam_amd/_lib.py b/defslam_amd/_lib.py
--- a/defslam_amd/_lib.py
+++ b/defslam_amd/_lib.py
@@ -213,7 +213,7 @@
 
 LAB_SYMBOLS = ["dsh_lab_set_option", "dsh_lab_sft_run_timed", "dsh_lab_sft_assemble_timed", "dsh_lab_sft_phase_ms", "dsh_lab_sft_step_trace",
                "dsh_lab_sft_system", "dsh_lab_sft_solver_info", "dsh_lab_sft_wave_check", "dsh_lab_sft_dump", "dsh_lab_sft_rounds_timed",
-               "dsh_lab_sft_factor_check"]
+               "dsh_lab_sft_factor_check", "dsh_lab_sft_round_schedule"]
 
 _lib = None
 _lab = None
@@ -372,6 +372,7 @@
         L.dsh_lab_sft_dump.argtypes = [vp, C.c_int, C.c_int, C.c_int64, c_double_p]
         L.dsh_lab_sft_rounds_timed.argtypes = [vp, c_double_p, c_i32_p]
         L.dsh_lab_sft_factor_check.argtypes = [vp, c_double_p, c_u8_p, C.c_int, c_double_p, c_i32_p]
+        L.dsh_lab_sft_round_schedule.argtypes = [c_i32_p, C.c_int32, C.c_int32, C.c_int32, C.c_int32, C.POINTER(C.c_int64), c_i32_p, c_i32_p, c_i32_p, C.c_int32]
         for name in LAB_SYMBOLS:
             getattr(L, name).restype = C.c_int
     return L
diff --git a/defslam_amd/csrc/dsh_api.cpp b/defslam_amd/csrc/dsh_api.cpp
--- a/defslam_amd/csrc/dsh_api.cpp
+++ b/defslam_amd/csrc/dsh_api.cpp
@@ -164,6 +164,9 @@
     if (c->opt.tail > 0) tail_below = c->opt.tail * c->num_cus;
     else tail_below = std::min(4 * c->num_cus, std::max(2 * c->num_cus, (int)((long long)3 * B / 4)));
   }
+  auto waves_of = [&](int n) { return std::min(n, c->opt.factor_waves > 0 ? c->opt.factor_waves : 4 * c->num_cus); };
+  auto tau_of = [&](int W) { return (S > 1 || c->opt.carry == 0) ? 0 : c->opt.carry > 0 ? c->opt.carry : sft_round_tau(W); };
+  int rounds = 0;
   auto launch = [&](int s, int phase) {
     const bool ev = c->phase_events && S == 1;
     if (ev) { hipEvent_t e; if (hipEventCreate(&e) == hipSuccess) { (void)hipEventRecord(e, c->stream); c->phase_events->push_back(e); c->phase_ids.push_back(phase); } }
@@ -172,7 +175,7 @@
       LDS_LOCK();
       if (phase == SFTB_PH_TAIL) r = sftb_tail_launch(c->d_probs + b0[s], c->d_runs + b0[s], c->d_counters + 16 * s, b0[s + 1] - b0[s], c->plan.max_kd, c->plan.jl_doubles, &LDS_MARKS(c).tail, c->num_cus, tail_below, c->sub_stream[s]);
       else r = sftb_launch(c->d_probs + b0[s], c->d_runs + b0[s], c->d_counters + 16 * s, c->d_linlist + b0[s], b0[s + 1] - b0[s], phase, c->plan.jl_doubles, c->plan.xyz_doubles, LDS_MARKS(c).b,
-                           c->num_cus, tail_below, c->sub_stream[s]);
+                           c->num_cus, tail_below, c->d_faclist + b0[s], c->d_running + b0[s], waves_of(b0[s + 1] - b0[s]), tau_of(waves_of(b0[s + 1] - b0[s])), rounds + 1, c->sub_stream[s]);
     }
     if (ev) { hipEvent_t e; if (hipEventCreate(&e) == hipSuccess) { (void)hipEventRecord(e, c->stream); c->phase_events->push_back(e); } }
     return r;
@@ -182,8 +185,8 @@
     for (int s = 1; s < S; s++) HIPCHK(c, hipStreamWaitEvent(c->sub_stream[s], c->sub_event[0], 0));
   }
   for (int s = 0; s < S; s++) HIPCHK(c, launch(s, SFTB_PH_INIT));
-  const int worst = std::max(1, c->plan.max_iters_batch) * 10 + 1;
-  int rounds = 0, group = std::max(1, std::min(worst, c->rounds_hint));
+  const int worst = 2 * (std::max(1, c->plan.max_iters_batch) * 10 + 1);
+  int group = std::max(1, std::min(worst, c->rounds_hint));
   if (tail_below >= B) group = 0;
   HIPCHK(c, c->spec_done.ensure(64 * kSftMaxSub, true));
   int rc = DSH_OK;
@@ -191,6 +194,7 @@
     for (int i = 0; i < group && rounds < worst; i++, rounds++)
       for (int s = 0; s < S; s++) {
         HIPCHK(c, launch(s, SFTB_PH_LIN));
+        HIPCHK(c, launch(s, SFTB_PH_PLAN));
         HIPCHK(c, launch(s, SFTB_PH_FACTOR));
         HIPCHK(c, launch(s, SFTB_PH_TRIAL));
       }
@@ -276,7 +280,7 @@
   L.ws.resize((size_t)B * K);
   L.ws_off = a.size;
   L.o_spec = a.take(sizeof(SftSpec) * (size_t)B * K);
-  L.o_runs = a.take(plan.rounds_mode ? sizeof(SftRun) * (size_t)B + 64 * kSftMaxSub + sizeof(int) * (size_t)B : 0);
+  L.o_runs = a.take(plan.rounds_mode ? sizeof(SftRun) * (size_t)B + 64 * kSftMaxSub + 3 * sizeof(int) * (size_t)B : 0);
   if (nh > 0)
     for (int e = 0; e < B * K; e++) {
       const SftProblemPlan& p = plan.prob[e % B];
@@ -453,6 +457,8 @@
   c->d_runs = (SftRun*)(base + L.o_runs);
   c->d_counters = (int*)(base + L.o_runs + sizeof(SftRun) * (size_t)B);
   c->d_linlist = c->d_counters + 16 * kSftMaxSub;
+  c->d_faclist = c->d_linlist + B;
+  c->d_running = c->d_faclist + B;
   c->d_sync = base + L.o_sync;
   c->plan = std::move(plan);
   c->layout = std::move(L);
@@ -708,6 +714,8 @@
   else if (k == "owner_waves") { if (value != 8 && value != 16) return dsh_fail(c, DSH_ERR_ARG, "dsh_lab_set_option: owner_waves is 8 or 16 (wavefronts of a FACTOR workgroup with helpers)"); c->opt.owner_waves = value; }
   else if (k == "helpers") { if (value < -1 || value > 3) return dsh_fail(c, DSH_ERR_ARG, "dsh_lab_set_option: helpers is -1 (automatic) or 0..3 workgroups per part"); c->opt.helpers = value; }
   else if (k == "tail") { if (value < -1 || value > 8) return dsh_fail(c, DSH_ERR_ARG, "dsh_lab_set_option: tail is -1 (automatic), 0 (rounds to the end) or the number of problems per CU from which downwards the last problems go to the tail kernel"); c->opt.tail = value; }
+  else if (k == "carry") { if (value < -1) return dsh_fail(c, DSH_ERR_ARG, "dsh_lab_set_option: carry is -1 (the product's rule), 0 (every running problem is factored in every round) or the largest remainder, in problems, that waits for the next round"); c->opt.carry = value; }
+  else if (k == "factor_waves") { if (value < 0) return dsh_fail(c, DSH_ERR_ARG, "dsh_lab_set_option: factor_waves is 0 (automatic: one per SIMD) or the number of wavefronts of a FACTOR launch"); c->opt.factor_waves = value; }
   else if (k == "speculate") { if (value < 0 || value > SFT_SPEC_MAXK) return dsh_fail(c, DSH_ERR_ARG, "dsh_lab_set_option: speculate is 0 (automatic) or 1..4 lanes"); c->opt.speculate = value; }
   else return dsh_fail(c, DSH_ERR_ARG, "dsh_lab_set_option: unknown option " + k);
   return DSH_OK;
@@ -794,8 +802,9 @@
   for (int b = 0; b < c->B; b++)
     if (c->h_probs[b].tile_mode != 1) return dsh_fail(c, DSH_ERR_STATE, "dsh_lab_sft_factor_check: register-window problems (half-bandwidth <= 128) only");
   const int B = c->B;
-  struct OwnedDevBuf { void* p = nullptr; ~OwnedDevBuf() { if (p) (void)hipFree(p); } } runs, counters;
+  struct OwnedDevBuf { void* p = nullptr; ~OwnedDevBuf() { if (p) (void)hipFree(p); } } runs, counters, list;
   HIPCHK(c, hipMalloc(&runs.p, sizeof(SftRun) * (size_t)B));
+  HIPCHK(c, hipMalloc(&list.p, 2 * sizeof(int) * (size_t)B));
   HIPCHK(c, hipMalloc(&counters.p, 16 * sizeof(int)));
   std::vector<SftRun> h_runs(B);
   for (int b = 0; b < B; b++) {
@@ -807,9 +816,12 @@
   }
   HIPCHK(c, sft_assembly_launch(c->d_probs, B, c->plan.max_kd, c->plan.jl_doubles, c->plan.rounds_mode ? 8 : c->plan.nw, c->stream));
   for (int b = 0; b < B; b++) HIPCHK(c, hipMemcpyAsync(c->h_probs[b].dbg + 1, &lambda[b], sizeof(double), hipMemcpyHostToDevice, c->stream));
+  std::vector<int> h_running(B);
+  for (int b = 0; b < B; b++) h_running[b] = h_runs[b].state == SFTB_TRIAL;
+  HIPCHK(c, hipMemcpyAsync((int*)list.p + B, h_running.data(), sizeof(int) * (size_t)B, hipMemcpyHostToDevice, c->stream));
   HIPCHK(c, hipMemcpyAsync(runs.p, h_runs.data(), sizeof(SftRun) * (size_t)B, hipMemcpyHostToDevice, c->stream));
   HIPCHK(c, hipMemsetAsync(counters.p, 0, 16 * sizeof(int), c->stream));
-  HIPCHK(c, sftb_factor_lab_launch(c->d_probs, (SftRun*)runs.p, (int*)counters.p, B, grid ? grid : std::min(B, 4 * c->num_cus), c->stream));
+  HIPCHK(c, sftb_factor_lab_launch(c->d_probs, (SftRun*)runs.p, (int*)counters.p, (int*)list.p, (const int*)list.p + B, B, grid ? grid : std::min(B, 4 * c->num_cus), c->stream));
   HIPCHK(c, hipStreamSynchronize(c->stream));
   HIPCHK(c, hipMemcpy(h_runs.data(), runs.p, sizeof(SftRun) * (size_t)B, hipMemcpyDeviceToHost));
   size_t off = 0;
@@ -821,6 +833,13 @@
     if (ok) ok[b] = h_runs[b].fact_ok;
   }
   return DSH_OK;
+}
+
+int dsh_lab_sft_round_schedule(const int32_t* trials, int32_t B, int32_t W, int32_t tau, int32_t tail_below, int64_t* out4, int32_t* got, int32_t* round_N, int32_t* round_take, int32_t cap) {
+  if (!trials || !out4 || B <= 0 || W <= 0 || tau < 0 || cap < 0) return DSH_ERR_ARG;
+  int most = 0;
+  for (int b = 0; b < B; b++) { if (trials[b] < 0) return DSH_ERR_ARG; most = std::max(most, trials[b]); }
+  return sft_round_schedule(trials, B, W, tau, tail_below, 2 * (most + 1), out4, got, round_N, round_take, cap) == 0 ? DSH_OK : DSH_ERR_STATE;
 }
 
 int dsh_lab_sft_rounds_timed(dsh_ctx* c, double* ms4, int32_t* rounds) {
@@ -833,14 +852,15 @@
   const int rc = run_rounds(c);
   c->phase_events = nullptr;
   (void)hipStreamSynchronize(c->stream);
-  for (int i = 0; i < 7; i++) ms4[i] = 0.0;
-  { int32_t cnt[16] = {0}; if (hipMemcpy(cnt, c->d_counters, sizeof(cnt), hipMemcpyDeviceToHost) == hipSuccess) { ms4[5] = (double)cnt[8]; ms4[6] = (double)cnt[9]; } }
+  for (int i = 0; i < 9; i++) ms4[i] = 0.0;
+  { int32_t cnt[16] = {0}; if (hipMemcpy(cnt, c->d_counters, sizeof(cnt), hipMemcpyDeviceToHost) == hipSuccess) { ms4[5] = (double)cnt[8]; ms4[6] = (double)cnt[9]; ms4[7] = (double)cnt[13]; } }
   int n_trial = 0;
   for (size_t i = 0; i + 1 < ev.size(); i += 2) {
     float ms = 0.f;
     (void)hipEventElapsedTime(&ms, ev[i], ev[i + 1]);
     const int ph = c->phase_ids[i / 2];
-    ms4[ph == SFTB_PH_INIT ? 0 : ph == SFTB_PH_LIN ? 1 : ph == SFTB_PH_FACTOR ? 2 : ph == SFTB_PH_TRIAL ? 3 : 4] += ms;
+    ms4[ph == SFTB_PH_INIT ? 0 : ph == SFTB_PH_LIN ? 1 : (ph == SFTB_PH_FACTOR || ph == SFTB_PH_PLAN) ? 2 : ph == SFTB_PH_TRIAL ? 3 : 4] += ms;
+    if (ph == SFTB_PH_PLAN) ms4[8] += ms;
     n_trial += ph == SFTB_PH_TRIAL;
   }
   if (rounds) *rounds = n_trial;
diff --git a/defslam_amd/csrc/dsh_sft_ctx.h b/defslam_amd/csrc/dsh_sft_ctx.h
--- a/defslam_amd/csrc/dsh_sft_ctx.h
+++ b/defslam_amd/csrc/dsh_sft_ctx.h
@@ -55,6 +55,8 @@
   SftRun* d_runs = nullptr;
   int* d_counters = nullptr;
   int* d_linlist = nullptr;
+  int* d_faclist = nullptr;
+  int* d_running = nullptr;
   int rounds_hint = 24;
   hipStream_t sub_stream[kSftMaxSub] = {nullptr, nullptr, nullptr, nullptr};
   hipEvent_t sub_event[kSftMaxSub] = {nullptr, nullptr, nullptr, nullptr};
diff --git a/defslam_amd/csrc/sft_batch.h b/defslam_amd/csrc/sft_batch.h
--- a/defslam_amd/csrc/sft_batch.h
+++ b/defslam_amd/csrc/sft_batch.h
@@ -18,15 +18,20 @@
   panel = out + 32;
 }
 
-__global__ __launch_bounds__(64 * SFTB_NW, 2) void sftb_init_kernel(const SftDev* __restrict__ probs, SftRun* __restrict__ runs, int* __restrict__ counters, int* __restrict__ lin_list, int tail_below) {
+#define SFTB_C_START 10
+#define SFTB_C_N 11
+#define SFTB_C_TAKE 12
+#define SFTB_C_SETS 13
+__global__ __launch_bounds__(64 * SFTB_NW, 2) void sftb_init_kernel(const SftDev* __restrict__ probs, SftRun* __restrict__ runs, int* __restrict__ counters, int* __restrict__ lin_list, int* __restrict__ running, int tail_below) {
   const SftDev& P = probs[blockIdx.x];
   if (blockIdx.x == 0 && threadIdx.x == 0 && (int)gridDim.x <= tail_below) counters[6] = 1;
   init_state<64 * SFTB_NW>(P);
   if (threadIdx.x == 0) {
     SftRun& R = runs[blockIdx.x];
     R.lambda = -1.0; R.ni = 2.0; R.chi_cur = 0.0; R.chi_ini = 0.0; R.rho = 0.0; R.lambda_start = 0.0;
-    R.it = 0; R.qmax = 0; R.nbad = 0; R.accepted = 0; R.all_ok = 1; R.iters = 0; R.trials = 0; R.fact_ok = 1;
+    R.it = 0; R.qmax = 0; R.nbad = 0; R.accepted = 0; R.all_ok = 1; R.iters = 0; R.trials = 0; R.fact_ok = 1; R.stamp = 0;
     R.state = P.max_iters > 0 ? SFTB_LIN : SFTB_FINISH;
+    running[blockIdx.x] = 0;
     if (P.max_iters > 0) lin_list[atomicAdd(&counters[2], 1)] = blockIdx.x;
   }
 }
@@ -53,7 +58,7 @@
 }
 
 __global__ __launch_bounds__(64 * SFTB_LIN_NW, SFTB_LIN_WAVES) void sftb_lin_kernel(const SftDev* __restrict__ probs, SftRun* __restrict__ runs, int* __restrict__ counters,
-                                                                                  const int* __restrict__ lin_list, int B, int tail_below) {
+                                                                                  const int* __restrict__ lin_list, int* __restrict__ running, int B, int tail_below) {
   constexpr int NW = SFTB_LIN_NW, NT = 64 * NW;
   extern __shared__ __attribute__((aligned(16))) char smem[];
   __shared__ int next_b;
@@ -75,10 +80,57 @@
     if (b < 0) break;
     if (tid == 0) { nxt = fetch(); atomicAdd(&counters[9], 1); }
     sftb_lin_problem<NW>(probs[b], runs[b], ctl, red, out, panel);
-  }
-}
-
-__global__ __launch_bounds__(64, 1) void sftb_factor_kernel(const SftDev* __restrict__ probs, SftRun* __restrict__ runs, int* __restrict__ counters, int B) {
+    if (tid == 0) running[b] = 1;
+  }
+}
+
+#define SFTB_PLAN_NT 1024
+__global__ __launch_bounds__(SFTB_PLAN_NT) void sftb_plan_kernel(const int* __restrict__ running, int* __restrict__ counters, int* __restrict__ fac_list, int B, int W, int tau) {
+  __shared__ int wsum[SFTB_PLAN_NT / 64];
+  if (counters[6]) return;
+  const int tid = threadIdx.x, lane = tid & 63, wv = tid >> 6;
+  const int start = counters[SFTB_C_START];
+  const int chunk = (B + SFTB_PLAN_NT - 1) / SFTB_PLAN_NT;
+  const int k0 = min(B, tid * chunk), k1 = min(B, k0 + chunk);
+  auto index_at = [&](int k) { const int b = start + k; return b >= B ? b - B : b; };
+  unsigned long long mask = 0;
+  int n = 0;
+  for (int k = k0; k < k1; k += 16) {
+    int st[16];
+#pragma unroll
+    for (int j = 0; j < 16; j++) st[j] = running[k + j < k1 ? index_at(k + j) : 0];
+#pragma unroll
+    for (int j = 0; j < 16; j++) {
+      const int run = k + j < k1 && st[j] != 0;
+      if (k + j - k0 < 64) mask |= (unsigned long long)run << (k + j - k0);
+      n += run;
+    }
+  }
+  int incl = n;
+  for (int d = 1; d < 64; d <<= 1) { const int v = __shfl_up(incl, d, 64); if (lane >= d) incl += v; }
+  if (lane == 63) wsum[wv] = incl;
+  __syncthreads();
+  int base = 0, N = 0;
+  for (int w = 0; w < SFTB_PLAN_NT / 64; w++) { const int v = wsum[w]; if (w < wv) base += v; N += v; }
+  const int take = sft_round_take(N, W, tau);
+  int pos = base + incl - n;
+  for (int k = k0; k < k1; k++) {
+    const int b = index_at(k);
+    const int run = k - k0 < 64 ? (int)((mask >> (k - k0)) & 1) : (int)(running[b] != 0);
+    if (!run) continue;
+    fac_list[pos] = b;
+    if (pos == take) counters[SFTB_C_START] = b;
+    pos++;
+  }
+  if (tid == 0) {
+    if (take == N) counters[SFTB_C_START] = 0;
+    counters[SFTB_C_N] = N;
+    counters[SFTB_C_TAKE] = take;
+    counters[SFTB_C_SETS] += (take + W - 1) / W;
+  }
+}
+
+__global__ __launch_bounds__(64, 1) void sftb_factor_kernel(const SftDev* __restrict__ probs, SftRun* __restrict__ runs, int* __restrict__ counters, const int* __restrict__ fac_list, int round) {
   extern __shared__ __attribute__((aligned(16))) char smem[];
   lds_double* lds = to_lds(reinterpret_cast<double*>(smem));
   const int lane = threadIdx.x;
@@ -89,16 +141,19 @@
   Q.Lg = nullptr; Q.Linv = nullptr; Q.x = nullptr; Q.nT = 0; Q.active = 0; Q.xb = 0.0;
   int n_done = 0;
   while (true) {
-    int b = 0;
-    if (lane == 0) b = atomicAdd(&counters[1], 1);
+    int b = -1;
+    if (lane == 0) {
+      const int take = counters[SFTB_C_TAKE];
+      const int i = atomicAdd(&counters[1], 1);
+      if (i < take) b = fac_list[i];
+    }
     b = __builtin_amdgcn_readfirstlane(b);
-    if (b >= B) break;
-    if (runs[b].state != SFTB_TRIAL) continue;
+    if (b < 0) break;
     const SftDev& P = probs[b];
     const double lambda = runs[b].lambda;
     double xcam;
     const int ok = wv_factor(P, lambda, lambda, lds, Q, xcam);
-    if (lane == 0) runs[b].fact_ok = ok;
+    if (lane == 0) { runs[b].fact_ok = ok; runs[b].stamp = round; }
     Q = wv_prev_of(P, ok, xcam, lane);
     n_done++;
   }
@@ -201,13 +256,14 @@
   return 1;
 }
 
-__global__ __launch_bounds__(64 * SFTB_NW, SFTB_TRIAL_WAVES) void sftb_trial_kernel(const SftDev* __restrict__ probs, SftRun* __restrict__ runs, int* __restrict__ counters, int* __restrict__ lin_list) {
+__global__ __launch_bounds__(64 * SFTB_NW, SFTB_TRIAL_WAVES) void sftb_trial_kernel(const SftDev* __restrict__ probs, SftRun* __restrict__ runs, int* __restrict__ counters, int* __restrict__ lin_list, int* __restrict__ running, int round) {
   constexpr int NW = SFTB_NW, NT = 64 * NW;
   SftRun& R = runs[blockIdx.x];
   const int st = R.state;
   if (counters[6]) return;
   if (blockIdx.x == 0 && threadIdx.x == 0) counters[1] = 0;
   if (st != SFTB_TRIAL && st != SFTB_FINISH) return;
+  if (st == SFTB_TRIAL && R.stamp != round) return;
   extern __shared__ __attribute__((aligned(16))) char smem[];
   const SftDev& P = probs[blockIdx.x];
   Ctl* ctl; double *red, *out, *panel;
@@ -218,7 +274,8 @@
     if (tid == 0) { R.state = SFTB_DONE; atomicAdd(&counters[0], 1); }
     return;
   }
-  (void)sftb_trial_problem<NW>(P, R, ctl, red, out, panel, counters, lin_list, blockIdx.x);
+  const int r = sftb_trial_problem<NW>(P, R, ctl, red, out, panel, counters, lin_list, blockIdx.x);
+  if (r != 0 && tid == 0) running[blockIdx.x] = 0;
 }
 
 __device__ __noinline__ void sftb_solve8(const SftDev& P, unsigned ctl_off, unsigned ws_off, double lambda) {
diff --git a/defslam_amd/csrc/sft_kernels.hip b/defslam_amd/csrc/sft_kernels.hip
--- a/defslam_amd/csrc/sft_kernels.hip
+++ b/defslam_amd/csrc/sft_kernels.hip
@@ -8,6 +8,7 @@
 #include <float.h>
 #define SFT_KERNEL_SOURCE
 #include "sft_problem.h"
+#include "sft_plan.h"
 #include "tile_chol.h"
 
 #define NB 32
@@ -3099,12 +3100,13 @@
 }
 #endif
 
-extern "C" hipError_t sftb_launch(const SftDev* d_probs, SftRun* d_runs, int* d_counters, int* d_list, int B, int phase, size_t jl_doubles, size_t xyz_doubles, size_t* configured, int num_cus, int tail_below, hipStream_t stream) {
+extern "C" hipError_t sftb_launch(const SftDev* d_probs, SftRun* d_runs, int* d_counters, int* d_list, int B, int phase, size_t jl_doubles, size_t xyz_doubles, size_t* configured, int num_cus, int tail_below,
+                                  int* d_fac_list, int* d_running, int factor_waves, int tau, int round, hipStream_t stream) {
   const size_t head = 512 + (16 * 27 + 5 + 32) * sizeof(double) + 64;
   if (phase == SFTB_PH_INIT) {
     hipError_t e = hipMemsetAsync(d_counters, 0, 16 * sizeof(int), stream);
     if (e != hipSuccess) return e;
-    hipLaunchKernelGGL(sftb_init_kernel, dim3(B), dim3(64 * SFTB_NW), 0, stream, d_probs, d_runs, d_counters, d_list, tail_below);
+    hipLaunchKernelGGL(sftb_init_kernel, dim3(B), dim3(64 * SFTB_NW), 0, stream, d_probs, d_runs, d_counters, d_list, d_running, tail_below);
   } else if (phase == SFTB_PH_LIN) {
     const size_t lds = head + jl_doubles * sizeof(double);
     if (lds > configured[0]) {
@@ -3113,9 +3115,11 @@
       configured[0] = lds;
     }
     const int per_cu = lds > 80 * 1024 ? 1 : 2;
-    hipLaunchKernelGGL(sftb_lin_kernel, dim3(std::min(B, per_cu * num_cus)), dim3(64 * SFTB_LIN_NW), lds, stream, d_probs, d_runs, d_counters, d_list, B, tail_below);
+    hipLaunchKernelGGL(sftb_lin_kernel, dim3(std::min(B, per_cu * num_cus)), dim3(64 * SFTB_LIN_NW), lds, stream, d_probs, d_runs, d_counters, d_list, d_running, B, tail_below);
   } else if (phase == SFTB_PH_FACTOR) {
-    hipLaunchKernelGGL(sftb_factor_kernel, dim3(std::min(B, 4 * num_cus)), dim3(64), WV_LDS_DOUBLES * sizeof(double), stream, d_probs, d_runs, d_counters, B);
+    hipLaunchKernelGGL(sftb_factor_kernel, dim3(factor_waves), dim3(64), WV_LDS_DOUBLES * sizeof(double), stream, d_probs, d_runs, d_counters, d_fac_list, round);
+  } else if (phase == SFTB_PH_PLAN) {
+    hipLaunchKernelGGL(sftb_plan_kernel, dim3(1), dim3(SFTB_PLAN_NT), 0, stream, d_running, d_counters, d_fac_list, B, factor_waves, tau);
   } else {
     const size_t lds = head + std::max<size_t>(2048, xyz_doubles) * sizeof(double);
     if (lds > configured[1]) {
@@ -3123,14 +3127,15 @@
       if (e != hipSuccess) return e;
       configured[1] = lds;
     }
-    hipLaunchKernelGGL(sftb_trial_kernel, dim3(B), dim3(64 * SFTB_NW), lds, stream, d_probs, d_runs, d_counters, d_list);
+    hipLaunchKernelGGL(sftb_trial_kernel, dim3(B), dim3(64 * SFTB_NW), lds, stream, d_probs, d_runs, d_counters, d_list, d_running, round);
   }
   return hipGetLastError();
 }
 
 #ifdef DSH_LAB
-extern "C" hipError_t sftb_factor_lab_launch(const SftDev* d_probs, SftRun* d_runs, int* d_counters, int B, int grid, hipStream_t stream) {
-  hipLaunchKernelGGL(sftb_factor_kernel, dim3(grid), dim3(64), WV_LDS_DOUBLES * sizeof(double), stream, d_probs, d_runs, d_counters, B);
+extern "C" hipError_t sftb_factor_lab_launch(const SftDev* d_probs, SftRun* d_runs, int* d_counters, int* d_fac_list, const int* d_running, int B, int grid, hipStream_t stream) {
+  hipLaunchKernelGGL(sftb_plan_kernel, dim3(1), dim3(SFTB_PLAN_NT), 0, stream, d_running, d_counters, d_fac_list, B, grid, 0);
+  hipLaunchKernelGGL(sftb_factor_kernel, dim3(grid), dim3(64), WV_LDS_DOUBLES * sizeof(double), stream, d_probs, d_runs, d_counters, d_fac_list, 0);
   return hipGetLastError();
 }
 #endif
diff --git a/defslam_amd/csrc/sft_plan.cpp b/defslam_amd/csrc/sft_plan.cpp
--- a/defslam_amd/csrc/sft_plan.cpp
+++ b/defslam_amd/csrc/sft_plan.cpp
@@ -36,7 +36,7 @@
     all_tiles = all_tiles && plan.prob[b].tile_mode == 1;
     plan.max_iters_batch = std::max(plan.max_iters_batch, (int)sizes[b].max_iters);
   }
-  if (all_tiles && 2 * B > num_cus) plan.nw = 4;
+  if (all_tiles && (2 * B > num_cus || opt.factor_waves > 0)) plan.nw = 4;
   if ((opt.waves == 4 && all_tiles) || opt.waves == 8) plan.nw = opt.waves;
   if (one_lane) plan.nw = 8;
   plan.rounds_mode = all_tiles && plan.nw == 4 && opt.waves == 0 && opt.rounds != 0 && !host_only;
@@ -93,3 +93,29 @@
   }
   return plan;
 }
+
+int sft_round_schedule(const int32_t* trials, int B, int W, int tau, int tail_below, int max_rounds, int64_t* out, int32_t* got, int32_t* round_N,
+                       int32_t* round_take, int cap) {
+  std::vector<int32_t> left(trials, trials + B), list(B), waited(B, 0);
+  std::vector<uint8_t> running(B);
+  int finished = 0, start = 0, rounds = 0, longest_wait = 0;
+  int64_t sets = 0;
+  if (got) for (int b = 0; b < B; b++) got[b] = 0;
+  while (finished < B && (tail_below < 0 || B - finished > tail_below)) {
+    if (rounds >= max_rounds) return 1;
+    for (int b = 0; b < B; b++) running[b] = left[b] > 0;
+    const SftRoundPlan p = sft_round_plan(running.data(), B, start, W, tau, list.data());
+    if (rounds < cap) { if (round_N) round_N[rounds] = p.N; if (round_take) round_take[rounds] = p.take; }
+    sets += (p.take + W - 1) / W;
+    for (int i = 0; i < p.N; i++) {
+      const int b = list[i];
+      if (i < p.take) { waited[b] = 0; if (got) got[b]++; if (--left[b] == 0) finished++; }
+      else longest_wait = std::max(longest_wait, ++waited[b]);
+    }
+    if (rounds == 0) for (int b = 0; b < B; b++) finished += trials[b] == 0;
+    start = p.next_start;
+    rounds++;
+  }
+  out[0] = rounds; out[1] = sets; out[2] = B - finished; out[3] = longest_wait;
+  return 0;
+}
diff --git a/defslam_amd/csrc/sft_plan.h b/defslam_amd/csrc/sft_plan.h
--- a/defslam_amd/csrc/sft_plan.h
+++ b/defslam_amd/csrc/sft_plan.h
@@ -10,7 +10,31 @@
 constexpr int kTS = 16, kBT = 8, kWB = 16;
 constexpr int kSftMaxSub = 4;
 
-struct SftOptions { int waves = 0; int dataflow = 1; int wide_off = 0; int speculate = 0; int split = 2; int rounds = 1; int streams = 0; int helpers = -1; int tail = -1; int owner_waves = 8; int helpers_wbt = 12; };
+#if defined(__HIPCC__)
+#define SFT_HD __host__ __device__
+#else
+#define SFT_HD
+#endif
+SFT_HD inline int sft_round_take(int N, int W, int tau) {
+  if (W <= 0) return N;
+  const int full = N / W, r = N % W;
+  return (full >= 1 && r > 0 && r <= tau) ? full * W : N;
+}
+inline int sft_round_tau(int W) { return W - W / 4; }
+
+struct SftRoundPlan { int N, take, next_start; };
+inline SftRoundPlan sft_round_plan(const uint8_t* running, int B, int start, int W, int tau, int32_t* fac_list) {
+  SftRoundPlan p{0, 0, 0};
+  for (int k = 0; k < B; k++) { const int b = (start + k) % B; if (running[b]) fac_list[p.N++] = b; }
+  p.take = sft_round_take(p.N, W, tau);
+  p.next_start = p.take < p.N ? fac_list[p.take] : 0;
+  return p;
+}
+
+int sft_round_schedule(const int32_t* trials, int B, int W, int tau, int tail_below, int max_rounds, int64_t* out, int32_t* got, int32_t* round_N,
+                       int32_t* round_take, int cap);
+
+struct SftOptions { int waves = 0; int dataflow = 1; int wide_off = 0; int speculate = 0; int split = 2; int rounds = 1; int streams = 0; int helpers = -1; int tail = -1; int owner_waves = 8; int helpers_wbt = 12; int carry = -1; int factor_waves = 0; };
 
 enum class SftUploadMode { batch, shared_camera, connected };
 
diff --git a/defslam_amd/csrc/sft_problem.h b/defslam_amd/csrc/sft_problem.h
--- a/defslam_amd/csrc/sft_problem.h
+++ b/defslam_amd/csrc/sft_problem.h
@@ -68,11 +68,14 @@
 #define SFTB_PH_LIN 1
 #define SFTB_PH_FACTOR 2
 #define SFTB_PH_TRIAL 3
+#define SFTB_PH_PLAN 5
 #define SFTB_PH_TAIL 4
 struct SftRun {
   double lambda, ni, chi_cur, chi_ini, rho, lambda_start;
   double pose_bak[8];
-  int32_t it, qmax, nbad, accepted, all_ok, iters, trials, state, fact_ok, pad[3];
+  int32_t it, qmax, nbad, accepted, all_ok, iters, trials, state, fact_ok;
+  int32_t stamp;
+  int32_t pad[2];
 };
 
 struct SftPart {
@@ -162,7 +165,7 @@
 extern "C" size_t sft_lm_kernel_lds_bytes(int kd, size_t jl_doubles);
 extern "C" hipError_t sft_lm_launch(const SftDev* d_probs, int B, int max_kd, size_t jl_doubles, int nw, size_t* configured, hipStream_t stream);
 extern "C" hipError_t sftb_launch(const SftDev* d_probs, SftRun* d_runs, int* d_counters, int* d_list, int B, int phase, size_t jl_doubles, size_t xyz_doubles,
-                                  size_t* configured, int num_cus, int tail_below, hipStream_t stream);
+                                  size_t* configured, int num_cus, int tail_below, int* d_fac_list, int* d_running, int factor_waves, int tau, int round, hipStream_t stream);
 extern "C" hipError_t sftb_tail_launch(const SftDev* d_probs, SftRun* d_runs, int* d_counters, int B, int max_kd, size_t jl_doubles, size_t* configured, int num_cus,
                                        int tail_below, hipStream_t stream);
 extern "C" hipError_t sft_spec_launch(const SftDev* d_probs, SftSpec* d_spec, int B, int K, int phase, int nh, int owner_waves, int max_kd, size_t jl_doubles,
@@ -174,5 +177,5 @@
 #ifdef DSH_LAB
 extern "C" hipError_t sft_wave_lab_launch(const SftDev* d_probs, int B, int which, double rel, int max_kd, size_t jl_doubles, hipStream_t stream);
 extern "C" hipError_t sft_assembly_launch(const SftDev* d_probs, int B, int max_kd, size_t jl_doubles, int nw, hipStream_t stream);
-extern "C" hipError_t sftb_factor_lab_launch(const SftDev* d_probs, SftRun* d_runs, int* d_counters, int B, int grid, hipStream_t stream);
+extern "C" hipError_t sftb_factor_lab_launch(const SftDev* d_probs, SftRun* d_runs, int* d_counters, int* d_fac_list, const int* d_running, int B, int grid, hipStream_t stream);
 #endif
diff --git a/defslam_amd/sft.py b/defslam_amd/sft.py
--- a/defslam_amd/sft.py
+++ b/defslam_amd/sft.py
@@ -41,6 +41,7 @@
     status: int = 0
     trace: np.ndarray = field(default=None)
     regs: Optional[tuple] = None
+    max_iters: Optional[int] = None
 
 
 class Context:
@@ -150,7 +151,7 @@
             reg_lap, reg_inex, reg_temp = f.regs
         fc.reg_lap, fc.reg_inex, fc.reg_temp = float(reg_lap), float(reg_inex), float(reg_temp)
         fc.neighbour_layers = int(layers)
-        fc.max_iters = int(max_iters)
+        fc.max_iters = int(max_iters if f.max_iters is None else min(f.max_iters, max_iters))
         return fc
 
     def batch_upload(self, frames: Sequence[Frame], RegLap=5000.0, RegInex=5000.0, RegTemp=0.0, NeighboursLayers=1, max_iters=50):
@@ -237,12 +238,13 @@
         offs = np.concatenate([[0], np.cumsum(dims)])
         return [x[offs[b]:offs[b + 1]] for b in range(B)], ok
 
-    def rounds_timed(self):
+    def rounds_timed(self, sets: bool = False):
         self._need_lab("dsh_lab_sft_rounds_timed")
-        ms = np.zeros(7)
+        ms = np.zeros(9)
         r = np.zeros(1, np.int32)
         self._check(self._L.dsh_lab_sft_rounds_timed(self._h, _ptr(ms, C.c_double), _ptr(r, C.c_int32)), "dsh_lab_sft_rounds_timed")
-        return dict(init=float(ms[0]), lin=float(ms[1]), factor=float(ms[2]), trial=float(ms[3]), tail=float(ms[4]), factorisations_in_rounds=int(ms[5]), linearisations_in_rounds=int(ms[6])), int(r[0])
+        ph = dict(init=float(ms[0]), lin=float(ms[1]), factor=float(ms[2]), trial=float(ms[3]), tail=float(ms[4]), factorisations_in_rounds=int(ms[5]), linearisations_in_rounds=int(ms[6]))
+        return (ph, int(r[0]), dict(wave_sets=int(ms[7]), plan_ms=float(ms[8]))) if sets else (ph, int(r[0]))
 
     def dump(self, b: int, what: int, n: int):
         self._need_lab("dsh_lab_sft_dump")
@@ -487,6 +489,20 @@
     return c0, s, n1p, n1p - n1
 
 
+def round_schedule(trials, W: int, tau: int, tail_below: int = -1):
+    L = _lib.load_lab()
+    t = np.ascontiguousarray(trials, np.int32)
+    cap = 2 * (int(t.max(initial=0)) + 1)
+    out = np.zeros(4, np.int64)
+    got, rn, rt = np.zeros(t.size, np.int32), np.zeros(cap, np.int32), np.zeros(cap, np.int32)
+    rc = L.dsh_lab_sft_round_schedule(_ptr(t, C.c_int32), t.size, int(W), int(tau), int(tail_below), _ptr(out, C.c_int64), _ptr(got, C.c_int32),
+                                      _ptr(rn, C.c_int32), _ptr(rt, C.c_int32), cap)
+    if rc != _lib.DSH_OK:
+        raise RuntimeError(f"dsh_lab_sft_round_schedule failed ({rc})")
+    n = int(out[0])
+    return dict(rounds=n, wave_sets=int(out[1]), tail_problems=int(out[2]), longest_wait=int(out[3]), got=got, N=rn[:n].copy(), take=rt[:n].copy())
+
+
 def frame_from_synth(fr) -> Frame:
     return Frame(Tcw=fr.Tcw.copy(), K=fr.K.copy(), N=fr.n_frame, obs_nodes=fr.obs_nodes, obs_bary=fr.obs_bary, obs_uv=fr.obs_uv,
                  obs_invsig2=fr.obs_invsig2, nodes_xyz=fr.xyz.copy())
diff --git a/include/defslam_hip_debug.h b/include/defslam_hip_debug.h
--- a/include/defslam_hip_debug.h
+++ b/include/defslam_hip_debug.h
@@ -17,7 +17,9 @@
 int dsh_lab_sft_assemble_timed(dsh_ctx* ctx, int launches, double* total_ms);
 int dsh_lab_sft_wave_check(dsh_ctx* ctx, double rel, int launches, int only, double* x_ref, double* x_new, int32_t* ok2, double* ms2);
 int dsh_lab_sft_factor_check(dsh_ctx* ctx, const double* lambda, const uint8_t* factor, int grid, double* x, int32_t* ok);
-int dsh_lab_sft_rounds_timed(dsh_ctx* ctx, double* ms7, int32_t* rounds);
+int dsh_lab_sft_rounds_timed(dsh_ctx* ctx, double* ms9, int32_t* rounds);
+int dsh_lab_sft_round_schedule(const int32_t* trials, int32_t B, int32_t W, int32_t tau, int32_t tail_below, int64_t* out4, int32_t* got,
+                               int32_t* round_N, int32_t* round_take, int32_t cap);
 int dsh_lab_sft_dump(dsh_ctx* ctx, int b, int what, int64_t n, double* out);
 int dsh_lab_sft_phase_ms(dsh_ctx* ctx, int b, double* out8);
 int dsh_lab_sft_step_trace(dsh_ctx* ctx, int b, double* out64);
```

After: 421,100. No clear change (-0.2%).
